# chongchen1999/llm-inference-engine

Measured on AMD Instinct MI355X. Metric: decode_tokens_per_s, higher is better.
Workload: dtype f16; 1 GPU; Llama-2-7B 32-layer fp16 decode, batch 1, ctx 2048 (BASELINE configs[2]); random-init weights, synthetic ids, KV pre-filled; global_batch=1, seq_len=2048, parallelism=replicas x1 (no collective), graph=True, layers=32

## Files before the change

include/llmie.h:

```cpp
#ifndef LLMIE_H
#define LLMIE_H

#include <stddef.h>
#include <stdint.h>

#ifdef __cplusplus
extern "C" {
#endif

#define LLMIE_ABI_VERSION 3

typedef enum { LLMIE_F32 = 0, LLMIE_F16 = 1 } llmie_dtype;

typedef enum {
    LLMIE_OK = 0,
    LLMIE_ERR_INVALID_ARG = -1,
    LLMIE_ERR_UNSUPPORTED = -2,
    LLMIE_ERR_LAUNCH = -3,
    LLMIE_ERR_WORKSPACE = -4
} llmie_status;

typedef void *llmie_stream;

typedef enum {
// ... 60 lines not shown
                      int step, const int32_t *step_dev, int rotary_dim, float rotary_base,
                      llmie_dtype dtype, llmie_stream stream);

size_t llmie_decoder_mha_workspace_bytes(int batch, int head_num, int head_size, int max_seq_len);
int llmie_decoder_mha(const void *qkv, const void *qkv_bias, void *k_cache, void *v_cache,
                      void *out, int layer, int batch, int head_num, int kv_head_num,
                      int head_size, int max_seq_len, int step, const int32_t *step_dev,
                      void *workspace, size_t workspace_bytes,
                      llmie_dtype dtype, llmie_stream stream);

int llmie_decoder_mha_rope(const void *qkv, const void *qkv_bias, void *k_cache, void *v_cache,
                           void *out, int layer, int batch, int head_num, int kv_head_num,
                           int head_size, int max_seq_len, int step, const int32_t *step_dev,
                           void *workspace, size_t workspace_bytes, const void *rope_table,
                           int rotary_dim, int32_t *tickets, llmie_dtype dtype, llmie_stream stream);

int llmie_decoder_mha_ragged(const void *qkv, const void *qkv_bias, void *k_cache, void *v_cache, void *out, int layer,
                             int batch, int head_num, int kv_head_num, int head_size, int max_seq_len,
                             const int32_t *ctx_len_dev, void *workspace, size_t workspace_bytes, const void *rope_table,
                             int rotary_dim, const int32_t *block_table, int max_pages, int num_pages,
                             llmie_dtype dtype, llmie_stream stream);

int llmie_concat_kv(const void *src, void *cache, const int32_t *cur_len,
                    const int32_t *history_len, int layer, int batch, int kv_head_num,
                    int max_q_len, int max_seq_len, int head_size,
                    llmie_dtype dtype, llmie_stream stream);

int llmie_repeat_kv(const void *cache, void *dst, const int32_t *ctx_len, int layer, int batch,
                    int head_num, int kv_head_num, int max_k_len, int max_seq_len, int head_size,
                    llmie_dtype dtype, llmie_stream stream);

int llmie_scale_mask_softmax(const void *qk, const void *mask, void *out, float scale,
                             int batch, int head_num, int q_len, int k_len,
                             llmie_dtype dtype, llmie_stream stream);

int llmie_transpose_remove_padding(const void *src, void *dst, const int32_t *padding_offset,
                                   int num_tokens, int batch, int seq_len, int head_num,
                                   int head_size, llmie_dtype dtype, llmie_stream stream);

int llmie_silu_and_mul(const void *in, void *out, int num_tokens, int inter,
                       llmie_dtype dtype, llmie_stream stream);

int llmie_topk(const void *probs, int32_t *tmp_ids, void *tmp_vals, int32_t *ids, void *vals,
               int rows, int vocab, int K, int blocks_per_row,
               llmie_dtype dtype, llmie_stream stream);

int llmie_sampling(const int32_t *topk_id, const void *topk_val, int32_t *seq_len,
                   uint8_t *finished, int32_t *out_id, int batch, int K, int step,
                   const int32_t *step_dev, int end_id, int vocab,
                   llmie_dtype dtype, llmie_stream stream);

typedef struct {
    float temperature;
    int top_k;
    float top_p;
    float min_p;
    float repetition_penalty;
    float presence_penalty;
    float frequency_penalty;
    uint32_t seed;
} llmie_sampling_params;
#define LLMIE_SAMPLE_MAX_HISTORY 8192
size_t llmie_sample_logits_workspace_bytes(int batch, int vocab);
int llmie_sample_logits(const void *logits, int batch, int vocab, const llmie_sampling_params *params_dev, int32_t *history,
                        int history_stride, int32_t *history_len, int history_append, int32_t *seq_len, uint8_t *finished,
                        int32_t *out_id, float *out_logprob, int step, const int32_t *step_dev, int end_id, void *workspace,
                        size_t workspace_bytes, llmie_dtype dtype, llmie_stream stream);

size_t llmie_score_tokens_workspace_bytes(int rows, int hidden_size, int vocab);
int llmie_score_tokens(const void *hidden, const void *norm_gamma, float rms_eps, const void *lm_head, const void *lm_bias,
                       const int32_t *targets, float *out_logprob, float *out_lse, int32_t *out_argmax,
                       float *out_argmax_logprob, int rows, int hidden_size, int vocab, void *workspace,
                       size_t workspace_bytes, llmie_dtype dtype, llmie_stream stream);


int llmie_linear_w8a16(const void *x, const int8_t *wq, const void *scale, void *y,
                       int M, int K, int N, const void *bias, const void *residual,
                       void *workspace, size_t workspace_bytes, llmie_stream stream);
int llmie_linear_w4a16(const void *x, const uint8_t *wq, const void *scale, void *y,
                       int M, int K, int N, int group, const void *bias, const void *residual,
                       void *workspace, size_t workspace_bytes, llmie_stream stream);
int llmie_linear_fp8(const void *x, const uint8_t *w_fp8, const float *w_scale, void *y,
                     int M, int K, int N, const void *bias, const void *residual,
                     void *workspace, size_t workspace_bytes, llmie_stream stream);
size_t llmie_linear_fp8_workspace_bytes(int M, int K, int N);
int llmie_linear_fp8_swiglu(const void *x, const uint8_t *w_fp8, const float *w_scale, void *y, int M, int K,
                            int two_inter, void *workspace, size_t workspace_bytes, llmie_stream stream);
int llmie_quantize_w8(const void *w, int8_t *wq, void *scale, int N, int K, llmie_stream stream);
int llmie_quantize_w4(const void *w, uint8_t *wq, void *scale, int N, int K, int group,
                      llmie_stream stream);
int llmie_quantize_fp8(const void *w, uint8_t *wq, float *scale, int N, int K, llmie_stream stream);

size_t llmie_packed_weight_bytes(llmie_weight_format fmt, int N, int K, int swiglu_pairs);
size_t llmie_packed_scale_bytes(llmie_weight_format fmt, int N, int K, int swiglu_pairs);
int llmie_pack_weight(llmie_weight_format fmt, const void *w, const void *scale, void *packed, void *packed_scale,
                      int N, int K, int swiglu_pairs, llmie_stream stream);
size_t llmie_linear_packed_workspace_bytes(llmie_weight_format fmt, int M, int K, int N);
enum { LLMIE_X32_X = 1, LLMIE_X32_Y = 2, LLMIE_X32_RES = 4 };
size_t llmie_x32_bytes(int C);
int llmie_x32_convert(const void *src, void *dst, int M, int C, int to_x32, llmie_stream stream);
int llmie_linear_packed(llmie_weight_format fmt, const void *x, const void *packed, const void *scale, void *y,
                        int M, int K, int N, int swiglu, int x32_flags, const void *residual, const void *gamma,
                        const void *pre_bias, float eps, void *workspace, size_t workspace_bytes,
                        llmie_stream stream);


typedef enum { LLMIE_KV_NATIVE = 0, LLMIE_KV_FP8 = 1 } llmie_kv_format;

typedef struct {
    const void *data;
    const void *scale;
    const void *bias;
} llmie_matrix;

typedef struct {
    const void *attn_norm_gamma;
    llmie_matrix qkv;
    llmie_matrix o;
    const void *ffn_norm_gamma;
    llmie_matrix gate_up;
    llmie_matrix down;
} llmie_layer_weights;

typedef struct {
    int head_num, kv_head_num, head_size, inter_size, num_layers, vocab_size;
    int max_seq_len, max_batch;
    int rotary_dim;
    float rotary_base, rms_eps;
    llmie_dtype dtype;
    llmie_weight_format wfmt;
    int int4_group;
    llmie_kv_format kv_fmt;
    float k_scale, v_scale;
    int flags;
} llmie_decoder_config;

#define LLMIE_DEC_NO_PACKED_COPY 1
#define LLMIE_DEC_PACKED_ONLY 2
size_t llmie_decoder_resident_weight_bytes(const llmie_decoder_config *cfg);

#define LLMIE_PLAN_PAGED 1u
#define LLMIE_PLAN_RAGGED 2u
#define LLMIE_PLAN_HIDDEN_MISALIGNED 4u
#define LLMIE_PLAN_WEIGHTS_MISALIGNED 8u
#define LLMIE_PLAN_GAMMAS_MISALIGNED 16u
#define LLMIE_PLAN_O_BIAS 32u
#define LLMIE_PLAN_SCALES_MISALIGNED 64u
#define LLMIE_SW_NO_FUSED_DECODE 1u
#define LLMIE_SW_NO_FUSED_BATCH 2u
#define LLMIE_SW_NO_PACKED_BATCH 4u
#define LLMIE_SW_CHAIN 8u
#define LLMIE_SW_NO_FUSED_SHORT_PREFILL 16u
#define LLMIE_SW_NO_QKV_ROPE_FUSION 32u
const char *llmie_decoder_plan_name(const llmie_decoder_config *cfg, int prefill, int rows, unsigned call_flags, unsigned switch_mask);

typedef struct llmie_decoder llmie_decoder;

size_t llmie_decoder_workspace_bytes(const llmie_decoder_config *cfg);
llmie_decoder *llmie_decoder_create(const llmie_decoder_config *cfg,
                                    const llmie_layer_weights *layers,
                                    void *workspace, size_t workspace_bytes);
void llmie_decoder_destroy(llmie_decoder *dec);
int llmie_decoder_repack(llmie_decoder *dec, const llmie_layer_weights *layers, llmie_stream stream);

int llmie_decoder_forward(llmie_decoder *dec, const void *hidden_in, void *hidden_out,
                          void *k_cache, void *v_cache, int batch, int step,
                          const int32_t *step_dev, llmie_stream stream);

#define LLMIE_KV_PAGE_TOKENS 128
int llmie_decoder_forward_paged(llmie_decoder *dec, const void *hidden_in, void *hidden_out, void *k_pool, void *v_pool,
                                const int32_t *block_table, int max_pages, int num_pages, int batch, int step,
                                const int32_t *step_dev, llmie_stream stream);
int llmie_decoder_forward_ragged(llmie_decoder *dec, const void *hidden_in, void *hidden_out, void *k_cache, void *v_cache,
                                 int batch, const int32_t *ctx_len_dev, llmie_stream stream);
int llmie_decoder_forward_paged_ragged(llmie_decoder *dec, const void *hidden_in, void *hidden_out, void *k_pool, void *v_pool,
                                       const int32_t *block_table, int max_pages, int num_pages, int batch,
                                       const int32_t *ctx_len_dev, llmie_stream stream);
int llmie_decoder_prefill_paged(llmie_decoder *dec, const void *hidden_in, void *hidden_out, void *k_pool, void *v_pool,
                                const int32_t *block_table, int max_pages, int num_pages, const int32_t *input_lengths,
                                const int32_t *history_lengths, int batch, int num_tokens, int max_q_len, void *workspace,
                                size_t workspace_bytes, llmie_stream stream);
int llmie_kv_pages_copy(void *dense, void *pool, const int32_t *block_table, const int32_t *ctx_len, int to_pages,
                        int layers, int batch, int kv_head_num, int max_seq_len, int head_size, int max_pages,
                        int num_pages, int elem_bytes, llmie_stream stream);

size_t llmie_decoder_prefill_workspace_bytes(const llmie_decoder_config *cfg, int max_tokens, int max_batch);
int llmie_decoder_prefill(llmie_decoder *dec, const void *hidden_in, void *hidden_out, void *k_cache, void *v_cache,
                          const int32_t *input_lengths, const int32_t *history_lengths, int batch, int num_tokens,
                          int max_q_len, void *workspace, size_t workspace_bytes, llmie_stream stream);

int llmie_lm_head_sample(llmie_decoder *dec, void *hidden ,
                         const void *final_norm_gamma, const llmie_matrix *lm_head,
                         llmie_weight_format lm_fmt, void *logits,
                         int32_t *tmp_ids, void *tmp_vals, int32_t *topk_ids, void *topk_vals,
                         int K, int blocks_per_row, int32_t *seq_len, uint8_t *finished,
                         int32_t *out_ids, int batch, int step, const int32_t *step_dev,
                         int end_id, llmie_stream stream);

int llmie_lm_head_sample_next(llmie_decoder *dec, void *hidden, const void *final_norm_gamma, const llmie_matrix *lm_head,
                              llmie_weight_format lm_fmt, void *logits, int32_t *tmp_ids, void *tmp_vals, int32_t *topk_ids,
                              void *topk_vals, int K, int blocks_per_row, int32_t *seq_len, uint8_t *finished, int32_t *out_ids,
                              int batch, int step, int32_t *step_dev, int end_id, const void *embed_table, void *next_hidden,
                              int advance_step, llmie_stream stream);

int llmie_lm_head_sample_params(llmie_decoder *dec, void *hidden, const void *final_norm_gamma, const llmie_matrix *lm_head,
                                llmie_weight_format lm_fmt, void *logits, const llmie_sampling_params *params_dev, int32_t *history,
                                int history_stride, int32_t *history_len, int history_append, int32_t *seq_len, uint8_t *finished,
                                int32_t *out_ids, float *out_logprob, int batch, int step, int32_t *step_dev, int end_id,
                                const void *embed_table, void *next_hidden, int advance_step, void *workspace, size_t workspace_bytes,
                                llmie_stream stream);

enum {
    LLMIE_OP_ATTN_NORM = 0, LLMIE_OP_QKV_GEMM, LLMIE_OP_ROPE, LLMIE_OP_MHA, LLMIE_OP_O_GEMM,
    LLMIE_OP_FFN_NORM, LLMIE_OP_GATE_UP_SWIGLU, LLMIE_OP_DOWN_GEMM, LLMIE_OP_FINAL_NORM,
    LLMIE_OP_LM_HEAD, LLMIE_OP_TOPK, LLMIE_OP_SAMPLING,
    LLMIE_OP_CHAIN,
    LLMIE_OP_COUNT
};
int llmie_decoder_profile_begin(llmie_decoder *dec, int max_events);
int llmie_decoder_profile_end(llmie_decoder *dec, llmie_stream stream, double *ms_by_op ,
                              int *launches_by_op );

int llmie_decoder_status(llmie_decoder *dec, llmie_stream stream);
int llmie_decoder_debug_stamps(llmie_decoder *dec, void *stamps_dev);

int llmie_advance_step(int32_t *step_dev, llmie_stream stream);

#ifdef __cplusplus
}
#endif
#endif
```

llm-inference-engine_amd/csrc/attention_decode.hip:

```cpp
#include "llmie_internal.h"

#include <cstdlib>
#include <type_traits>

namespace llmie {

struct fp8kv_t {
    uint8_t b;
};
template <typename KT> struct CacheVec {
    using type = typename Vec16<KT>::type;
    static constexpr int n = Vec16<KT>::n;
};
template <> struct CacheVec<fp8kv_t> {
    using type = uint4_t;
    static constexpr int n = 16;
};
template <typename KT, int N> __device__ __forceinline__ void kv_to_f32(const typename CacheVec<KT>::type &v, float (&o)[N]) {
    if constexpr (std::is_same<KT, fp8kv_t>::value) {
#pragma unroll
        for (int w = 0; w < 4; ++w) {
            const auto lo = __builtin_amdgcn_cvt_pk_f32_fp8(static_cast<int>(v[w]), false);
            const auto hi = __builtin_amdgcn_cvt_pk_f32_fp8(static_cast<int>(v[w]), true);
            o[4 * w] = lo[0];
            o[4 * w + 1] = lo[1];
            o[4 * w + 2] = hi[0];
            o[4 * w + 3] = hi[1];
        }
    } else {
#pragma unroll
        for (int e = 0; e < N; ++e) o[e] = to_f32(v[e]);
    }
}
template <typename KT, typename T, int N> __device__ __forceinline__ typename CacheVec<KT>::type kv_pack(const T (&x)[N], float inv_scale) {
    typename CacheVec<KT>::type v;
    if constexpr (std::is_same<KT, fp8kv_t>::value) {
#pragma unroll
        for (int w = 0; w < 4; ++w)
            v[w] = pack4_e4m3(to_f32(x[4 * w]) * inv_scale, to_f32(x[4 * w + 1]) * inv_scale, to_f32(x[4 * w + 2]) * inv_scale,
                              to_f32(x[4 * w + 3]) * inv_scale);
    } else {
#pragma unroll
        for (int e = 0; e < N; ++e) v[e] = x[e];
    }
    return v;
}
template <typename T, int N> __device__ __forceinline__ void load_elems(const T *p, T (&dst)[N]) {
    constexpr int PER = Vec16<T>::n;
    static_assert(N % PER == 0, "whole 16-byte loads");
#pragma unroll
    for (int c = 0; c < N / PER; ++c) {
        const typename Vec16<T>::type v = reinterpret_cast<const typename Vec16<T>::type *>(p)[c];
#pragma unroll
        for (int e = 0; e < PER; ++e) dst[c * PER + e] = v[e];
    }
}

template <typename KT, int HS, int NWV = 4, int GL = 8> struct AttnGeom {
    static constexpr int N = CacheVec<KT>::n;
    static constexpr int LPT = HS / N;
    static constexpr int TPW = 64 / LPT;
    static constexpr int CHUNK = NWV * GL * TPW;
};

__host__ __device__ inline int attn_min_chunk() { return 32; }

struct QkvSlabs {
    const float *slab;
    int KS;
    size_t stride;
    SlabScale sc;
};

constexpr int KV_PAGE = 128;
struct PagedKv {
    const int32_t *table;
    int max_pages;
    int step_stride;
    int out_x32;
};
__device__ __forceinline__ int seq_step(const int32_t *step_dev, int step_arg, int stride, int b, int max_seq_len) {
    const int s = step_dev ? step_dev[static_cast<size_t>(b) * stride] : step_arg;
    return (s >= 1 && s <= max_seq_len) ? s : 0;
}
__device__ __forceinline__ size_t attn_out_index(int x32, int b, int k, int width) {
    if (!x32) return static_cast<size_t>(b) * width + k;
    return (static_cast<size_t>(k >> 5) * 2 + (b >> 4)) * 512 + ((k & 31) >> 3) * 128 + (b & 15) * 8 + (k & 7);
}

__device__ __forceinline__ void merge_round(const float (&ms)[16], const float (&ls)[16], const float (&os)[16], int s0, int nsplits,
                                            float &M, float &L, float &o) {
    float Mc = M;
#pragma unroll
    for (int i = 0; i < 16; ++i)
        if (s0 + i < nsplits) Mc = fmaxf(Mc, ms[i]);
    const float rescale = (M == -INFINITY) ? 0.f : __expf(M - Mc);
    L *= rescale;
    o *= rescale;
#pragma unroll
    for (int i = 0; i < 16; ++i)
        if (s0 + i < nsplits) {
            const float f = __expf(ms[i] - Mc);
            L = fmaf(f, ls[i], L);
            o = fmaf(f, os[i], o);
        }
    M = Mc;
}
__device__ __forceinline__ void merge_load(const float *__restrict__ p, int s0, int last, size_t stride, int d, float (&ms)[16],
                                           float (&ls)[16], float (&os)[16]) {
#pragma unroll
    for (int i = 0; i < 16; ++i) {
        const int s = min(s0 + i, last);
        ms[i] = p[s * stride];
        ls[i] = p[s * stride + 1];
        os[i] = p[s * stride + 2 + d];
    }
}
__device__ __forceinline__ float merge_splits(const float *__restrict__ p, int nsplits, size_t stride, int d) {
    float M = -INFINITY, L = 0.f, o = 0.f;
    for (int s0 = 0; s0 < nsplits; s0 += 16) {
        float ms[16], ls[16], os[16];
        merge_load(p, s0, nsplits - 1, stride, d, ms, ls, os);
        merge_round(ms, ls, os, s0, nsplits, M, L, o);
    }
    return o / (L + 1e-6f);
}

template <typename T, int HS, int REP, int kAttnWaves = 4, int kAttnG = 8, typename KT = T>
__global__ __launch_bounds__(kAttnWaves * 64) void decode_attn_split_kernel(
    const T *__restrict__ qkv, const T *__restrict__ qkv_bias, KT *k_cache, KT *v_cache,
    float *__restrict__ part, T *__restrict__ out, int head_num, int kv_head_num, int max_seq_len,
    int step_arg, const int32_t *__restrict__ step_dev, int max_splits,
    const float2 *__restrict__ rope , int rotary_dim,
    int32_t *tickets ,
    const QkvSlabs qs ,
    const float k_scale, const float v_scale ,
    const PagedKv pg ,
    const int cpw ) {
    using G = AttnGeom<KT, HS, kAttnWaves, kAttnG>;
    using V = typename CacheVec<KT>::type;
    constexpr int N = G::N, LPT = G::LPT, TPW = G::TPW, CHUNK = G::CHUNK;
    constexpr int NT = kAttnWaves * 64;
    constexpr bool FP8KV = std::is_same<KT, fp8kv_t>::value;
    static_assert(HS % N == 0 && LPT >= 1 && LPT <= 64 && (LPT & (LPT - 1)) == 0, "head size");

    const int split = blockIdx.x, g = blockIdx.y, b = blockIdx.z;
    const int step = seq_step(step_dev, step_arg, pg.step_stride, b, max_seq_len);
    const int span = cpw * CHUNK;
    const int t0 = split * span;
    if (t0 >= step) return;
    int tc0 = t0;
    int t_end = min(step, tc0 + CHUNK);
    const int nsplits = (step + span - 1) / span;
    const int batch = gridDim.z;

    const int lane = threadIdx.x & 63, wave = threadIdx.x >> 6;
    const int sub = lane / LPT, dl = lane % LPT;
    const int qkv_heads = head_num + 2 * kv_head_num;
    const float scale = rsqrtf(static_cast<float>(HS));

    const T *row = qkv + static_cast<size_t>(b) * qkv_heads * HS;
    constexpr int NPG = CHUNK > KV_PAGE ? CHUNK / KV_PAGE : 1;
    static_assert(CHUNK % KV_PAGE == 0 || KV_PAGE % CHUNK == 0, "chunk vs page size");
    int pg0 = 0;
    KT *kbase[NPG], *vbase[NPG];
    auto set_pages = [&]() {
        pg0 = tc0 / KV_PAGE;
#pragma unroll
        for (int j = 0; j < NPG; ++j) {
            size_t off;
            if (pg.table) {
                const int page = pg.table[static_cast<size_t>(b) * pg.max_pages + min(pg0 + j, pg.max_pages - 1)];
                off = (static_cast<size_t>(page) * kv_head_num + g) * KV_PAGE * HS;
            } else {
                off = (static_cast<size_t>(b) * kv_head_num + g) * max_seq_len * HS + static_cast<size_t>(pg0 + j) * KV_PAGE * HS;
            }
            kbase[j] = k_cache + off;
            vbase[j] = v_cache + off;
        }
    };
    set_pages();
    auto krow = [&](int t) { return kbase[NPG == 1 ? 0 : (t / KV_PAGE - pg0)] + static_cast<size_t>(t % KV_PAGE) * HS; };
    auto vrow = [&](int t) { return vbase[NPG == 1 ? 0 : (t / KV_PAGE - pg0)] + static_cast<size_t>(t % KV_PAGE) * HS; };
    KT *kc = kbase[0];
    const int t_new = step - 1;
    T qraw[REP][N];
    constexpr int ITEMS_PER_HEAD = HS / 4;
    constexpr int LROUNDS = ((REP + 2) * ITEMS_PER_HEAD + NT - 1) / NT;
    __shared__ __attribute__((aligned(16))) T qkvlds[(REP + 2) * HS];
    const bool wg_has_new = t_new >= t0 && t_new < t0 + span;
    floatx4 spart[LROUNDS][4];
    half4_t sscale[LROUNDS];
    floatx4 sscalef[LROUNDS];
    const float xs_b = (qs.slab && qs.sc.wf) ? qs.sc.xs[b] : 1.f;
    size_t scol[LROUNDS];
    bool sact[LROUNDS];
    if (qs.slab) {
#pragma unroll
        for (int lr = 0; lr < LROUNDS; ++lr) {
            const int item = lr * NT + threadIdx.x;
            const int hsel = item / ITEMS_PER_HEAD, d4 = item - hsel * ITEMS_PER_HEAD;
            sact[lr] = hsel < REP || (wg_has_new && hsel < REP + 2);
            const int hh = hsel < REP ? g * REP + hsel : (hsel == REP ? head_num + g : head_num + kv_head_num + g);
            scol[lr] = static_cast<size_t>(hh) * HS + d4 * 4;
            if (sact[lr]) {
                const float *p = qs.slab + static_cast<size_t>(b) * qkv_heads * HS + scol[lr];
#pragma unroll
                for (int kk = 0; kk < 4; ++kk)
                    spart[lr][kk] = *reinterpret_cast<const floatx4 *>(p + static_cast<size_t>(min(kk, qs.KS - 1)) * qs.stride);
                if (qs.sc.wh) sscale[lr] = *reinterpret_cast<const half4_t *>(qs.sc.wh + scol[lr]);
                if (qs.sc.wf) sscalef[lr] = *reinterpret_cast<const floatx4 *>(qs.sc.wf + scol[lr]);
            }
        }
    } else {
#pragma unroll
        for (int r = 0; r < REP; ++r) load_elems<T, N>(row + static_cast<size_t>(g * REP + r) * HS + dl * N, qraw[r]);
    }
    const int hk = head_num + g, hv = head_num + kv_head_num + g;
    const T *dummy = reinterpret_cast<const T *>(kc);
    T knraw[N], vnraw[N], qbias[REP][N], kbias[N], vbias[N];
    load_elems<T, N>(qs.slab ? dummy : row + static_cast<size_t>(hk) * HS + dl * N, knraw);
    load_elems<T, N>(qs.slab ? dummy : row + static_cast<size_t>(hv) * HS + dl * N, vnraw);
#pragma unroll
    for (int r = 0; r < REP; ++r)
        load_elems<T, N>(qkv_bias ? qkv_bias + static_cast<size_t>(g * REP + r) * HS + dl * N : dummy, qbias[r]);
    load_elems<T, N>(qkv_bias ? qkv_bias + static_cast<size_t>(hk) * HS + dl * N : dummy, kbias);
    load_elems<T, N>(qkv_bias ? qkv_bias + static_cast<size_t>(hv) * HS + dl * N : dummy, vbias);
    float2 csraw[N];
    if (rope) {
        const float2 *cs = rope + static_cast<size_t>(t_new) * (HS / 2) + (dl % (LPT / 2)) * N;
#pragma unroll
        for (int e = 0; e < N; ++e) csraw[e] = cs[e];
    }
    V kv[kAttnG], vv[kAttnG];
    int tok[kAttnG];
    auto issue_loads = [&]() {
#pragma unroll
        for (int i = 0; i < kAttnG; ++i) {
            const int t = tc0 + (wave * kAttnG + i) * TPW + sub;
            tok[i] = t;
            kv[i] = load_nt(reinterpret_cast<const V *>(krow(min(t, t_end - 1))) + dl);
        }
#pragma unroll
        for (int i = 0; i < kAttnG; ++i)
            vv[i] = load_nt(reinterpret_cast<const V *>(vrow(min(tok[i], t_end - 1))) + dl);
    };
    issue_loads();
    if (qs.slab) {
#pragma unroll
        for (int lr = 0; lr < LROUNDS; ++lr) {
            if (sact[lr]) {
                const float *p = qs.slab + static_cast<size_t>(b) * qkv_heads * HS + scol[lr];
                floatx4 f = spart[lr][0];
#pragma unroll
                for (int kk = 1; kk < 4; ++kk)
                    if (kk < qs.KS) f += spart[lr][kk];
                for (int k = 4; k < qs.KS; ++k) f += *reinterpret_cast<const floatx4 *>(p + static_cast<size_t>(k) * qs.stride);
                const int item = lr * NT + threadIdx.x;
#pragma unroll
                for (int e = 0; e < 4; ++e) {
                    float v = f[e];
                    if (qs.sc.wh) v *= to_f32(sscale[lr][e]);
                    if (qs.sc.wf) v *= sscalef[lr][e] * xs_b;
                    qkvlds[item * 4 + e] = from_f32<T>(v);
                }
            }
        }
        __syncthreads();
#pragma unroll
        for (int r = 0; r < REP; ++r) load_elems<T, N>(&qkvlds[r * HS + dl * N], qraw[r]);
    }
    const bool rope_first = dl < LPT / 2;
    float rc[N], rs[N];
    if (rope) {
#pragma unroll
        for (int e = 0; e < N; ++e) {
            const bool rot = ((dl % (LPT / 2)) * N + e) < (rotary_dim >> 1);
            const float2 v = rot ? csraw[e] : float2{1.f, 0.f};
            rc[e] = v.x;
            rs[e] = rope_first ? -v.y : v.y;
        }
    }
    auto rotate = [&](float (&x)[N]) {
#pragma unroll
        for (int e = 0; e < N; ++e) {
            const float partner = (LPT / 2 < 16) ? lane_xor_lt16<(LPT / 2 < 16 ? LPT / 2 : 8)>(x[e]) : __shfl_xor(x[e], LPT / 2, 64);
            x[e] = x[e] * rc[e] + partner * rs[e];
        }
    };
    const float k_p2 = __builtin_bit_cast(float, __builtin_bit_cast(uint32_t, k_scale) & 0x7f800000u);
    const float k_q = FP8KV ? k_scale / k_p2 : k_scale;
    (void)k_p2;
    float qf[REP][N];
#pragma unroll
    for (int r = 0; r < REP; ++r) {
        float f[N];
#pragma unroll
        for (int e = 0; e < N; ++e) f[e] = to_f32(qraw[r][e]);
        if (rope) {
            rotate(f);
#pragma unroll
            for (int e = 0; e < N; ++e) f[e] = to_f32(from_f32<T>(f[e]));
        }
#pragma unroll
        for (int e = 0; e < N; ++e) {
            f[e] += qkv_bias ? to_f32(qbias[r][e]) : 0.f;
            qf[r][e] = f[e] * (scale * k_q);
        }
    }
    half2_t qh[FP8KV ? REP : 1][FP8KV ? N / 2 : 1];
    if constexpr (FP8KV) {
#pragma unroll
        for (int r = 0; r < REP; ++r)
#pragma unroll
            for (int j = 0; j < N / 2; ++j) qh[r][j] = half2_t{from_f32<half_t>(qf[r][2 * j]), from_f32<half_t>(qf[r][2 * j + 1])};
    }

    V knv, vnv;
    {
        T kn[N], vn[N];
#pragma unroll
        for (int e = 0; e < N; ++e) {
            kn[e] = knraw[e];
            vn[e] = vnraw[e];
        }
        if (qs.slab) {
            load_elems<T, N>(&qkvlds[REP * HS + dl * N], kn);
            load_elems<T, N>(&qkvlds[(REP + 1) * HS + dl * N], vn);
        }
        if (rope) {
            float f[N];
#pragma unroll
            for (int e = 0; e < N; ++e) f[e] = to_f32(kn[e]);
            rotate(f);
#pragma unroll
            for (int e = 0; e < N; ++e) kn[e] = from_f32<T>(f[e]);
        }
#pragma unroll
        for (int e = 0; e < N; ++e) {
            kn[e] = qkv_bias ? from_f32<T>(to_f32(kn[e]) + to_f32(kbias[e])) : kn[e];
            vn[e] = qkv_bias ? from_f32<T>(to_f32(vn[e]) + to_f32(vbias[e])) : vn[e];
        }
        knv = kv_pack<KT, T, N>(kn, 1.0f / k_scale);
        vnv = kv_pack<KT, T, N>(vn, 1.0f / v_scale);
    }
    auto inject = [&]() {
        bool mine = false;
        if (t_new >= tc0 && t_new < tc0 + CHUNK) {
#pragma unroll
        for (int i = 0; i < kAttnG; ++i) {
            const bool is_new = tok[i] == t_new;
            mine |= is_new;
            uint4_t kw = __builtin_bit_cast(uint4_t, kv[i]), vw = __builtin_bit_cast(uint4_t, vv[i]);
            const uint4_t knw = __builtin_bit_cast(uint4_t, knv), vnw = __builtin_bit_cast(uint4_t, vnv);
#pragma unroll
            for (int w = 0; w < 4; ++w) {
                kw[w] = is_new ? knw[w] : kw[w];
                vw[w] = is_new ? vnw[w] : vw[w];
            }
            kv[i] = __builtin_bit_cast(V, kw);
            vv[i] = __builtin_bit_cast(V, vw);
        }
        }
        if (mine) {
            reinterpret_cast<V *>(krow(t_new))[dl] = knv;
            reinterpret_cast<V *>(vrow(t_new))[dl] = vnv;
        }
    };
    inject();

    float mx[REP], acc[REP][N], ls[REP];
#pragma unroll
    for (int r = 0; r < REP; ++r) {
        mx[r] = -INFINITY;
        ls[r] = 0.f;
#pragma unroll
        for (int e = 0; e < N; ++e) acc[r][e] = 0.f;
    }
    auto accumulate = [&](const bool first) {
    float lg[REP][kAttnG];
    float cm[REP];
#pragma unroll
    for (int r = 0; r < REP; ++r) cm[r] = -INFINITY;
#pragma unroll
    for (int i = 0; i < kAttnG; ++i) {
        const bool valid = tok[i] < t_end;
        float kf[FP8KV ? 1 : N];
        half2_t kh[FP8KV ? N / 2 : 1];
        if constexpr (FP8KV) {
            const uint4_t kw = __builtin_bit_cast(uint4_t, kv[i]);
#pragma unroll
            for (int w = 0; w < 4; ++w) {
                kh[2 * w] = __builtin_amdgcn_cvt_scalef32_pk_f16_fp8(static_cast<int>(kw[w]), k_p2, false);
                kh[2 * w + 1] = __builtin_amdgcn_cvt_scalef32_pk_f16_fp8(static_cast<int>(kw[w]), k_p2, true);
            }
        } else {
            kv_to_f32<KT, N>(kv[i], kf);
        }
#pragma unroll
        for (int r = 0; r < REP; ++r) {
            float d = 0.f;
            if (valid) {
                if constexpr (FP8KV) {
#pragma unroll
                    for (int j = 0; j < N / 2; ++j) d = __builtin_amdgcn_fdot2(kh[j], qh[r][j], d, false);
                } else {
#pragma unroll
                    for (int e = 0; e < N; ++e) d = fmaf(qf[r][e], kf[e], d);
                }
            }
            d = group_sum<LPT>(d);
            lg[r][i] = valid ? d : -INFINITY;
            cm[r] = fmaxf(cm[r], lg[r][i]);
        }
    }
#pragma unroll
    for (int r = 0; r < REP; ++r) {
#pragma unroll
        for (int o = LPT; o < 64; o <<= 1) cm[r] = lane_xor_max_o(cm[r], o);
        const float mnew = fmaxf(mx[r], cm[r]);
        if (!first) {
            const float f = (mx[r] == -INFINITY) ? 0.f : __expf(mx[r] - mnew);
            ls[r] *= f;
#pragma unroll
            for (int e = 0; e < N; ++e) acc[r][e] *= f;
        }
        mx[r] = mnew;
    }
#pragma unroll
    for (int i = 0; i < kAttnG; ++i) {
        const bool valid = tok[i] < t_end;
        if (valid) {
            float vf[N];
            kv_to_f32<KT, N>(vv[i], vf);
#pragma unroll
            for (int r = 0; r < REP; ++r) {
                const float p = __expf(lg[r][i] - mx[r]);
                ls[r] += p;
#pragma unroll
                for (int e = 0; e < N; ++e) acc[r][e] = fmaf(p, vf[e], acc[r][e]);
            }
        }
    }
    };
    accumulate(true);
    if constexpr (FP8KV) {
        for (int c = 1; c < cpw; ++c) {
            tc0 += CHUNK;
            if (tc0 >= step) break;
            t_end = min(step, tc0 + CHUNK);
            set_pages();
            issue_loads();
            inject();
            accumulate(false);
        }
    }
#pragma unroll
    for (int r = 0; r < REP; ++r) {
#pragma unroll
        for (int o = LPT; o < 64; o <<= 1) {
            ls[r] = lane_xor_sum_o(ls[r], o);
#pragma unroll
            for (int e = 0; e < N; ++e) acc[r][e] = lane_xor_sum_o(acc[r][e], o);
        }
    }
    __shared__ float s_m[REP][kAttnWaves], s_l[REP][kAttnWaves];
    __shared__ float s_o[REP][kAttnWaves][HS];
    if (sub == 0) {
#pragma unroll
        for (int r = 0; r < REP; ++r) {
#pragma unroll
            for (int e = 0; e < N; ++e) s_o[r][wave][dl * N + e] = acc[r][e] * v_scale;
            if (dl == 0) {
                s_m[r][wave] = mx[r];
                s_l[r][wave] = ls[r];
            }
        }
    }
    __syncthreads();
    for (int i = threadIdx.x; i < REP * HS; i += NT) {
        const int r = i / HS, d = i - r * HS;
        float M = s_m[r][0];
#pragma unroll
        for (int w = 1; w < kAttnWaves; ++w) M = fmaxf(M, s_m[r][w]);
        float L = 0.f, o = 0.f;
#pragma unroll
        for (int w = 0; w < kAttnWaves; ++w) {
            const float f = (s_m[r][w] == -INFINITY) ? 0.f : __expf(s_m[r][w] - M);
            L += f * s_l[r][w];
            o += f * s_o[r][w][d];
        }
        const int h = g * REP + r;
        if (nsplits == 1) {
            out[attn_out_index(pg.out_x32, b, h * HS + d, head_num * HS)] = from_f32<T>(o / (L + 1e-6f));
        } else {
            float *p = part + ((static_cast<size_t>(b) * head_num + h) * max_splits + split) * (HS + 2);
            p[2 + d] = o;
            if (d == 0) {
                p[0] = M;
                p[1] = L;
            }
        }
    }
    (void)batch;
    if (tickets && nsplits > 1) {
        __shared__ int s_ticket;
        asm volatile("s_waitcnt vmcnt(0)" ::: "memory");
        __syncthreads();
        int32_t *cnt = tickets + static_cast<size_t>(b) * kv_head_num + g;
        if (threadIdx.x == 0) {
            __builtin_amdgcn_fence(__ATOMIC_RELEASE, "agent");
            asm volatile("s_waitcnt vmcnt(0)" ::: "memory");
            s_ticket = __hip_atomic_fetch_add(cnt, 1, __ATOMIC_RELAXED, __HIP_MEMORY_SCOPE_AGENT);
        }
        __syncthreads();
        if (s_ticket == nsplits - 1) {
            if (threadIdx.x == 0) {
                __builtin_amdgcn_fence(__ATOMIC_ACQUIRE, "agent");
                asm volatile("s_waitcnt vmcnt(0)" ::: "memory");
                __hip_atomic_store(cnt, 0, __ATOMIC_RELAXED, __HIP_MEMORY_SCOPE_AGENT);
            }
            __syncthreads();
            const size_t stride = static_cast<size_t>(HS) + 2;
            for (int i = threadIdx.x; i < REP * HS; i += NT) {
                const int r = i / HS, d = i - r * HS;
                const int h = g * REP + r;
                const float *p = part + (static_cast<size_t>(b) * head_num + h) * max_splits * stride;
                const float v = merge_splits(p, nsplits, stride, d);
                out[attn_out_index(pg.out_x32, b, h * HS + d, head_num * HS)] = from_f32<T>(v);
            }
        }
    }
}

template <typename T>
__global__ __launch_bounds__(256) void decode_attn_combine_kernel(const float *__restrict__ part,
                                                                  T *__restrict__ out, int head_num,
                                                                  int head_size, int chunk, int step_arg,
                                                                  const int32_t *__restrict__ step_dev,
                                                                  int max_splits, int step_stride, int max_seq_len, int out_x32) {
    const int h = blockIdx.x, b = blockIdx.y;
    const size_t stride = static_cast<size_t>(head_size) + 2;
    const float *p = part + (static_cast<size_t>(b) * head_num + h) * max_splits * stride;
    int d = threadIdx.x;
    float ms[16], ls[16], os[16];
    merge_load(p, 0, max_splits - 1, stride, min(d, head_size - 1), ms, ls, os);
    const int step = seq_step(step_dev, step_arg, step_stride, b, max_seq_len);
    const int nsplits = (step + chunk - 1) / chunk;
    if (nsplits <= 1) return;
    if (d < head_size) {
        float M = -INFINITY, L = 0.f, o = 0.f;
        merge_round(ms, ls, os, 0, nsplits, M, L, o);
        for (int s0 = 16; s0 < nsplits; s0 += 16) {
            merge_load(p, s0, nsplits - 1, stride, d, ms, ls, os);
            merge_round(ms, ls, os, s0, nsplits, M, L, o);
        }
        out[attn_out_index(out_x32, b, h * head_size + d, head_num * head_size)] = from_f32<T>(o / (L + 1e-6f));
    }
    for (d += blockDim.x; d < head_size; d += blockDim.x)
        out[attn_out_index(out_x32, b, h * head_size + d, head_num * head_size)] = from_f32<T>(merge_splits(p, nsplits, stride, d));
}

template <typename T>
__global__ __launch_bounds__(256) void decode_attn_generic_kernel(
    const T *__restrict__ qkv, const T *__restrict__ qkv_bias, T *k_cache, T *v_cache, T *__restrict__ out,
    int head_num, int kv_head_num, int head_size, int max_seq_len, int step_arg,
    const int32_t *__restrict__ step_dev) {
    extern __shared__ float logits[];
    __shared__ float red[4];
    const int h = blockIdx.x, b = blockIdx.y;
    const int step = seq_step(step_dev, step_arg, 0, b, max_seq_len);
    if (step == 0) return;
    const int rep = head_num / kv_head_num, g = h / rep;
    const int qkv_heads = head_num + 2 * kv_head_num;
    const T *row = qkv + static_cast<size_t>(b) * qkv_heads * head_size;
    const int hk = head_num + g, hv = head_num + kv_head_num + g;
    const size_t head_off = (static_cast<size_t>(b) * kv_head_num + g) * max_seq_len * head_size;
    T *kc = k_cache + head_off, *vc = v_cache + head_off;
    const int t_new = step - 1;
    const float scale = rsqrtf(static_cast<float>(head_size));
    auto qv = [&](int d) { return to_f32(row[static_cast<size_t>(h) * head_size + d]) + (qkv_bias ? to_f32(qkv_bias[static_cast<size_t>(h) * head_size + d]) : 0.f); };
    auto knew = [&](int d) { return from_f32<T>(to_f32(row[static_cast<size_t>(hk) * head_size + d]) + (qkv_bias ? to_f32(qkv_bias[static_cast<size_t>(hk) * head_size + d]) : 0.f)); };
    auto vnew = [&](int d) { return from_f32<T>(to_f32(row[static_cast<size_t>(hv) * head_size + d]) + (qkv_bias ? to_f32(qkv_bias[static_cast<size_t>(hv) * head_size + d]) : 0.f)); };
    if (h % rep == 0) {
        for (int d = threadIdx.x; d < head_size; d += 256) {
            kc[static_cast<size_t>(t_new) * head_size + d] = knew(d);
            vc[static_cast<size_t>(t_new) * head_size + d] = vnew(d);
        }
    }
    float mx = -INFINITY;
    for (int t = threadIdx.x; t < step; t += 256) {
        float acc = 0.f;
        for (int d = 0; d < head_size; ++d) {
            const float kvl = (t == t_new) ? to_f32(knew(d)) : to_f32(kc[static_cast<size_t>(t) * head_size + d]);
            acc = fmaf(qv(d), kvl, acc);
        }
        acc *= scale;
        logits[t] = acc;
        mx = fmaxf(mx, acc);
    }
    mx = block_max<4>(mx, red);
    float sum = 0.f;
    for (int t = threadIdx.x; t < step; t += 256) {
        const float p = expf(logits[t] - mx);
        logits[t] = p;
        sum += p;
    }
    sum = block_sum<4>(sum, red) + 1e-6f;
    __syncthreads();
    for (int d = threadIdx.x; d < head_size; d += 256) {
        float o = 0.f;
        for (int t = 0; t < step; ++t) {
            const float vvl = (t == t_new) ? to_f32(vnew(d)) : to_f32(vc[static_cast<size_t>(t) * head_size + d]);
            o = fmaf(logits[t], vvl, o);
        }
        out[(static_cast<size_t>(b) * head_num + h) * head_size + d] = from_f32<T>(o / sum);
    }
}

struct KvScale {
    float k, v;
};

template <typename T, int HS, int REP, typename KT = T>
static void launch_split(const T *qkv, const T *bias, KT *kc, KT *vc, float *part, T *out, int batch,
                         int head_num, int kv_head_num, int max_seq_len, int step, const int32_t *step_dev,
                         int max_splits_ws, const float2 *rope, int rot_dim, int32_t *tickets, const QkvSlabs &qs,
                         KvScale ks, PagedKv pg, hipStream_t st) {
    const int bound = step_dev ? max_seq_len : step;
    int cpw = 1;
    if constexpr (!std::is_same<KT, T>::value) {
        while (cpw < 8 && batch * kv_head_num >= 128 * cpw) cpw *= 2;
    }
    int CHUNK, splits;
#define LLMIE_ATTN_LAUNCH(NWV_, GL_)                                                                                   \
    do {                                                                                                                \
        CHUNK = cpw * AttnGeom<KT, HS, NWV_, GL_>::CHUNK;                                                               \
        splits = (bound + CHUNK - 1) / CHUNK;                                                                           \
        dim3 grid(splits, kv_head_num, batch);                                                                          \
        decode_attn_split_kernel<T, HS, REP, NWV_, GL_, KT><<<grid, NWV_ * 64, 0, st>>>(                                \
            qkv, bias, kc, vc, part, out, head_num, kv_head_num, max_seq_len, step, step_dev, max_splits_ws, rope, rot_dim, \
            tickets, qs, ks.k, ks.v, pg, cpw);                                                                          \
    } while (0)
    LLMIE_ATTN_LAUNCH(4, 8);
#undef LLMIE_ATTN_LAUNCH
    if (splits > 1 && !tickets) {
        dim3 cgrid(head_num, batch);
        decode_attn_combine_kernel<T><<<cgrid, HS < 64 ? 64 : (HS > 256 ? 256 : HS), 0, st>>>(part, out, head_num, HS, CHUNK,
                                                                                              step, step_dev, max_splits_ws, pg.step_stride,
                                                                                              max_seq_len, pg.out_x32);
    }
}

template <typename T, int HS, typename KT = T>
static bool dispatch_rep(int rep, const T *qkv, const T *bias, KT *kc, KT *vc, float *part, T *out, int batch,
                         int head_num, int kv_head_num, int max_seq_len, int step, const int32_t *step_dev,
                         int max_splits_ws, const float2 *rope, int rot_dim, int32_t *tickets, const QkvSlabs &qs,
                         KvScale ks, PagedKv pg, hipStream_t st) {
    switch (rep) {
        case 1: launch_split<T, HS, 1, KT>(qkv, bias, kc, vc, part, out, batch, head_num, kv_head_num, max_seq_len, step, step_dev, max_splits_ws, rope, rot_dim, tickets, qs, ks, pg, st); return true;
        case 2: launch_split<T, HS, 2, KT>(qkv, bias, kc, vc, part, out, batch, head_num, kv_head_num, max_seq_len, step, step_dev, max_splits_ws, rope, rot_dim, tickets, qs, ks, pg, st); return true;
        case 4: launch_split<T, HS, 4, KT>(qkv, bias, kc, vc, part, out, batch, head_num, kv_head_num, max_seq_len, step, step_dev, max_splits_ws, rope, rot_dim, tickets, qs, ks, pg, st); return true;
        case 8:
            if constexpr (!std::is_same<KT, T>::value) return false;
            else launch_split<T, HS, 8, KT>(qkv, bias, kc, vc, part, out, batch, head_num, kv_head_num, max_seq_len, step, step_dev, max_splits_ws, rope, rot_dim, tickets, qs, ks, pg, st); return true;
        default: return false;
    }
}

template <typename T>
static int decoder_mha_impl(const T *qkv, const T *bias, T *k_cache, T *v_cache, T *out, int layer, int batch,
                            int head_num, int kv_head_num, int head_size, int max_seq_len, int step,
                            const int32_t *step_dev, void *workspace, size_t workspace_bytes, const float2 *rope,
                            int rot_dim, int32_t *tickets, const QkvSlabs &qs, hipStream_t st, PagedKv pg = PagedKv{nullptr, 0, 0, 0},
                            int num_pages = 0) {
    const size_t layer_off = pg.table ? static_cast<size_t>(layer) * num_pages * kv_head_num * KV_PAGE * head_size
                                      : static_cast<size_t>(layer) * batch * kv_head_num * max_seq_len * head_size;
    T *kc = k_cache + layer_off, *vc = v_cache + layer_off;
    const int rep = head_num / kv_head_num;
    const int max_splits_ws = (max_seq_len + attn_min_chunk() - 1) / attn_min_chunk();
    const bool aligned = ((reinterpret_cast<uintptr_t>(qkv) | reinterpret_cast<uintptr_t>(kc) |
                           reinterpret_cast<uintptr_t>(vc)) % 16 == 0) && (!bias || reinterpret_cast<uintptr_t>(bias) % 16 == 0);
    bool done = false;
    if (aligned && batch <= 65535 && kv_head_num <= 65535) {
        const size_t need = llmie_decoder_mha_workspace_bytes(batch, head_num, head_size, max_seq_len);
        float *part = static_cast<float *>(workspace);
        auto ws_ok = [&]() { return workspace && workspace_bytes >= need; };
        if (head_size == 128 && ws_ok())
            done = dispatch_rep<T, 128>(rep, qkv, bias, kc, vc, part, out, batch, head_num, kv_head_num, max_seq_len, step, step_dev, max_splits_ws, rope, rot_dim, tickets, qs, KvScale{1.f, 1.f}, pg, st);
        else if (head_size == 64 && ws_ok())
            done = dispatch_rep<T, 64>(rep, qkv, bias, kc, vc, part, out, batch, head_num, kv_head_num, max_seq_len, step, step_dev, max_splits_ws, rope, rot_dim, tickets, qs, KvScale{1.f, 1.f}, pg, st);
        else if (head_size == 32 && ws_ok())
            done = dispatch_rep<T, 32>(rep, qkv, bias, kc, vc, part, out, batch, head_num, kv_head_num, max_seq_len, step, step_dev, max_splits_ws, rope, rot_dim, tickets, qs, KvScale{1.f, 1.f}, pg, st);
        else if (head_size == 256 && ws_ok())
            done = dispatch_rep<T, 256>(rep, qkv, bias, kc, vc, part, out, batch, head_num, kv_head_num, max_seq_len, step, step_dev, max_splits_ws, rope, rot_dim, tickets, qs, KvScale{1.f, 1.f}, pg, st);
        if (!done && (head_size == 128 || head_size == 64 || head_size == 32 || head_size == 256) && !ws_ok() &&
            (rep == 1 || rep == 2 || rep == 4 || rep == 8)) {
            set_error("decoder_mha: workspace too small (%zu < %zu bytes)", workspace_bytes, need);
            return LLMIE_ERR_WORKSPACE;
        }
    }
    if (!done && pg.table) {
        set_error("decoder_mha: the paged KV cache needs head_size in {32,64,128,256} and head_num/kv_head_num in {1,2,4,8}");
        return LLMIE_ERR_UNSUPPORTED;
    }
    if (!done && qs.slab) {
        set_error("decoder_mha: q/k/v from split-K slabs needs head_size in {32,64,128,256} and head_num/kv_head_num in {1,2,4,8}");
        return LLMIE_ERR_UNSUPPORTED;
    }
    if (!done && rope) {
        set_error("decoder_mha: fused RoPE needs head_size in {32,64,128,256} and head_num/kv_head_num in {1,2,4,8}");
        return LLMIE_ERR_UNSUPPORTED;
    }
    if (!done && (pg.step_stride || pg.out_x32)) {
        set_error("decoder_mha: ragged batches / x32 output need head_size in {32,64,128,256} and head_num/kv_head_num in {1,2,4,8}");
        return LLMIE_ERR_UNSUPPORTED;
    }
    if (!done) {
        const int bound = step_dev ? max_seq_len : step;
        const size_t lds = sizeof(float) * static_cast<size_t>(bound);
        if (lds > 60 * 1024) {
            set_error("decoder_mha: generic path supports at most 15360 tokens (head_size=%d, rep=%d)", head_size, rep);
            return LLMIE_ERR_UNSUPPORTED;
        }
        dim3 grid(head_num, batch);
        decode_attn_generic_kernel<T><<<grid, 256, lds, st>>>(qkv, bias, kc, vc, out, head_num, kv_head_num,
                                                             head_size, max_seq_len, step, step_dev);
    }
    return launch_status("decoder_mha");
}

static int decoder_mha_fp8kv(const half_t *qkv, const half_t *bias, uint8_t *k_cache, uint8_t *v_cache, half_t *out, int layer, int batch,
                             int head_num, int kv_head_num, int head_size, int max_seq_len, int step, const int32_t *step_dev,
                             void *workspace, size_t workspace_bytes, const float2 *rope, int rot_dim, const QkvSlabs &qs,
                             KvScale ks, hipStream_t st, PagedKv pg, int num_pages) {
    const size_t layer_off = pg.table ? static_cast<size_t>(layer) * num_pages * kv_head_num * KV_PAGE * head_size
                                      : static_cast<size_t>(layer) * batch * kv_head_num * max_seq_len * head_size;
    fp8kv_t *kc = reinterpret_cast<fp8kv_t *>(k_cache) + layer_off, *vc = reinterpret_cast<fp8kv_t *>(v_cache) + layer_off;
    const int rep = head_num / kv_head_num;
    const int max_splits_ws = (max_seq_len + attn_min_chunk() - 1) / attn_min_chunk();
    const size_t need = llmie_decoder_mha_workspace_bytes(batch, head_num, head_size, max_seq_len);
    if ((reinterpret_cast<uintptr_t>(qkv) | reinterpret_cast<uintptr_t>(kc) | reinterpret_cast<uintptr_t>(vc) |
         reinterpret_cast<uintptr_t>(bias)) % 16 || !workspace || workspace_bytes < need || batch > 65535 || !(ks.k > 0.f) ||
        !(ks.v > 0.f) || (rep != 1 && rep != 2 && rep != 4) || (head_size != 128 && head_size != 64)) {
        set_error("decoder_mha(fp8 KV): needs head_size 64/128, head ratio 1/2/4, 16-byte aligned buffers, positive scales and "
                  "the llmie_decoder_mha workspace");
        return LLMIE_ERR_UNSUPPORTED;
    }
    float *part = static_cast<float *>(workspace);
    bool done;
    if (head_size == 128)
        done = dispatch_rep<half_t, 128, fp8kv_t>(rep, qkv, bias, kc, vc, part, out, batch, head_num, kv_head_num, max_seq_len, step,
                                                  step_dev, max_splits_ws, rope, rot_dim, nullptr, qs, ks, pg, st);
    else
        done = dispatch_rep<half_t, 64, fp8kv_t>(rep, qkv, bias, kc, vc, part, out, batch, head_num, kv_head_num, max_seq_len, step,
                                                 step_dev, max_splits_ws, rope, rot_dim, nullptr, qs, ks, pg, st);
    (void)done;
    return launch_status("decoder_mha(fp8 KV)");
}

int decoder_mha_rope(const void *qkv, const void *qkv_bias, const KvView &kv, void *out, int layer, int batch,
                     int head_num, int kv_head_num, int head_size, int max_seq_len, const DecodePos &pos,
                     void *workspace, size_t workspace_bytes, const float2 *rope, int rot_dim, int32_t *tickets,
                     llmie_dtype dtype, hipStream_t st, const SplitKSlabs *qkv_slabs, const SlabScale *qkv_scale, int out_x32) {
    void *k_cache = kv.k, *v_cache = kv.v;
    const int32_t *block_table = kv.block_table, *step_dev = pos.step_dev;
    const int max_pages = kv.max_pages, num_pages = kv.num_pages, kv_fp8 = kv.fp8, step = pos.step, ragged = pos.ragged;
    const float k_scale = kv.k_scale, v_scale = kv.v_scale;
    const PagedKv pg{block_table, max_pages, ragged ? 1 : 0, out_x32 ? 1 : 0};
    if (ragged && !step_dev) {
        set_error("decoder_mha: a ragged batch needs the device array of context lengths");
        return LLMIE_ERR_INVALID_ARG;
    }
    if (out_x32 && (batch > 32 || dtype != LLMIE_F16)) {
        set_error("decoder_mha: the x32 output image holds at most 32 fp16 rows");
        return LLMIE_ERR_UNSUPPORTED;
    }
    if (block_table && (max_pages <= 0 || num_pages <= 0 || static_cast<long long>(max_pages) * KV_PAGE < max_seq_len)) {
        set_error("decoder_mha: paged KV cache needs max_pages * %d >= max_seq_len and num_pages > 0", KV_PAGE);
        return LLMIE_ERR_UNSUPPORTED;
    }
    QkvSlabs qs{nullptr, 0, 0, SlabScale{nullptr, nullptr, nullptr}};
    const SlabScale no_scale{nullptr, nullptr, nullptr};
    const SlabScale &qsc = qkv_scale ? *qkv_scale : no_scale;
    if (qkv_slabs && (reinterpret_cast<uintptr_t>(qsc.wh) % 8 || reinterpret_cast<uintptr_t>(qsc.wf) % 16 ||
                      reinterpret_cast<uintptr_t>(qkv_slabs->slab) % 16 ||
                      (static_cast<size_t>(qkv_slabs->M) * qkv_slabs->N) % 4)) {
        set_error("decoder_mha: q/k/v from split-K slabs needs 16-byte aligned slabs and aligned scale vectors");
        return LLMIE_ERR_UNSUPPORTED;
    }
    if (qkv_slabs) qs = QkvSlabs{qkv_slabs->slab, qkv_slabs->KS, static_cast<size_t>(qkv_slabs->M) * qkv_slabs->N, qsc};
    if (kv_fp8) {
        if (dtype != LLMIE_F16 || tickets) {
            set_error("decoder_mha(fp8 KV): fp16 activations, separate merge kernel only");
            return LLMIE_ERR_UNSUPPORTED;
        }
        return decoder_mha_fp8kv((const half_t *)qkv, (const half_t *)qkv_bias, (uint8_t *)k_cache, (uint8_t *)v_cache, (half_t *)out,
                                 layer, batch, head_num, kv_head_num, head_size, max_seq_len, step, step_dev, workspace,
                                 workspace_bytes, rope, rot_dim, qs, KvScale{k_scale, v_scale}, st, pg, num_pages);
    }
    if (dtype == LLMIE_F32)
        return decoder_mha_impl<float>((const float *)qkv, (const float *)qkv_bias, (float *)k_cache, (float *)v_cache,
                                       (float *)out, layer, batch, head_num, kv_head_num, head_size, max_seq_len, step,
                                       step_dev, workspace, workspace_bytes, rope, rot_dim, tickets, qs, st, pg, num_pages);
    return decoder_mha_impl<half_t>((const half_t *)qkv, (const half_t *)qkv_bias, (half_t *)k_cache, (half_t *)v_cache,
                                    (half_t *)out, layer, batch, head_num, kv_head_num, head_size, max_seq_len, step,
                                    step_dev, workspace, workspace_bytes, rope, rot_dim, tickets, qs, st, pg, num_pages);
}

}

using namespace llmie;

extern "C" size_t llmie_decoder_mha_workspace_bytes(int batch, int head_num, int head_size, int max_seq_len) {
    if (batch <= 0 || head_num <= 0 || head_size <= 0 || max_seq_len <= 0) return 0;
    const size_t splits = (static_cast<size_t>(max_seq_len) + attn_min_chunk() - 1) / attn_min_chunk();
    return static_cast<size_t>(batch) * head_num * splits * (head_size + 2) * sizeof(float);
}

extern "C" int llmie_decoder_mha(const void *qkv, const void *qkv_bias, void *k_cache, void *v_cache, void *out,
                                 int layer, int batch, int head_num, int kv_head_num, int head_size,
                                 int max_seq_len, int step, const int32_t *step_dev, void *workspace,
                                 size_t workspace_bytes, llmie_dtype dtype, llmie_stream stream) {
    LLMIE_REQUIRE(qkv && k_cache && v_cache && out, "decoder_mha: NULL pointer");
    LLMIE_REQUIRE(layer >= 0 && batch > 0 && head_num > 0 && kv_head_num > 0 && head_size > 0 && max_seq_len > 0,
                  "decoder_mha: bad shape");
    LLMIE_REQUIRE(head_num % kv_head_num == 0, "decoder_mha: kv_head_num must divide head_num");
    LLMIE_REQUIRE(step_dev || (step >= 1 && step <= max_seq_len), "decoder_mha: step %d outside [1, max_seq_len=%d]",
                  step, max_seq_len);
    if (dtype == LLMIE_F32)
        return decoder_mha_impl<float>((const float *)qkv, (const float *)qkv_bias, (float *)k_cache, (float *)v_cache,
                                       (float *)out, layer, batch, head_num, kv_head_num, head_size, max_seq_len, step,
                                       step_dev, workspace, workspace_bytes, nullptr, 0, nullptr, QkvSlabs{nullptr, 0, 0, SlabScale{nullptr, nullptr, nullptr}}, as_stream(stream));
    if (dtype == LLMIE_F16)
        return decoder_mha_impl<half_t>((const half_t *)qkv, (const half_t *)qkv_bias, (half_t *)k_cache,
                                        (half_t *)v_cache, (half_t *)out, layer, batch, head_num, kv_head_num, head_size,
                                        max_seq_len, step, step_dev, workspace, workspace_bytes, nullptr, 0, nullptr, QkvSlabs{nullptr, 0, 0, SlabScale{nullptr, nullptr, nullptr}}, as_stream(stream));
    LLMIE_UNSUPPORTED("decoder_mha: dtype %d", (int)dtype);
}

extern "C" int llmie_decoder_mha_rope(const void *qkv, const void *qkv_bias, void *k_cache, void *v_cache, void *out,
                                      int layer, int batch, int head_num, int kv_head_num, int head_size,
                                      int max_seq_len, int step, const int32_t *step_dev, void *workspace,
                                      size_t workspace_bytes, const void *rope_table, int rotary_dim, int32_t *tickets,
                                      llmie_dtype dtype, llmie_stream stream) {
    LLMIE_REQUIRE(qkv && k_cache && v_cache && out, "decoder_mha_rope: NULL pointer");
    LLMIE_REQUIRE(layer >= 0 && batch > 0 && head_num > 0 && kv_head_num > 0 && head_size > 0 && max_seq_len > 0,
                  "decoder_mha_rope: bad shape");
    LLMIE_REQUIRE(head_num % kv_head_num == 0, "decoder_mha_rope: kv_head_num must divide head_num");
    LLMIE_REQUIRE(step_dev || (step >= 1 && step <= max_seq_len), "decoder_mha_rope: step %d outside [1, max_seq_len=%d]",
                  step, max_seq_len);
    LLMIE_REQUIRE(!rope_table || (rotary_dim > 0 && rotary_dim % 2 == 0), "decoder_mha_rope: bad rotary_dim");
    if (dtype != LLMIE_F32 && dtype != LLMIE_F16) LLMIE_UNSUPPORTED("decoder_mha_rope: dtype %d", (int)dtype);
    const int rep = head_num / kv_head_num;
    const bool hs_ok = head_size == 32 || head_size == 64 || head_size == 128 || head_size == 256;
    const bool rep_ok = rep == 1 || rep == 2 || rep == 4 || rep == 8;
    if ((rope_table || tickets) && !(hs_ok && rep_ok))
        LLMIE_UNSUPPORTED("decoder_mha_rope: fused RoPE / in-launch merge need head_size in {32,64,128,256} and "
                          "head_num/kv_head_num in {1,2,4,8}");
    return decoder_mha_rope(qkv, qkv_bias, kv_dense(k_cache, v_cache), out, layer, batch, head_num, kv_head_num, head_size,
                            max_seq_len, DecodePos{step, step_dev, 0}, workspace, workspace_bytes,
                            static_cast<const float2 *>(rope_table), rotary_dim, tickets, dtype, as_stream(stream));
}

extern "C" int llmie_decoder_mha_ragged(const void *qkv, const void *qkv_bias, void *k_cache, void *v_cache, void *out, int layer,
                                        int batch, int head_num, int kv_head_num, int head_size, int max_seq_len,
                                        const int32_t *ctx_len_dev, void *workspace, size_t workspace_bytes, const void *rope_table,
                                        int rotary_dim, const int32_t *block_table, int max_pages, int num_pages,
                                        llmie_dtype dtype, llmie_stream stream) {
    LLMIE_REQUIRE(qkv && k_cache && v_cache && out && ctx_len_dev, "decoder_mha_ragged: NULL pointer");
    LLMIE_REQUIRE(layer >= 0 && batch > 0 && head_num > 0 && kv_head_num > 0 && head_size > 0 && max_seq_len > 0,
                  "decoder_mha_ragged: bad shape");
    LLMIE_REQUIRE(head_num % kv_head_num == 0, "decoder_mha_ragged: kv_head_num must divide head_num");
    LLMIE_REQUIRE(!rope_table || (rotary_dim > 0 && rotary_dim % 2 == 0), "decoder_mha_ragged: bad rotary_dim");
    if (dtype != LLMIE_F32 && dtype != LLMIE_F16) LLMIE_UNSUPPORTED("decoder_mha_ragged: dtype %d", (int)dtype);
    return decoder_mha_rope(qkv, qkv_bias, KvView{k_cache, v_cache, block_table, max_pages, num_pages, 0, 1.f, 1.f}, out, layer, batch,
                            head_num, kv_head_num, head_size, max_seq_len, DecodePos{-1, ctx_len_dev, 1}, workspace, workspace_bytes,
                            static_cast<const float2 *>(rope_table), rotary_dim, nullptr, dtype, as_stream(stream));
}
```

llm-inference-engine_amd/csrc/engine.hip:

```cpp
#include "llmie_internal.h"

#include <cmath>
#include <cstdlib>
#include <new>
#include <vector>

using namespace llmie;

struct llmie_decoder {
    llmie_decoder_config cfg;
    std::vector<llmie_layer_weights> layers;
    int H, QKV, I;
    size_t esz;
    char *resid, *qkv, *mha, *act, *gu;
    void *attn_ws;
    size_t attn_ws_bytes;
    float2 *rope_table;
    void *fp8_ws;
    size_t fp8_ws_bytes;
    SlabWs slab_ws;
    unsigned *tail_ticket = nullptr;
    struct PackedLayer {
        const unsigned char *qkv, *o, *gate_up, *down;
        const void *sc[4];
    };
    std::vector<PackedLayer> packed;
    int pk_wf = 0;
    bool packed_only = false;
    half_t *hx = nullptr, *actx = nullptr;
    half_t *mhax = nullptr;
    float *pk_slab = nullptr;
    size_t pk_slab_floats = 0;
    unsigned char *pk_base = nullptr;
    unsigned *pk_sync = nullptr, *pk_err = nullptr;
    unsigned long long *pk_stamps = nullptr;
    bool profiling = false;
    std::vector<hipEvent_t> ev;
    std::vector<int> ev_op;
    size_t ev_used = 0;
};

struct OpTimer {
    llmie_decoder *d;
    hipStream_t st;
    bool on;
    size_t idx;
    OpTimer(llmie_decoder *dec, int op, llmie_stream s) : d(dec), st(as_stream(s)), on(false), idx(0) {
        if (d->profiling && d->ev_used + 1 <= d->ev_op.size()) {
            idx = d->ev_used++;
            d->ev_op[idx] = op;
            on = hipEventRecord(d->ev[2 * idx], st) == hipSuccess;
        }
    }
    ~OpTimer() {
        if (on) (void)hipEventRecord(d->ev[2 * idx + 1], st);
    }
};
#define TIMED(op, expr)                 \
    do {                                \
        OpTimer _t(dec, op, stream);    \
        rc = (expr);                    \
    } while (0);                        \
    if (rc) return rc

static size_t align_up(size_t v) { return (v + 255) & ~static_cast<size_t>(255); }

static bool config_ok(const llmie_decoder_config *c) {
    if (!c) return false;
    if (c->head_num <= 0 || c->kv_head_num <= 0 || c->head_size <= 0 || c->inter_size <= 0 ||
        c->num_layers <= 0 || c->max_seq_len <= 0 || c->max_batch <= 0)
        return false;
    if (c->head_num % c->kv_head_num) return false;
    if (c->rotary_dim <= 0 || c->rotary_dim % 2) return false;
    if (c->dtype != LLMIE_F32 && c->dtype != LLMIE_F16) return false;
    if (c->dtype == LLMIE_F32 && c->wfmt != LLMIE_W_F32) return false;
    if (c->dtype == LLMIE_F16 && c->wfmt == LLMIE_W_F32) return false;
    if (c->kv_fmt != LLMIE_KV_NATIVE && c->kv_fmt != LLMIE_KV_FP8) return false;
    if (c->flags & ~(LLMIE_DEC_NO_PACKED_COPY | LLMIE_DEC_PACKED_ONLY)) return false;
    if ((c->flags & LLMIE_DEC_NO_PACKED_COPY) && (c->flags & LLMIE_DEC_PACKED_ONLY)) return false;
    if (c->kv_fmt == LLMIE_KV_FP8) {
        const int rep = c->head_num / c->kv_head_num;
        if (c->dtype != LLMIE_F16 || (c->head_size != 128 && c->head_size != 64) || (rep != 1 && rep != 2 && rep != 4)) return false;
    }
    return true;
}

struct Carve {
    size_t off = 0;
    size_t take(size_t bytes) {
        const size_t o = off;
        off += align_up(bytes);
        return o;
    }
};

static int gemv_max_batch(llmie_weight_format wfmt) {
    switch (wfmt) {
        case LLMIE_W_F16: return 5;
        case LLMIE_W_INT8: return 2;
        case LLMIE_W_FP8: return 2;
        case LLMIE_W_INT4: return 2;
        default: return 4;
    }
}

static int packed_rows_max(const llmie_decoder_config &c) { return c.wfmt == LLMIE_W_FP8 ? 16 : 32; }
static bool packed_batch(const llmie_decoder_config &c, int batch) {
    return (batch > gemv_max_batch(c.wfmt) || (c.flags & LLMIE_DEC_PACKED_ONLY)) && batch <= packed_rows_max(c);
}

static int packed_wf(const llmie_decoder_config *c) {
    if (c->dtype != LLMIE_F16) return 0;
    const int wf = c->wfmt == LLMIE_W_F16 ? PKF_F16
                   : (c->wfmt == LLMIE_W_INT8 ? PKF_I8 : (c->wfmt == LLMIE_W_FP8 ? PKF_FP8 : (c->wfmt == LLMIE_W_INT4 && c->int4_group == 128 ? PKF_I4 : 0)));
    const bool only = (c->flags & LLMIE_DEC_PACKED_ONLY) != 0;
    if (!wf || (c->flags & LLMIE_DEC_NO_PACKED_COPY)) return 0;
    const int rows_max = packed_rows_max(*c);
    if (!packed_batch(*c, only || c->max_batch < rows_max ? c->max_batch : rows_max)) return 0;
    const int H = c->head_num * c->head_size, QKV = (c->head_num + 2 * c->kv_head_num) * c->head_size, I = c->inter_size;
    const int m = c->max_batch < 32 ? c->max_batch : 32;
    if (H % 32 || I % 32) return 0;
    if (!pk_eligible(wf, m, H, QKV, PKE_PLAIN) || !pk_eligible(wf, m, H, H, PKE_PLAIN) || !pk_eligible(wf, m, H, 2 * I, PKE_SWIGLU) ||
        !pk_eligible(wf, m, I, H, PKE_PLAIN))
        return 0;
    return wf;
}
struct PackedCarve {
    size_t per_layer[4], layer_bytes, hx, actx, mhax, slab, sync, total;
};
static PackedCarve packed_carve(const llmie_decoder_config *c, int wf) {
    PackedCarve p{};
    if (!wf) return p;
    const int H = c->head_num * c->head_size, QKV = (c->head_num + 2 * c->kv_head_num) * c->head_size, I = c->inter_size;
    p.per_layer[0] = align_up(pk_packed_bytes(wf, QKV, H, 0)) + align_up(pk_packed_scale_bytes(wf, QKV, H, 0));
    p.per_layer[1] = align_up(pk_packed_bytes(wf, H, H, 0)) + align_up(pk_packed_scale_bytes(wf, H, H, 0));
    p.per_layer[2] = align_up(pk_packed_bytes(wf, 2 * I, H, 1)) + align_up(pk_packed_scale_bytes(wf, 2 * I, H, 1));
    p.per_layer[3] = align_up(pk_packed_bytes(wf, H, I, 0)) + align_up(pk_packed_scale_bytes(wf, H, I, 0));
    p.layer_bytes = p.per_layer[0] + p.per_layer[1] + p.per_layer[2] + p.per_layer[3];
    p.hx = align_up(static_cast<size_t>(H) * 64);
    p.actx = align_up(static_cast<size_t>(I) * 64);
    p.mhax = p.hx;
    const int m = c->max_batch < 32 ? c->max_batch : 32;
    size_t sl = 0;
    for (int mm = 1; mm <= m; ++mm) {
        const size_t f = pk_slab_floats(wf, mm, I, H);
        sl = f > sl ? f : sl;
    }
    p.slab = align_up(sl * sizeof(float) + 16);
    p.sync = align_up(static_cast<size_t>(c->num_layers) * pk_chain_sync_bytes()) + 256;
    p.total = p.layer_bytes * c->num_layers + p.hx + p.actx + p.mhax + p.slab + p.sync;
    return p;
}
static size_t engine_slab_floats(const llmie_decoder_config *c, int rows) {
    int wbits;
    switch (c->wfmt) {
        case LLMIE_W_F16: wbits = 16; break;
// ... 191 lines not shown
        unsigned char *tail = pb + pc.layer_bytes * cfg->num_layers;
        d->hx = reinterpret_cast<half_t *>(tail);
        d->actx = reinterpret_cast<half_t *>(tail + pc.hx);
        d->mhax = reinterpret_cast<half_t *>(tail + pc.hx + pc.actx);
        d->pk_slab = reinterpret_cast<float *>(tail + pc.hx + pc.actx + pc.mhax);
        d->pk_slab_floats = (pc.slab - 16) / sizeof(float);
        d->pk_sync = reinterpret_cast<unsigned *>(tail + pc.hx + pc.actx + pc.mhax + pc.slab);
        d->pk_err = reinterpret_cast<unsigned *>(tail + pc.hx + pc.actx + pc.mhax + pc.slab + pc.sync - 256);
        if (prc != LLMIE_OK || hipMemset(tail, 0, pc.hx + pc.actx + pc.mhax) != hipSuccess || hipMemset(d->pk_sync, 0, pc.sync) != hipSuccess ||
            hipDeviceSynchronize() != hipSuccess) {
            set_error("decoder_create: packing the weights for the batch path failed");
            delete d;
            return nullptr;
        }
        if (cfg->flags & LLMIE_DEC_PACKED_ONLY) {
            d->packed_only = true;
            for (llmie_layer_weights &w : d->layers) w.qkv.data = w.o.data = w.gate_up.data = w.down.data = nullptr;
        }
    }
    {
        const int half = cfg->head_size / 2;
        std::vector<float2> tab(static_cast<size_t>(cfg->max_seq_len) * half);
        for (int pos = 0; pos < cfg->max_seq_len; ++pos)
            for (int j = 0; j < half; ++j) {
                float2 v{1.f, 0.f};
                if (j < cfg->rotary_dim / 2) {
                    const float ang = static_cast<float>(pos) / powf(cfg->rotary_base, static_cast<float>(2 * j) / static_cast<float>(cfg->rotary_dim));
                    v = float2{cosf(ang), sinf(ang)};
                }
                tab[static_cast<size_t>(pos) * half + j] = v;
            }
        if (hipMemcpy(d->rope_table, tab.data(), tab.size() * sizeof(float2), hipMemcpyHostToDevice) != hipSuccess) {
            set_error("decoder_create: RoPE table upload failed");
            delete d;
            return nullptr;
        }
    }
    return d;
}

extern "C" void llmie_decoder_destroy(llmie_decoder *dec) {
    if (!dec) return;
    for (hipEvent_t e : dec->ev) (void)hipEventDestroy(e);
    delete dec;
}

extern "C" int llmie_decoder_profile_begin(llmie_decoder *dec, int max_events) {
    LLMIE_REQUIRE(dec && max_events > 0, "decoder_profile_begin: bad arguments");
    while (dec->ev.size() < 2 * static_cast<size_t>(max_events)) {
        hipEvent_t e;
        if (hipEventCreate(&e) != hipSuccess) {
            set_error("decoder_profile_begin: hipEventCreate failed");
            return LLMIE_ERR_LAUNCH;
        }
        dec->ev.push_back(e);
    }
    dec->ev_op.assign(max_events, 0);
    dec->ev_used = 0;
    dec->profiling = true;
    return LLMIE_OK;
}

extern "C" int llmie_decoder_profile_end(llmie_decoder *dec, llmie_stream stream, double *ms_by_op, int *launches_by_op) {
    LLMIE_REQUIRE(dec && ms_by_op && launches_by_op, "decoder_profile_end: NULL pointer");
    dec->profiling = false;
    if (hipStreamSynchronize(as_stream(stream)) != hipSuccess) {
        set_error("decoder_profile_end: stream synchronise failed");
        return LLMIE_ERR_LAUNCH;
    }
    for (int i = 0; i < LLMIE_OP_COUNT; ++i) {
        ms_by_op[i] = 0.0;
        launches_by_op[i] = 0;
    }
    for (size_t i = 0; i < dec->ev_used; ++i) {
        float ms = 0.f;
        if (hipEventElapsedTime(&ms, dec->ev[2 * i], dec->ev[2 * i + 1]) == hipSuccess) {
            ms_by_op[dec->ev_op[i]] += ms;
            launches_by_op[dec->ev_op[i]] += 1;
        }
    }
    dec->ev_used = 0;
    return LLMIE_OK;
}

extern "C" int llmie_decoder_status(llmie_decoder *dec, llmie_stream stream) {
    LLMIE_REQUIRE(dec, "decoder_status: NULL decoder");
    if (hipStreamSynchronize(as_stream(stream)) != hipSuccess) {
        set_error("decoder_status: stream synchronise failed: %s", hipGetErrorString(hipGetLastError()));
        return LLMIE_ERR_LAUNCH;
    }
    if (!dec->pk_err) return LLMIE_OK;
    unsigned word = 0;
    if (hipMemcpy(&word, dec->pk_err, sizeof(word), hipMemcpyDeviceToHost) != hipSuccess) {
        set_error("decoder_status: reading the device error word failed");
        return LLMIE_ERR_LAUNCH;
    }
    if (word) {
        (void)hipMemset(dec->pk_err, 0, sizeof(word));
        (void)hipMemset(dec->pk_sync, 0, static_cast<size_t>(dec->cfg.num_layers) * pk_chain_sync_bytes());
        set_error("decoder: a grid barrier of the persistent chain launch timed out (code 0x%08x, phase %u): not every workgroup was "
                  "resident; set LLMIE_NO_CHAIN=1 to use the launch sequence", word, word & 0xfu);
        return LLMIE_ERR_LAUNCH;
    }
    return LLMIE_OK;
}

extern "C" int llmie_decoder_debug_stamps(llmie_decoder *dec, void *stamps_dev) {
    LLMIE_REQUIRE(dec, "decoder_debug_stamps: NULL decoder");
    dec->pk_stamps = static_cast<unsigned long long *>(stamps_dev);
    return LLMIE_OK;
}

static int engine_linear(const llmie_decoder *d, llmie_weight_format fmt, const void *x, const llmie_matrix &w,
                         void *y, int M, int K, int N, bool swiglu, const void *residual, bool use_bias,
                         llmie_stream stream) {
    const void *bias = use_bias ? w.bias : nullptr;
    switch (fmt) {
        case LLMIE_W_F16:
            return linear_f16_nk((const half_t *)x, (const half_t *)w.data, (half_t *)y, M, K, N,
                                 swiglu ? EPI_SWIGLU_ : EPI_NONE_, (const half_t *)bias, (const half_t *)residual, d->slab_ws,
                                 as_stream(stream));
        case LLMIE_W_F32:
            if (swiglu) {
                int rc = llmie_linear(x, w.data, d->gu, M, K, N, 1, bias, nullptr, LLMIE_F32, nullptr, 0, stream);
                if (rc) return rc;
                return llmie_silu_and_mul(d->gu, y, M, N / 2, LLMIE_F32, stream);
            }
            return llmie_linear(x, w.data, y, M, K, N, 1, bias, residual, LLMIE_F32, nullptr, 0, stream);
        case LLMIE_W_INT8:
        case LLMIE_W_INT4: {
            const int bits = fmt == LLMIE_W_INT8 ? 8 : 4;
            int rc = linear_wq(bits, (const half_t *)x, w.data, (const half_t *)w.scale, (half_t *)y, M, K, N, d->cfg.int4_group,
                               swiglu ? EPI_SWIGLU_ : EPI_NONE_, (const half_t *)bias, (const half_t *)residual, nullptr, nullptr,
                               0.f, d->slab_ws, as_stream(stream));
            return rc;
        }
        case LLMIE_W_FP8: {
            if (swiglu) {
                int rc = linear_fp8((const half_t *)x, (const uint8_t *)w.data, (const float *)w.scale, (half_t *)d->gu, M, K, N,
                                    (const half_t *)bias, nullptr, d->fp8_ws, d->fp8_ws_bytes, d->slab_ws, as_stream(stream));
                if (rc) return rc;
                return llmie_silu_and_mul(d->gu, y, M, N / 2, LLMIE_F16, stream);
            }
            return linear_fp8((const half_t *)x, (const uint8_t *)w.data, (const float *)w.scale, (half_t *)y, M, K, N,
                              (const half_t *)bias, (const half_t *)residual, d->fp8_ws, d->fp8_ws_bytes, d->slab_ws, as_stream(stream));
        }
        default:
            set_error("engine: weight format %d not supported by this build", (int)fmt);
            return LLMIE_ERR_UNSUPPORTED;
    }
}

struct EngineSwitches {
    bool no_fused_decode, no_fused_batch, no_packed_batch, chain, no_fused_short_prefill, no_qkv_rope_fusion;
};
static const EngineSwitches &engine_switches() {
    static const EngineSwitches s{getenv("LLMIE_NO_FUSED_DECODE") != nullptr,        getenv("LLMIE_NO_FUSED_BATCH") != nullptr,
                                  getenv("LLMIE_NO_PACKED_BATCH") != nullptr,        getenv("LLMIE_CHAIN") != nullptr,
                                  getenv("LLMIE_NO_FUSED_SHORT_PREFILL") != nullptr, getenv("LLMIE_NO_QKV_ROPE_FUSION") != nullptr};
    return s;
}
static EngineSwitches switches_of_mask(unsigned m) {
    return EngineSwitches{(m & LLMIE_SW_NO_FUSED_DECODE) != 0,        (m & LLMIE_SW_NO_FUSED_BATCH) != 0, (m & LLMIE_SW_NO_PACKED_BATCH) != 0,
                          (m & LLMIE_SW_CHAIN) != 0,                  (m & LLMIE_SW_NO_FUSED_SHORT_PREFILL) != 0,
                          (m & LLMIE_SW_NO_QKV_ROPE_FUSION) != 0};
}
static bool fused_attention_geometry(const llmie_decoder_config &c) {
    const int rep = c.head_num / c.kv_head_num;
    return (c.head_size == 32 || c.head_size == 64 || c.head_size == 128 || c.head_size == 256) && (rep == 1 || rep == 2 || rep == 4 || rep == 8);
}

enum DecodePath : int { DP_REFUSED = 0, DP_GEMV, DP_PACKED, DP_PACKED_CHAIN, DP_SPLITK, DP_UNFUSED };
enum DecodeRefusal : int { DREF_NONE = 0, DREF_PACKED_ONLY, DREF_PAGED, DREF_KV_FP8, DREF_RAGGED };
struct DecodeCall {
    llmie_decoder_config cfg;
    int batch;
    bool paged, ragged;
    unsigned mis_hidden, mis_wqkv0;
    EngineSwitches sw;
};
struct DecodePlan {
    int path, refusal;
    bool chain_wanted;
};
static DecodePlan plan_decode(const DecodeCall &d) {
    const llmie_decoder_config &c = d.cfg;
    const int batch = d.batch, H = c.head_num * c.head_size, I = c.inter_size;
    const bool attn_ok = fused_attention_geometry(c);
    const int wbits = c.wfmt == LLMIE_W_F16 ? 16 : (c.wfmt == LLMIE_W_INT8 ? 8 : (c.wfmt == LLMIE_W_INT4 ? 4 : 0));
    const bool fp8 = c.wfmt == LLMIE_W_FP8, packed_only = (c.flags & LLMIE_DEC_PACKED_ONLY) != 0;
    const int gemv_max = gemv_max_batch(c.wfmt);
    const bool int4_ok = wbits == 4 && c.int4_group == 128 && batch <= 64;
    const bool batch_path_ok = !d.sw.no_fused_batch && c.dtype == LLMIE_F16 && (wbits == 16 || wbits == 8 || int4_ok || fp8) && attn_ok &&
                               batch <= 128 && H % 256 == 0 && I % 256 == 0 && H >= 512 && I >= 512 && splitk_rownorm_eligible(H);
    const bool gemv_ok = !packed_only && (batch <= gemv_max || !batch_path_ok) &&
                         (wbits == 16 ? gemv_f16_eligible(batch, H, reinterpret_cast<const void *>(static_cast<uintptr_t>(d.mis_hidden)),
                                                          reinterpret_cast<const void *>(static_cast<uintptr_t>(d.mis_wqkv0)))
                                      : ((wbits != 0 || fp8) && ksplit_eligible(batch, H, fp8 ? 8 : wbits)));
    if (!d.sw.no_fused_decode && c.dtype == LLMIE_F16 && (wbits != 0 || fp8) && attn_ok && H % 8 == 0 && gemv_ok) return {DP_GEMV, DREF_NONE, false};
    const bool packed_on = !d.sw.no_packed_batch && !d.sw.no_fused_decode && attn_ok;
    if (packed_only && !(packed_on && packed_batch(c, batch))) return {DP_REFUSED, DREF_PACKED_ONLY, false};
    if (packed_on && packed_wf(&c) && packed_batch(c, batch)) return {DP_PACKED, DREF_NONE, d.sw.chain};
    if (batch_path_ok) return {DP_SPLITK, DREF_NONE, false};
    if (d.paged) return {DP_REFUSED, DREF_PAGED, false};
    if (c.kv_fmt == LLMIE_KV_FP8) return {DP_REFUSED, DREF_KV_FP8, false};
    if (d.ragged && !attn_ok) return {DP_REFUSED, DREF_RAGGED, false};
    return {DP_UNFUSED, DREF_NONE, false};
}
static int decode_refuse(const DecodeCall &d, const DecodePlan &p) {
    switch (p.refusal) {
        case DREF_PACKED_ONLY:
            set_error("decoder_forward: a LLMIE_DEC_PACKED_ONLY engine decodes on the packed kernels only (batch <= %d, no path switch)",
                      packed_rows_max(d.cfg));
            break;
        case DREF_PAGED: set_error("decoder_forward_paged: the paged KV cache needs the fused decode paths (fp16 engines, batch <= 128)"); break;
        case DREF_KV_FP8:
            set_error("decoder_forward: the fp8 KV cache needs the fused decode paths (batch <= 128, fp16/int8/int4/fp8 weights with "
                      "H and I multiples of 256 at batch > 8)");
            break;
        default: set_error("decoder_forward_ragged: needs head_size in {32,64,128,256} and head_num/kv_head_num in {1,2,4,8}"); break;
    }
    return LLMIE_ERR_UNSUPPORTED;
}
static const char *decode_path_name(int path) {
    static const char *const names[] = {"refused", "gemv", "packed", "packed_chain", "splitk", "unfused"};
    return names[path];
}

enum PrefillPath : int { PP_REFUSED = 0, PP_PACKED_ONLY, PP_SHORT_SPLITK, PP_LEAN, PP_GENERAL };
enum PrefillRefusal : int { PREF_NONE = 0, PREF_FORMAT, PREF_PACKED_ONLY_FP8 };
struct PrefillCall {
    llmie_decoder_config cfg;
    int T;
    bool weights_a16;
    bool int4_scales_a4;
    bool hidden_gammas_a16;
    bool o_bias;
    EngineSwitches sw;
};
struct PrefillPlan {
    int path, refusal;
};
static PrefillPlan plan_prefill(const PrefillCall &p) {
    const llmie_decoder_config &c = p.cfg;
    const int T = p.T, H = c.head_num * c.head_size, I = c.inter_size;
    const bool fp8 = c.wfmt == LLMIE_W_FP8;
    const int wqbits = c.wfmt == LLMIE_W_INT8 ? 8 : (c.wfmt == LLMIE_W_INT4 ? 4 : 0);
    if (c.dtype != LLMIE_F16 || (c.wfmt != LLMIE_W_F16 && !fp8 && !wqbits) || c.head_size != 128) return {PP_REFUSED, PREF_FORMAT};
    if (c.flags & LLMIE_DEC_PACKED_ONLY) return fp8 ? PrefillPlan{PP_REFUSED, PREF_PACKED_ONLY_FP8} : PrefillPlan{PP_PACKED_ONLY, PREF_NONE};
    const bool short_fmt_ok = !fp8 && (wqbits != 4 || (c.int4_group == 128 && T <= 64));
    if (!p.sw.no_fused_short_prefill && short_fmt_ok && p.weights_a16 && (wqbits != 4 || p.int4_scales_a4) && T <= 128 && H % 256 == 0 &&
        I % 256 == 0 && H >= 512 && I >= 512 && splitk_rownorm_eligible(H))
        return {PP_SHORT_SPLITK, PREF_NONE};
    if (!fp8 && p.hidden_gammas_a16 && rmsnorm_oop_eligible(H) && !p.o_bias) return {PP_LEAN, PREF_NONE};
    return {PP_GENERAL, PREF_NONE};
}
static int prefill_refuse(const PrefillPlan &p) {
    if (p.refusal == PREF_FORMAT)
        LLMIE_UNSUPPORTED("decoder_prefill: fp16 activations + fp16 / int8 / int4 / fp8 weights + head_size 128 only (use the per-kernel path)");
    LLMIE_UNSUPPORTED("decoder_prefill: LLMIE_DEC_PACKED_ONLY engines prefill fp16 / int8 / int4 weights only");
}
static const char *prefill_path_name(int path) {
    static const char *const names[] = {"refused", "packed_only", "short_splitk", "lean", "general"};
    return names[path];
}

extern "C" const char *llmie_decoder_plan_name(const llmie_decoder_config *cfg, int prefill, int rows, unsigned call_flags,
                                               unsigned switch_mask) {
    if (!config_ok(cfg)) {
        set_error("decoder_plan_name: invalid config");
        return nullptr;
    }
    if ((cfg->flags & LLMIE_DEC_PACKED_ONLY) && !packed_wf(cfg)) {
        set_error("decoder_create: LLMIE_DEC_PACKED_ONLY needs max_batch <= 32 (fp8: 16) and shapes / a format the packed kernels take");
        return nullptr;
    }
    const EngineSwitches sw = switches_of_mask(switch_mask);
    if (prefill) {
        if (rows < 1) {
            set_error("decoder_plan_name: %d tokens", rows);
            return nullptr;
        }
        const PrefillCall pc{*cfg, rows, !(call_flags & LLMIE_PLAN_WEIGHTS_MISALIGNED), !(call_flags & LLMIE_PLAN_SCALES_MISALIGNED),
                             !(call_flags & (LLMIE_PLAN_HIDDEN_MISALIGNED | LLMIE_PLAN_GAMMAS_MISALIGNED)), (call_flags & LLMIE_PLAN_O_BIAS) != 0, sw};
        const PrefillPlan p = plan_prefill(pc);
        if (p.path == PP_REFUSED) return (void)prefill_refuse(p), nullptr;
        return prefill_path_name(p.path);
    }
    if (rows < 1 || rows > cfg->max_batch) {
        set_error("decoder_forward: batch %d outside [1,%d]", rows, cfg->max_batch);
        return nullptr;
    }
    const DecodeCall dc{*cfg, rows, (call_flags & LLMIE_PLAN_PAGED) != 0, (call_flags & LLMIE_PLAN_RAGGED) != 0,
                        (call_flags & LLMIE_PLAN_HIDDEN_MISALIGNED) ? 8u : 0u, (call_flags & LLMIE_PLAN_WEIGHTS_MISALIGNED) ? 8u : 0u, sw};
    const DecodePlan p = plan_decode(dc);
    if (p.path == DP_REFUSED) return (void)decode_refuse(dc, p), nullptr;
    return decode_path_name(p.path);
}

static KvView kv_view(const llmie_decoder_config &c, void *k, void *v, const int32_t *block_table, int max_pages, int num_pages) {
    const bool fp8 = c.kv_fmt == LLMIE_KV_FP8;
    return KvView{k, v, block_table, max_pages, num_pages, fp8 ? 1 : 0, (fp8 && c.k_scale > 0.f) ? c.k_scale : 1.f,
                  (fp8 && c.v_scale > 0.f) ? c.v_scale : 1.f};
}

struct DecodeStep {
    llmie_decoder *dec;
    const llmie_decoder_config &c;
    void *h;
    int batch;
    KvView kv;
    DecodePos pos;
    llmie_stream stream;
    hipStream_t st;
    int H, QKV, I, wbits;
    bool fp8;
    llmie_dtype dt;

    int attention(const void *qkv, const void *qkv_bias, void *out, int layer, const SplitKSlabs *qkv_slabs = nullptr,
                  const SlabScale *qkv_scale = nullptr, int out_x32 = 0) const {
        return decoder_mha_rope(qkv, qkv_bias, kv, out, layer, batch, c.head_num, c.kv_head_num, c.head_size, c.max_seq_len, pos, dec->attn_ws,
                                dec->attn_ws_bytes, dec->rope_table, c.rotary_dim, nullptr, dt, st, qkv_slabs, qkv_scale, out_x32);
    }

    int gemv() const {
        int rc;
        auto lin = [&](const void *x, const llmie_matrix &w, void *y, int K, int N, int epi, const void *residual,
                       const void *gamma, const void *pre_bias) -> int {
            if (fp8) {
                if (ksplit_eligible(batch, K, 8))
                    return linear_fp8_gemv((const half_t *)x, (const uint8_t *)w.data, (const float *)w.scale, (half_t *)y, batch,
                                           K, N, epi, nullptr, (const half_t *)residual, (const half_t *)gamma,
                                           (const half_t *)pre_bias, c.rms_eps, st);
                return linear_fp8((const half_t *)x, (const uint8_t *)w.data, (const float *)w.scale, (half_t *)y, batch, K, N, nullptr,
                                  (const half_t *)residual, dec->fp8_ws, dec->fp8_ws_bytes, dec->slab_ws, st);
            }
            if (wbits == 16) {
                if (gamma)
                    return linear_f16_nk_norm((const half_t *)x, (const half_t *)w.data, (half_t *)y, batch, K, N, epi, nullptr,
                                              (const half_t *)residual, (const half_t *)gamma, (const half_t *)pre_bias,
                                              c.rms_eps, st);
                return linear_f16_nk((const half_t *)x, (const half_t *)w.data, (half_t *)y, batch, K, N, epi, nullptr,
                                     (const half_t *)residual, dec->slab_ws, st);
            }
            return linear_wq(wbits, (const half_t *)x, w.data, (const half_t *)w.scale, (half_t *)y, batch, K, N, c.int4_group,
                             epi, nullptr, (const half_t *)residual, (const half_t *)gamma, (const half_t *)pre_bias,
                             c.rms_eps, dec->slab_ws, st);
        };
        for (int l = 0; l < c.num_layers; ++l) {
            const llmie_layer_weights &w = dec->layers[l];
            TIMED(LLMIE_OP_QKV_GEMM, lin(h, w.qkv, dec->qkv, H, QKV, EPI_NONE_, nullptr, w.attn_norm_gamma, nullptr));
            TIMED(LLMIE_OP_MHA, attention(dec->qkv, w.qkv.bias, dec->mha, l));
            TIMED(LLMIE_OP_O_GEMM, lin(dec->mha, w.o, h, H, H, EPI_NONE_, h, nullptr, nullptr));
            TIMED(LLMIE_OP_GATE_UP_SWIGLU, lin(h, w.gate_up, dec->act, H, 2 * I, EPI_SWIGLU_, nullptr, w.ffn_norm_gamma, w.o.bias));
            TIMED(LLMIE_OP_DOWN_GEMM, lin(dec->act, w.down, h, I, H, EPI_NONE_, h, nullptr, nullptr));
        }
        return LLMIE_OK;
    }

    int packed() const {
        int rc;
        const int wf = dec->pk_wf;
        half_t *hh = static_cast<half_t *>(h);
        half_t *qkvb = reinterpret_cast<half_t *>(dec->qkv);
        for (int l = 0; l < c.num_layers; ++l) {
            const llmie_layer_weights &w = dec->layers[l];
            const llmie_decoder::PackedLayer &pw = dec->packed[l];
            const bool first = l == 0, last = l + 1 == c.num_layers;
            TIMED(LLMIE_OP_QKV_GEMM, pk_linear(wf, first ? hh : dec->hx, pw.qkv, pw.sc[0] ? pw.sc[0] : w.qkv.scale, qkvb, batch, H, QKV, PKE_PLAIN, first ? 0 : PKX_X,
                                               nullptr, static_cast<const half_t *>(w.attn_norm_gamma), nullptr, c.rms_eps, nullptr, 0, st));
            TIMED(LLMIE_OP_MHA, attention(dec->qkv, w.qkv.bias, dec->mhax, l, nullptr, nullptr, 1));
            TIMED(LLMIE_OP_O_GEMM, pk_linear(wf, dec->mhax, pw.o, pw.sc[1] ? pw.sc[1] : w.o.scale, dec->hx, batch, H, H, PKE_PLAIN, PKX_X | PKX_Y | (first ? 0 : PKX_RES),
                                             first ? hh : dec->hx, nullptr, nullptr, 0.f, nullptr, 0, st));
            TIMED(LLMIE_OP_GATE_UP_SWIGLU, pk_linear(wf, dec->hx, pw.gate_up, pw.sc[2] ? pw.sc[2] : w.gate_up.scale, dec->actx, batch, H, 2 * I, PKE_SWIGLU, PKX_X | PKX_Y,
                                                     nullptr, static_cast<const half_t *>(w.ffn_norm_gamma), static_cast<const half_t *>(w.o.bias),
                                                     c.rms_eps, nullptr, 0, st));
            TIMED(LLMIE_OP_DOWN_GEMM, pk_linear(wf, dec->actx, pw.down, pw.sc[3] ? pw.sc[3] : w.down.scale, last ? hh : dec->hx, batch, I, H, PKE_PLAIN,
                                                PKX_X | PKX_RES | (last ? 0 : PKX_Y), dec->hx, nullptr, nullptr, 0.f, dec->pk_slab,
                                                dec->pk_slab_floats, st));
        }
        return LLMIE_OK;
    }
    bool chain_joins() const {
        if (!dec->pk_sync) return false;
        const int wf = dec->pk_wf;
        half_t *qkvb = reinterpret_cast<half_t *>(dec->qkv);
        const llmie_layer_weights &w = dec->layers[0];
        const llmie_decoder::PackedLayer &pw = dec->packed[0];
        PkChain ch;
        pk_chain_begin(&ch, wf, batch);
        return ch.ok &&
                !pk_chain_add(&ch, 0, dec->mhax, pw.o, pw.sc[1] ? pw.sc[1] : w.o.scale, dec->hx, H, H, PKE_PLAIN, PKX_X | PKX_Y | PKX_RES, dec->hx, nullptr, nullptr, 0.f, nullptr, 0) &&
                !pk_chain_add(&ch, 1, dec->hx, pw.gate_up, pw.sc[2] ? pw.sc[2] : w.gate_up.scale, dec->actx, H, 2 * I, PKE_SWIGLU, PKX_X | PKX_Y, nullptr,
                              static_cast<const half_t *>(w.ffn_norm_gamma), static_cast<const half_t *>(w.o.bias), c.rms_eps, nullptr, 0) &&
                !pk_chain_add(&ch, 2, dec->actx, pw.down, pw.sc[3] ? pw.sc[3] : w.down.scale, dec->hx, I, H, PKE_PLAIN, PKX_X | PKX_RES | PKX_Y, dec->hx, nullptr, nullptr,
                              0.f, dec->pk_slab, dec->pk_slab_floats) &&
                (c.num_layers == 1 ||
                 !pk_chain_add(&ch, 4, dec->hx, pw.qkv, pw.sc[0] ? pw.sc[0] : w.qkv.scale, qkvb, H, QKV, PKE_PLAIN, PKX_X, nullptr,
                               static_cast<const half_t *>(w.attn_norm_gamma), nullptr, c.rms_eps, nullptr, 0));
    }
    int packed_chain() const {
        int rc;
        const int wf = dec->pk_wf;
        half_t *hh = static_cast<half_t *>(h);
        half_t *qkvb = reinterpret_cast<half_t *>(dec->qkv);
        for (int l = 0; l < c.num_layers; ++l) {
            const llmie_layer_weights &w = dec->layers[l];
            const llmie_decoder::PackedLayer &pw = dec->packed[l];
            const bool first = l == 0, last = l + 1 == c.num_layers;
            if (first)
                TIMED(LLMIE_OP_QKV_GEMM, pk_linear(wf, hh, pw.qkv, pw.sc[0] ? pw.sc[0] : w.qkv.scale, qkvb, batch, H, QKV, PKE_PLAIN, 0, nullptr,
                                                   static_cast<const half_t *>(w.attn_norm_gamma), nullptr, c.rms_eps, nullptr, 0, st));
            TIMED(LLMIE_OP_MHA, attention(dec->qkv, w.qkv.bias, dec->mhax, l, nullptr, nullptr, 1));
            PkChain ch;
            pk_chain_begin(&ch, wf, batch);
            rc = pk_chain_add(&ch, 0, dec->mhax, pw.o, pw.sc[1] ? pw.sc[1] : w.o.scale, dec->hx, H, H, PKE_PLAIN, PKX_X | PKX_Y | (first ? 0 : PKX_RES),
                              first ? hh : dec->hx, nullptr, nullptr, 0.f, nullptr, 0);
            if (!rc) rc = pk_chain_add(&ch, 1, dec->hx, pw.gate_up, pw.sc[2] ? pw.sc[2] : w.gate_up.scale, dec->actx, H, 2 * I, PKE_SWIGLU, PKX_X | PKX_Y, nullptr,
                                       static_cast<const half_t *>(w.ffn_norm_gamma), static_cast<const half_t *>(w.o.bias), c.rms_eps, nullptr, 0);
            if (!rc) rc = pk_chain_add(&ch, 2, dec->actx, pw.down, pw.sc[3] ? pw.sc[3] : w.down.scale, last ? hh : dec->hx, I, H, PKE_PLAIN,
                                       PKX_X | PKX_RES | (last ? 0 : PKX_Y), dec->hx, nullptr, nullptr, 0.f, dec->pk_slab, dec->pk_slab_floats);
            if (!rc && !last) {
                const llmie_layer_weights &wn = dec->layers[l + 1];
                const llmie_decoder::PackedLayer &pn = dec->packed[l + 1];
                rc = pk_chain_add(&ch, 4, dec->hx, pn.qkv, pn.sc[0] ? pn.sc[0] : wn.qkv.scale, qkvb, H, QKV, PKE_PLAIN, PKX_X, nullptr,
                                  static_cast<const half_t *>(wn.attn_norm_gamma), nullptr, c.rms_eps, nullptr, 0);
            }
            if (rc) return rc;
            ch.stamps = dec->pk_stamps;
            TIMED(LLMIE_OP_CHAIN, pk_chain_launch(&ch, dec->pk_sync + static_cast<size_t>(l) * (pk_chain_sync_bytes() / sizeof(unsigned)), dec->pk_err, st));
        }
        return LLMIE_OK;
    }

    int splitk() const {
        int rc;
        half_t *hh = static_cast<half_t *>(h), *resid = reinterpret_cast<half_t *>(dec->resid);
        half_t *mha = reinterpret_cast<half_t *>(dec->mha), *act = reinterpret_cast<half_t *>(dec->act);
        const int fmt = fp8 ? WF_FP8 : wbits;
        const size_t unit = dec->fp8_ws_bytes, kmax = static_cast<size_t>(I > H ? I : H);
        auto xq_of = [&](int u) { return fp8 ? reinterpret_cast<uint8_t *>(dec->fp8_ws) + u * unit : nullptr; };
        auto xs_of = [&](int u) {
            return fp8 ? reinterpret_cast<float *>(xq_of(u) + ((static_cast<size_t>(c.max_batch) * kmax + 255) & ~size_t(255))) : nullptr;
        };
        uint8_t *xqA = xq_of(0), *xqB = xq_of(1), *xqC = xq_of(2);
        float *xsA = xs_of(0), *xsB = xs_of(1), *xsC = xs_of(2);
        auto scale_of = [&](const llmie_matrix &m, const float *xs) {
            if (fp8) return SlabScale{nullptr, static_cast<const float *>(m.scale), xs};
            return SlabScale{wbits == 8 ? static_cast<const half_t *>(m.scale) : nullptr, nullptr, nullptr};
        };
        auto gs_of = [&](const llmie_matrix &m) { return wbits == 4 ? static_cast<const half_t *>(m.scale) : nullptr; };
        TIMED(LLMIE_OP_ATTN_NORM, llmie_rmsnorm(h, dec->resid, dec->layers[0].attn_norm_gamma, c.rms_eps, batch, H, dt, stream));
        if (fp8) TIMED(LLMIE_OP_ATTN_NORM, quantize_rows_fp8(hh, xqA, xsA, batch, H, st));
        for (int l = 0; l < c.num_layers; ++l) {
            const llmie_layer_weights &w = dec->layers[l];
            const bool last = l + 1 == c.num_layers;
            const void *xin = fp8 ? static_cast<const void *>(xqA) : hh;
            SplitKSlabs sk;
            TIMED(LLMIE_OP_QKV_GEMM, linear_splitk_partial(fmt, xin, w.qkv.data, batch, H, QKV, st, &sk, dec->slab_ws, gs_of(w.qkv)));
            const SlabScale qsc = scale_of(w.qkv, xsA);
            TIMED(LLMIE_OP_MHA, attention(nullptr, w.qkv.bias, dec->mha, l, &sk, &qsc));
            if (fp8) TIMED(LLMIE_OP_O_GEMM, quantize_rows_fp8(mha, xqB, xsB, batch, H, st));
            TIMED(LLMIE_OP_O_GEMM, linear_splitk_partial(fmt, fp8 ? static_cast<const void *>(xqB) : mha, w.o.data, batch, H, H, st, &sk, dec->slab_ws, gs_of(w.o)));
            TIMED(LLMIE_OP_FFN_NORM, splitk_rownorm(sk, scale_of(w.o, xsB), static_cast<const half_t *>(w.o.bias), resid,
                                                    static_cast<const half_t *>(w.ffn_norm_gamma), c.rms_eps,
                                                    fp8 ? nullptr : hh, xqA, xsA, st));
            TIMED(LLMIE_OP_GATE_UP_SWIGLU, linear_splitk_partial(fmt, xin, w.gate_up.data, batch, H, 2 * I, st, &sk, dec->slab_ws, gs_of(w.gate_up)));
            TIMED(LLMIE_OP_GATE_UP_SWIGLU, splitk_finalize(sk, scale_of(w.gate_up, xsA), act, EPI_SWIGLU_, nullptr, nullptr, st));
            if (fp8) TIMED(LLMIE_OP_DOWN_GEMM, quantize_rows_fp8(act, xqC, xsC, batch, I, st));
            TIMED(LLMIE_OP_DOWN_GEMM, linear_splitk_partial(fmt, fp8 ? static_cast<const void *>(xqC) : act, w.down.data, batch, I, H, st, &sk, dec->slab_ws, gs_of(w.down)));
            const void *next_gamma = last ? nullptr : dec->layers[l + 1].attn_norm_gamma;
            TIMED(LLMIE_OP_ATTN_NORM, splitk_rownorm(sk, scale_of(w.down, xsC), nullptr, resid, static_cast<const half_t *>(next_gamma),
                                                     c.rms_eps, (fp8 && !last) ? nullptr : hh, last ? nullptr : xqA, xsA, st));
        }
        return LLMIE_OK;
    }
    int unfused() const;
};

int DecodeStep::unfused() const {
    int rc;
    const bool fused_rope = fused_attention_geometry(c);
    for (int l = 0; l < c.num_layers; ++l) {
        const llmie_layer_weights &w = dec->layers[l];
        TIMED(LLMIE_OP_ATTN_NORM, llmie_rmsnorm(h, dec->resid, w.attn_norm_gamma, c.rms_eps, batch, H, dt, stream));
        TIMED(LLMIE_OP_QKV_GEMM, engine_linear(dec, c.wfmt, h, w.qkv, dec->qkv, batch, H, QKV, false, nullptr, false, stream));
        if (fused_rope) {
            TIMED(LLMIE_OP_MHA, attention(dec->qkv, w.qkv.bias, dec->mha, l));
        } else {
            TIMED(LLMIE_OP_ROPE, llmie_rope_decode(dec->qkv, batch, c.head_num, c.kv_head_num, c.head_size, pos.step, pos.step_dev,
                                                   c.rotary_dim, c.rotary_base, dt, stream));
            TIMED(LLMIE_OP_MHA, llmie_decoder_mha(dec->qkv, w.qkv.bias, kv.k, kv.v, dec->mha, l, batch, c.head_num,
                                                  c.kv_head_num, c.head_size, c.max_seq_len, pos.step, pos.step_dev, dec->attn_ws,
                                                  dec->attn_ws_bytes, dt, stream));
        }
        TIMED(LLMIE_OP_O_GEMM, engine_linear(dec, c.wfmt, dec->mha, w.o, h, batch, H, H, false, nullptr, false, stream));
        TIMED(LLMIE_OP_FFN_NORM, llmie_fused_add_bias_residual_rmsnorm(dec->resid, h, w.o.bias, w.ffn_norm_gamma,
                                                                       c.rms_eps, batch, H, dt, stream));
        TIMED(LLMIE_OP_GATE_UP_SWIGLU, engine_linear(dec, c.wfmt, h, w.gate_up, dec->act, batch, H, 2 * I, true, nullptr, false, stream));
        TIMED(LLMIE_OP_DOWN_GEMM, engine_linear(dec, c.wfmt, dec->act, w.down, h, batch, I, H, false, dec->resid, false, stream));
    }
    return LLMIE_OK;
}

static int decoder_forward(llmie_decoder *dec, const void *hidden_in, void *hidden_out, void *k_cache, void *v_cache,
                           const int32_t *block_table, int max_pages, int num_pages, int batch, const DecodePos &pos, llmie_stream stream) {
    LLMIE_REQUIRE(dec && hidden_in && hidden_out && k_cache && v_cache, "decoder_forward: NULL pointer");
    const llmie_decoder_config &c = dec->cfg;
    LLMIE_REQUIRE(batch >= 1 && batch <= c.max_batch, "decoder_forward: batch %d outside [1,%d]", batch, c.max_batch);
    LLMIE_REQUIRE(pos.step_dev || (pos.step >= 1 && pos.step <= c.max_seq_len), "decoder_forward: step %d outside [1,%d]", pos.step,
                  c.max_seq_len);
    if (hidden_out != hidden_in) {
        hipError_t e = hipMemcpyAsync(hidden_out, hidden_in, static_cast<size_t>(batch) * dec->H * dec->esz,
                                      hipMemcpyDeviceToDevice, as_stream(stream));
        if (e != hipSuccess) {
            set_error("decoder_forward: copy failed: %s", hipGetErrorString(e));
            return LLMIE_ERR_LAUNCH;
        }
    }
    const DecodeCall call{c, batch, block_table != nullptr, pos.ragged != 0, mis16(hidden_out), mis16(dec->layers[0].qkv.data), engine_switches()};
    const DecodePlan plan = plan_decode(call);
    const DecodeStep s{dec, c, hidden_out, batch, kv_view(c, k_cache, v_cache, block_table, max_pages, num_pages), pos, stream, as_stream(stream),
                       dec->H, dec->QKV, dec->I, c.wfmt == LLMIE_W_F16 ? 16 : (c.wfmt == LLMIE_W_INT8 ? 8 : (c.wfmt == LLMIE_W_INT4 ? 4 : 0)),
                       c.wfmt == LLMIE_W_FP8, c.dtype};
    switch (plan.path) {
        case DP_GEMV: return s.gemv();
        case DP_PACKED: return plan.chain_wanted && s.chain_joins() ? s.packed_chain() : s.packed();
        case DP_SPLITK: return s.splitk();
        case DP_UNFUSED: return s.unfused();
        default: return decode_refuse(call, plan);
    }
}

extern "C" int llmie_decoder_forward(llmie_decoder *dec, const void *hidden_in, void *hidden_out, void *k_cache,
                                     void *v_cache, int batch, int step, const int32_t *step_dev,
                                     llmie_stream stream) {
    return decoder_forward(dec, hidden_in, hidden_out, k_cache, v_cache, nullptr, 0, 0, batch, DecodePos{step, step_dev, 0}, stream);
}

extern "C" int llmie_decoder_forward_ragged(llmie_decoder *dec, const void *hidden_in, void *hidden_out, void *k_cache,
                                            void *v_cache, int batch, const int32_t *ctx_len_dev, llmie_stream stream) {
    LLMIE_REQUIRE(dec && ctx_len_dev, "decoder_forward_ragged: NULL pointer");
    return decoder_forward(dec, hidden_in, hidden_out, k_cache, v_cache, nullptr, 0, 0, batch, DecodePos{-1, ctx_len_dev, 1}, stream);
}

static int paged_args_ok(const llmie_decoder *dec, const int32_t *block_table, int max_pages, int num_pages, const char *who) {
    LLMIE_REQUIRE(dec && block_table, "%s: NULL pointer", who);
    LLMIE_REQUIRE(max_pages > 0 && num_pages > 0 &&
                      static_cast<long long>(max_pages) * LLMIE_KV_PAGE_TOKENS >= dec->cfg.max_seq_len,
                  "%s: max_pages * %d must cover max_seq_len %d", who, LLMIE_KV_PAGE_TOKENS, dec->cfg.max_seq_len);
    return LLMIE_OK;
}

extern "C" int llmie_decoder_forward_paged_ragged(llmie_decoder *dec, const void *hidden_in, void *hidden_out, void *k_pool,
                                                  void *v_pool, const int32_t *block_table, int max_pages, int num_pages, int batch,
                                                  const int32_t *ctx_len_dev, llmie_stream stream) {
    LLMIE_REQUIRE(dec && ctx_len_dev, "decoder_forward_paged_ragged: NULL pointer");
    if (int rc = paged_args_ok(dec, block_table, max_pages, num_pages, "decoder_forward_paged")) return rc;
    return decoder_forward(dec, hidden_in, hidden_out, k_pool, v_pool, block_table, max_pages, num_pages, batch, DecodePos{-1, ctx_len_dev, 1},
                           stream);
}

extern "C" int llmie_decoder_forward_paged(llmie_decoder *dec, const void *hidden_in, void *hidden_out, void *k_pool, void *v_pool,
                                           const int32_t *block_table, int max_pages, int num_pages, int batch, int step,
                                           const int32_t *step_dev, llmie_stream stream) {
    if (int rc = paged_args_ok(dec, block_table, max_pages, num_pages, "decoder_forward_paged")) return rc;
    return decoder_forward(dec, hidden_in, hidden_out, k_pool, v_pool, block_table, max_pages, num_pages, batch, DecodePos{step, step_dev, 0},
                           stream);
}

static size_t prefill_slab_floats(const llmie_decoder_config *c, int T) {
    size_t m = engine_slab_floats(c, T < 192 ? T : 192);
    if (T > 192 && c->wfmt != LLMIE_W_FP8) {
        const int H = c->head_num * c->head_size, QKV = (c->head_num + 2 * c->kv_head_num) * c->head_size, I = c->inter_size;
        const int shapes[4][2] = {{H, QKV}, {H, H}, {H, 2 * I}, {I, H}};
        for (const auto &sh : shapes) {
            const size_t f = linear_f16_reserve_slab_floats(T, sh[0], sh[1]);
            m = f > m ? f : m;
        }
    }
    return m;
}
struct PrefillCarve {
    size_t resid, qkv, attn, gu, act, pad, cum, fp8_ws, slabs, deq, tokens, total;
};
static PrefillCarve prefill_carve(const llmie_decoder_config *c, int T, int B) {
    const size_t e = 2, H = static_cast<size_t>(c->head_num) * c->head_size;
    const size_t QKV = static_cast<size_t>(c->head_num + 2 * c->kv_head_num) * c->head_size, I = c->inter_size;
    Carve k;
    PrefillCarve o;
    o.resid = k.take(static_cast<size_t>(T) * H * e);
    o.qkv = k.take(static_cast<size_t>(T) * QKV * e);
    o.attn = k.take(static_cast<size_t>(T) * H * e);
    o.gu = k.take(static_cast<size_t>(T) * 2 * I * e);
    o.act = k.take(static_cast<size_t>(T) * I * e);
    o.pad = k.take(static_cast<size_t>(T) * sizeof(int32_t));
    o.cum = k.take(static_cast<size_t>(B + 1) * sizeof(int32_t));
    o.fp8_ws = k.take(c->wfmt == LLMIE_W_FP8 ? llmie_linear_fp8_workspace_bytes(T, static_cast<int>(I > H ? I : H), 0) : 256);
    o.slabs = k.take(prefill_slab_floats(c, T) * sizeof(float) + 256);
    size_t dq = 0;
    if (c->wfmt == LLMIE_W_INT8 || c->wfmt == LLMIE_W_INT4 || (c->flags & LLMIE_DEC_PACKED_ONLY)) {
        const size_t shapes[4][2] = {{H, QKV}, {H, H}, {H, 2 * I}, {I, H}};
        for (const auto &sh : shapes) {
            const size_t b = sh[0] * sh[1] * sizeof(half_t);
            dq = b > dq ? b : dq;
        }
    }
    o.deq = k.take(dq + 256);
    o.tokens = k.take(static_cast<size_t>(T) * 2 * sizeof(int32_t) + 256);
    o.total = k.off;
    return o;
}

extern "C" size_t llmie_decoder_prefill_workspace_bytes(const llmie_decoder_config *cfg, int max_tokens, int max_batch) {
    if (!config_ok(cfg) || max_tokens <= 0 || max_batch <= 0) return 0;
    return prefill_carve(cfg, max_tokens, max_batch).total;
}

struct PrefillPass {
    llmie_decoder *dec;
    const llmie_decoder_config &c;
    llmie_stream stream;
    hipStream_t st;
    KvView kv;
    const int32_t *cum, *history_lengths;
    int batch, T, max_q_len, H, QKV, I;
    bool fp8;
    int wqbits;
    half_t *h, *resid, *qkv, *attn, *gu, *act;
    void *f8ws;
    size_t f8ws_bytes;
    SlabWs slabs;
    void *deq;
    size_t deq_bytes;
    QkvRopeArgs *rope_args;
    bool rope_fuse_off, rope_fusable;

    int proj(const half_t *x, const llmie_matrix &w, half_t *y, int K, int N, const half_t *residual) const {
        if (wqbits)
            return linear_wq(wqbits, x, w.data, (const half_t *)w.scale, y, T, K, N, c.int4_group, EPI_NONE_, nullptr, residual, nullptr,
                             nullptr, 0.f, slabs, st, deq, deq_bytes);
        if (fp8)
            return linear_fp8(x, (const uint8_t *)w.data, (const float *)w.scale, y, T, K, N, nullptr, residual, f8ws, f8ws_bytes,
                              slabs, st);
        return linear_f16_nk(x, (const half_t *)w.data, y, T, K, N, EPI_NONE_, nullptr, residual, slabs, st);
    }
    int gate_up(const half_t *x, const llmie_matrix &w) const {
        int rc;
        const LinearCall gc = linear_call(wqbits ? wqbits : 16, T, H, 2 * I, EPI_SWIGLU_, c.int4_group, x, w.data, w.scale, act, nullptr, nullptr,
                                          nullptr, nullptr, slabs, wqbits ? deq : nullptr, deq_bytes);
        if (wqbits && (T < kWqPrefillRows || gemm256_swiglu_fills(T, 2 * I)) && plan_linear_wq(gc).route != LR_REFUSED) {
            TIMED(LLMIE_OP_GATE_UP_SWIGLU, linear_wq(wqbits, x, w.data, (const half_t *)w.scale, act, T, H, 2 * I, c.int4_group, EPI_SWIGLU_,
                                                     nullptr, nullptr, nullptr, nullptr, 0.f, slabs, st, deq, deq_bytes));
        } else if (!wqbits && plan_linear_f16(gc).route != LR_REFUSED) {
            TIMED(LLMIE_OP_GATE_UP_SWIGLU, linear_f16_nk(x, (const half_t *)w.data, act, T, H, 2 * I, EPI_SWIGLU_, nullptr, nullptr, slabs, st));
        } else {
            TIMED(LLMIE_OP_GATE_UP_SWIGLU, proj(x, w, gu, H, 2 * I, nullptr));
            TIMED(LLMIE_OP_GATE_UP_SWIGLU, llmie_silu_and_mul(gu, act, T, I, LLMIE_F16, stream));
        }
        return LLMIE_OK;
    }
    int qkv_rope(int l, const llmie_matrix &w, G256Operands ops, const void *x, const float *xs, const void *Wd, const void *wsc) const {
        gemm256_qkv_rope_launch(ops, x, Wd, qkv, T, QKV, H, xs, static_cast<const float *>(wsc), static_cast<const half_t *>(w.bias), rope_args, l, st);
        return launch_status("decoder_prefill(qkv + rope + append)");
    }
    int qkv_proj(int l, const llmie_matrix &w, const half_t *x, int *fused) const {
        *fused = 0;
        if (rope_fusable && !fp8 && reinterpret_cast<uintptr_t>(w.bias) % 8 == 0) {
            if (!wqbits && gemm256_qkv_rope_eligible(G256_F16, T, QKV, H, x, w.data, nullptr, qkv)) {
                *fused = 1;
                return qkv_rope(l, w, G256_F16, x, nullptr, w.data, nullptr);
            }
            const int route = !wqbits ? LR_REFUSED
                                      : plan_linear_wq(linear_call(wqbits, T, H, QKV, EPI_NONE_, c.int4_group, x, w.data, w.scale, qkv, nullptr, nullptr,
                                                                   nullptr, nullptr, slabs, deq, deq_bytes)).route;
            if (route == LR_W8_G8P && gemm256_qkv_rope_eligible(G256_W8, T, QKV, H, x, w.data, w.scale, qkv)) {
                *fused = 1;
// ... 340 lines not shown
```

llm-inference-engine_amd/csrc/gemm_kernels.cuh:

```cuda
#pragma once
#include "device_utils.cuh"

namespace llmie {

enum : int { EPI_NONE = 0, EPI_SWIGLU = 1 };


struct GemvArgs {
    const half_t *x;
    const void *W;
    half_t *y;
    int K, N;
    const half_t *bias;
    const half_t *residual;
    const half_t *gamma;
    const half_t *pre_bias;
    float eps;
    int epi, norm;
    const void *scale;
    int group;
};


template <int WBITS> struct WFmt;
template <> struct WFmt<16> { static constexpr int XE = 1; };
template <> struct WFmt<8> { static constexpr int XE = 2; };
template <> struct WFmt<4> { static constexpr int XE = 4; };

__device__ __forceinline__ half2_t as_half2(unsigned int u) { return __builtin_bit_cast(half2_t, u); }

template <int WBITS, bool FP8 = false>
__device__ __forceinline__ float chunk_dot(const uint4_t w, const half8_t (&x)[WFmt<WBITS>::XE], float acc) {
    if constexpr (WBITS == 16) {
        return dot8(__builtin_bit_cast(half8_t, w), x[0], acc);
    } else if constexpr (WBITS == 8 && FP8) {
#pragma unroll
        for (int i = 0; i < 4; ++i) {
            const half2_t wlo = __builtin_amdgcn_cvt_scalef32_pk_f16_fp8(static_cast<int>(w[i]), 1.0f, false);
            const half2_t whi = __builtin_amdgcn_cvt_scalef32_pk_f16_fp8(static_cast<int>(w[i]), 1.0f, true);
            const half8_t xv = x[i >> 1];
            const int b = (i & 1) * 4;
            acc = __builtin_amdgcn_fdot2(wlo, half2_t{xv[b], xv[b + 1]}, acc, false);
            acc = __builtin_amdgcn_fdot2(whi, half2_t{xv[b + 2], xv[b + 3]}, acc, false);
        }
        return acc;
    } else if constexpr (WBITS == 8) {
#pragma unroll
        for (int i = 0; i < 4; ++i) {
            const unsigned int v = w[i] ^ 0x80808080u;
            const unsigned int lo = __builtin_amdgcn_perm(0x64646464u, v, 0x04010400u);
            const unsigned int hi = __builtin_amdgcn_perm(0x64646464u, v, 0x04030402u);
            const half2_t wlo = as_half2(lo), whi = as_half2(hi);
            const half8_t xv = x[i >> 1];
            const int b = (i & 1) * 4;
            acc = __builtin_amdgcn_fdot2(wlo, half2_t{xv[b], xv[b + 1]}, acc, false);
            acc = __builtin_amdgcn_fdot2(whi, half2_t{xv[b + 2], xv[b + 3]}, acc, false);
        }
        return acc;
    } else {
#pragma unroll
        for (int i = 0; i < 4; ++i) {
            const half8_t xv = x[i];
            const unsigned int w0 = w[i], w8 = w[i] >> 8;
            const half2_t h0 = as_half2((w0 & 0x000F000Fu) | 0x64006400u);
            const half2_t h1 = as_half2((w0 & 0x00F000F0u) | 0x64006400u);
            const half2_t h2 = as_half2((w8 & 0x000F000Fu) | 0x64006400u);
            const half2_t h3 = as_half2((w8 & 0x00F000F0u) | 0x64006400u);
            acc = __builtin_amdgcn_fdot2(h0, half2_t{xv[0], xv[1]}, acc, false);
            acc = __builtin_amdgcn_fdot2(h1, half2_t{xv[2], xv[3]}, acc, false);
            acc = __builtin_amdgcn_fdot2(h2, half2_t{xv[4], xv[5]}, acc, false);
            acc = __builtin_amdgcn_fdot2(h3, half2_t{xv[6], xv[7]}, acc, false);
        }
        return acc;
    }
}
__device__ __forceinline__ half8_t prescale_x_int4(const half8_t v) {
    const float s = 0.0625f;
    return half8_t{v[0], v[1], from_f32<half_t>(to_f32(v[2]) * s), from_f32<half_t>(to_f32(v[3]) * s),
                   v[4], v[5], from_f32<half_t>(to_f32(v[6]) * s), from_f32<half_t>(to_f32(v[7]) * s)};
}
__device__ __forceinline__ float int4_offset_term(const half8_t v) {
    return 1032.0f * (to_f32(v[0]) + to_f32(v[1]) + to_f32(v[4]) + to_f32(v[5])) +
           1152.0f * (to_f32(v[2]) + to_f32(v[3]) + to_f32(v[6]) + to_f32(v[7]));
}
__device__ __forceinline__ half8_t permute_x_int4(const half8_t v) {
    return half8_t{v[0], v[4], v[1], v[5], v[2], v[6], v[3], v[7]};
}

template <int M, int RPW, int XC, int WBITS, bool DB = false, bool FP8 = false, int RI = 1>
__global__ __launch_bounds__(256) void gemv_ksplit_kernel(const GemvArgs a) {
    static_assert(RPW % 2 == 0, "rows come in pairs");
    constexpr int XE = WFmt<WBITS>::XE;
    constexpr int EPC = 8 * XE;
    __shared__ float red[2][4][M * RPW];
    __shared__ float ssq[4][M];
    const int K = a.K, N = a.N;
    const int nch = K / EPC;
    const int nx8 = K >> 3;
    const size_t row_bytes = static_cast<size_t>(K) * WBITS / 8;
    static_assert(RI == 1 || RI == 2, "one or two rows per workgroup instruction");
    const int tid = threadIdx.x, lane = tid & 63, wave = tid >> 6;
    constexpr int TPR = 256 / RI, WPR = 4 / RI;
    const int sub = tid / TPR, ct = tid % TPR;
    const bool swiglu = a.epi == EPI_SWIGLU;
    const int half_n = N >> 1;
    const int out_n = swiglu ? half_n : N;
    const int ngroups = swiglu ? (half_n + (RPW / 2) * RI - 1) / ((RPW / 2) * RI) : (N + RPW * RI - 1) / (RPW * RI);
    auto row_of = [&](int grp, int r) {
        int row = swiglu ? (grp * (RPW / 2) + (r >> 1)) * RI + sub + (r & 1) * half_n : (grp * RPW + r) * RI + sub;
        const int lim = swiglu ? ((r & 1) ? N : half_n) : N;
        return row < lim ? row : lim - 1;
    };

    half8_t xr[M][XC][XE];
    const half8_t *xg = reinterpret_cast<const half8_t *>(a.x);
#pragma unroll
    for (int m = 0; m < M; ++m)
#pragma unroll
        for (int j = 0; j < XC; ++j) {
            const int cc = j * TPR + ct;
#pragma unroll
            for (int e = 0; e < XE; ++e)
                xr[m][j][e] = cc < nch ? xg[m * nx8 + cc * XE + e] : half8_t{0, 0, 0, 0, 0, 0, 0, 0};
        }
    half8_t g[XC][XE];
    if (a.norm) {
        const half8_t *gm = reinterpret_cast<const half8_t *>(a.gamma);
#pragma unroll
        for (int j = 0; j < XC; ++j) {
            const int cc = j * TPR + ct;
#pragma unroll
            for (int e = 0; e < XE; ++e) g[j][e] = cc < nch ? gm[cc * XE + e] : half8_t{0, 0, 0, 0, 0, 0, 0, 0};
        }
    }
    constexpr int SR = WBITS == 4 ? RPW : 1, SX = WBITS == 4 ? XC : 1;
    uint4_t wbA[RPW][XC], wbB[DB ? RPW : 1][DB ? XC : 1];
    half_t wscA[SR][SX], wscB[DB ? SR : 1][DB ? SX : 1];
    const unsigned char *Wb = reinterpret_cast<const unsigned char *>(a.W);
    const half_t *scale = reinterpret_cast<const half_t *>(a.scale);
    const int sgroups = (WBITS == 4) ? K / a.group : 1;
    auto load_group = [&](int grp, auto &wb, auto &wsc) {
#pragma unroll
        for (int r = 0; r < RPW; ++r) {
            const uint4_t *w = reinterpret_cast<const uint4_t *>(Wb + static_cast<size_t>(row_of(grp, r)) * row_bytes);
            if constexpr (WBITS == 4) {
                const half_t *srow = scale + static_cast<size_t>(row_of(grp, r)) * sgroups;
#pragma unroll
                for (int j = 0; j < XC; ++j) wsc[r][j] = srow[(min(j * TPR + ct, nch - 1) * EPC) / a.group];
            }
#pragma unroll
            for (int j = 0; j < XC; ++j) {
                const int cc = min(j * TPR + ct, nch - 1);
                wb[r][j] = load_nt(w + cc);
            }
        }
    };
    int grp = blockIdx.x;
    if (grp < ngroups) load_group(grp, wbA, wscA);

    if (a.norm) {
        const half8_t *pb = reinterpret_cast<const half8_t *>(a.pre_bias);
        if (pb) {
#pragma unroll
            for (int j = 0; j < XC; ++j) {
                const int cc = j * TPR + ct;
                if (cc < nch) {
#pragma unroll
                    for (int e = 0; e < XE; ++e) {
                        const half8_t b = pb[cc * XE + e];
#pragma unroll
                        for (int m = 0; m < M; ++m)
#pragma unroll
                            for (int i = 0; i < 8; ++i) xr[m][j][e][i] = from_f32<half_t>(to_f32(xr[m][j][e][i]) + to_f32(b[i]));
                    }
                }
            }
        }
#pragma unroll
        for (int m = 0; m < M; ++m) {
            float ss = 0.f;
#pragma unroll
            for (int j = 0; j < XC; ++j)
#pragma unroll
                for (int e = 0; e < XE; ++e) ss = dot8(xr[m][j][e], xr[m][j][e], ss);
            ss = wave_sum(ss);
            if (lane == 0) ssq[wave][m] = ss;
        }
        __syncthreads();
#pragma unroll
        for (int m = 0; m < M; ++m) {
            const float inv = rsqrtf((RI == 1 ? ssq[0][m] + ssq[1][m] + ssq[2][m] + ssq[3][m] : ssq[0][m] + ssq[1][m]) / static_cast<float>(K) + a.eps);
#pragma unroll
            for (int j = 0; j < XC; ++j)
#pragma unroll
                for (int e = 0; e < XE; ++e)
#pragma unroll
                    for (int i = 0; i < 8; ++i)
                        xr[m][j][e][i] = from_f32<half_t>(to_f32(xr[m][j][e][i]) * to_f32(g[j][e][i]) * inv);
        }
    }
    if constexpr (WBITS == 4) {
#pragma unroll
        for (int m = 0; m < M; ++m)
#pragma unroll
            for (int j = 0; j < XC; ++j)
#pragma unroll
                for (int e = 0; e < XE; ++e) xr[m][j][e] = prescale_x_int4(permute_x_int4(xr[m][j][e]));
    }
    float xcorr4[WBITS == 4 ? M : 1][WBITS == 4 ? XC : 1];
    if constexpr (WBITS == 4) {
#pragma unroll
        for (int m = 0; m < M; ++m)
#pragma unroll
            for (int j = 0; j < XC; ++j) {
                float t = 0.f;
#pragma unroll
                for (int e = 0; e < XE; ++e) t += int4_offset_term(xr[m][j][e]);
                xcorr4[m][j] = -t;
            }
    }
    __shared__ float amx[FP8 ? 4 : 1][M], xscale_sh[M];
    if constexpr (FP8) {
#pragma unroll
        for (int m = 0; m < M; ++m) {
            float amax = 0.f;
#pragma unroll
            for (int j = 0; j < XC; ++j)
#pragma unroll
                for (int e = 0; e < XE; ++e)
#pragma unroll
                    for (int i = 0; i < 8; ++i) amax = fmaxf(amax, fabsf(to_f32(xr[m][j][e][i])));
            amax = wave_max(amax);
            if (lane == 0) amx[wave][m] = amax;
        }
        __syncthreads();
#pragma unroll
        for (int m = 0; m < M; ++m) {
            const float amax = fmaxf(fmaxf(amx[0][m], amx[1][m]), fmaxf(amx[2][m], amx[3][m]));
            const float sc = amax > 0.f ? amax / 448.0f : 1.0f;
            if (tid == 0) xscale_sh[m] = sc;
#pragma unroll
            for (int j = 0; j < XC; ++j)
#pragma unroll
                for (int e = 0; e < XE; ++e)
#pragma unroll
                    for (int i = 0; i < 8; i += 2) {
                        const float f0 = fminf(fmaxf(to_f32(xr[m][j][e][i]) / sc, -448.f), 448.f);
                        const float f1 = fminf(fmaxf(to_f32(xr[m][j][e][i + 1]) / sc, -448.f), 448.f);
                        const int pk = __builtin_amdgcn_cvt_pk_fp8_f32(f0, f1, 0, false);
                        const half2_t h = __builtin_amdgcn_cvt_scalef32_pk_f16_fp8(pk, 1.0f, false);
                        xr[m][j][e][i] = h[0];
                        xr[m][j][e][i + 1] = h[1];
                    }
        }
    }

    float xcorr[M];
#pragma unroll
    for (int m = 0; m < M; ++m) {
        xcorr[m] = 0.f;
        if constexpr (WBITS == 8 && !FP8) {
            float sx = 0.f;
#pragma unroll
            for (int j = 0; j < XC; ++j)
#pragma unroll
                for (int e = 0; e < XE; ++e)
#pragma unroll
                    for (int i = 0; i < 8; ++i) sx += to_f32(xr[m][j][e][i]);
            xcorr[m] = -1152.0f * sx;
        }
    }
    auto step = [&](auto &wb, auto &wsc, auto &wbn, auto &wscn, const int cur, const int it) {
        const int nxt = cur + gridDim.x;
        if constexpr (DB) {
            if (nxt < ngroups) load_group(nxt, wbn, wscn);
        }
        float acc[M][RPW];
#pragma unroll
        for (int r = 0; r < RPW; ++r) {
            float sc[XC];
            if constexpr (WBITS == 4) {
#pragma unroll
                for (int j = 0; j < XC; ++j) sc[j] = to_f32(wsc[r][j]);
            }
#pragma unroll
            for (int m = 0; m < M; ++m) {
                float sdot = xcorr[m];
#pragma unroll
                for (int j = 0; j < XC; ++j) {
                    if constexpr (WBITS == 4) sdot = fmaf(sc[j], chunk_dot<4>(wb[r][j], xr[m][j], xcorr4[m][j]), sdot);
                    else sdot = chunk_dot<WBITS, FP8>(wb[r][j], xr[m][j], sdot);
                }
                acc[m][r] = sdot;
            }
        }
        if constexpr (!DB) {
            if (nxt < ngroups) load_group(nxt, wb, wsc);
        }
#pragma unroll
        for (int r = 0; r < RPW; ++r)
#pragma unroll
            for (int m = 0; m < M; ++m) acc[m][r] = wave_sum(acc[m][r]);
        float *slot = &red[it & 1][0][0];
        if (lane == 0) {
#pragma unroll
            for (int m = 0; m < M; ++m)
#pragma unroll
                for (int r = 0; r < RPW; ++r) slot[wave * (M * RPW) + m * RPW + r] = acc[m][r];
        }
        __syncthreads();
        auto row_scale = [&](int row) {
            if constexpr (FP8) return reinterpret_cast<const float *>(a.scale)[row];
            else return (WBITS == 8) ? to_f32(scale[row]) : 1.0f;
        };
        if (swiglu) {
            if (tid < M * (RPW / 2) * RI) {
                const int m = tid / ((RPW / 2) * RI), qh = tid % ((RPW / 2) * RI), q = qh / RI, h = qh % RI;
                const int col = (cur * (RPW / 2) + q) * RI + h;
                if (col < half_n) {
                    float gt = 0.f, up = 0.f;
#pragma unroll
                    for (int w = 0; w < WPR; ++w) {
                        gt += slot[(h * WPR + w) * (M * RPW) + m * RPW + 2 * q];
                        up += slot[(h * WPR + w) * (M * RPW) + m * RPW + 2 * q + 1];
                    }
                    gt *= row_scale(col) * (FP8 ? xscale_sh[m] : 1.0f);
                    up *= row_scale(col + half_n) * (FP8 ? xscale_sh[m] : 1.0f);
                    a.y[static_cast<size_t>(m) * out_n + col] = from_f32<half_t>((gt / (1.0f + expf(-gt))) * up);
                }
            }
        } else {
            if (tid < M * RPW * RI) {
                const int m = tid / (RPW * RI), rh = tid % (RPW * RI), r = rh / RI, h = rh % RI;
                const int col = (cur * RPW + r) * RI + h;
                if (col < N) {
                    float v = 0.f;
#pragma unroll
                    for (int w = 0; w < WPR; ++w) v += slot[(h * WPR + w) * (M * RPW) + m * RPW + r];
                    v *= row_scale(col) * (FP8 ? xscale_sh[m] : 1.0f);
                    if (a.bias) v += to_f32(a.bias[col]);
                    if (a.residual) v += to_f32(a.residual[static_cast<size_t>(m) * N + col]);
                    a.y[static_cast<size_t>(m) * N + col] = from_f32<half_t>(v);
                }
            }
        }
    };
    for (int it = 0; grp < ngroups;) {
        step(wbA, wscA, wbB, wscB, grp, it);
        grp += gridDim.x;
        ++it;
        if constexpr (DB) {
            if (grp < ngroups) {
                step(wbB, wscB, wbA, wscA, grp, it);
                grp += gridDim.x;
                ++it;
            }
        }
    }
}

template <int M>
__global__ __launch_bounds__(256) void gemv_lds_kernel(const GemvArgs a) {
    constexpr int U = 8;
    extern __shared__ __attribute__((aligned(16))) unsigned char smem_raw[];
    half8_t *xs = reinterpret_cast<half8_t *>(smem_raw);
    __shared__ float inv_rms[M];
    const int K = a.K, N = a.N;
    const int nch = K >> 3, total = M * nch;
    const int tid = threadIdx.x, lane = tid & 63, wave = tid >> 6;
    const bool swiglu = a.epi == EPI_SWIGLU;
    {
        const half8_t *xg = reinterpret_cast<const half8_t *>(a.x);
        const half8_t *pb = reinterpret_cast<const half8_t *>(a.pre_bias);
        for (int i = tid; i < total; i += 256) {
            half8_t v = xg[i];
            if (a.norm && pb) {
                const half8_t b = pb[i % nch];
#pragma unroll
                for (int e = 0; e < 8; ++e) v[e] = from_f32<half_t>(to_f32(v[e]) + to_f32(b[e]));
            }
            xs[i] = v;
        }
    }
    __syncthreads();
    if (a.norm) {
        for (int m = wave; m < M; m += 4) {
            float ss = 0.f;
            for (int c = lane; c < nch; c += 64) {
                const half8_t v = xs[m * nch + c];
                ss = dot8(v, v, ss);
            }
            ss = wave_sum(ss);
            if (lane == 0) inv_rms[m] = rsqrtf(ss / static_cast<float>(K) + a.eps);
        }
        __syncthreads();
        const half8_t *gm = reinterpret_cast<const half8_t *>(a.gamma);
        for (int i = tid; i < total; i += 256) {
            const int m = i / nch, c = i - m * nch;
            half8_t v = xs[i];
            const half8_t g = gm[c];
            const float sc = inv_rms[m];
#pragma unroll
            for (int e = 0; e < 8; ++e) v[e] = from_f32<half_t>(to_f32(v[e]) * to_f32(g[e]) * sc);
            xs[i] = v;
        }
        __syncthreads();
    }
    const int half_n = N >> 1;
    const int npairs = swiglu ? half_n : ((N + 1) >> 1);
    for (int pair = blockIdx.x * 4 + wave; pair < npairs; pair += gridDim.x * 4) {
        const int r0 = swiglu ? pair : 2 * pair;
        const int r1 = swiglu ? pair + half_n : min(2 * pair + 1, N - 1);
        const half8_t *w0 = reinterpret_cast<const half8_t *>(static_cast<const half_t *>(a.W) + static_cast<size_t>(r0) * K);
        const half8_t *w1 = reinterpret_cast<const half8_t *>(static_cast<const half_t *>(a.W) + static_cast<size_t>(r1) * K);
        float acc0[M], acc1[M];
#pragma unroll
        for (int m = 0; m < M; ++m) acc0[m] = acc1[m] = 0.f;
        for (int c = lane; c < nch; c += 64 * U) {
            half8_t a0[U], a1[U];
#pragma unroll
            for (int u = 0; u < U; ++u) {
                const int cc = c + 64 * u;
                if (cc < nch) {
                    a0[u] = load_nt(w0 + cc);
                    a1[u] = load_nt(w1 + cc);
                }
            }
#pragma unroll
            for (int u = 0; u < U; ++u) {
                const int cc = c + 64 * u;
                if (cc < nch) {
#pragma unroll
                    for (int m = 0; m < M; ++m) {
                        const half8_t xv = xs[m * nch + cc];
                        acc0[m] = dot8(a0[u], xv, acc0[m]);
                        acc1[m] = dot8(a1[u], xv, acc1[m]);
                    }
                }
            }
        }
#pragma unroll
        for (int m = 0; m < M; ++m) {
            acc0[m] = wave_sum(acc0[m]);
            acc1[m] = wave_sum(acc1[m]);
        }
        if (lane == 0) {
#pragma unroll
            for (int m = 0; m < M; ++m) {
                if (swiglu) {
                    const float gt = acc0[m], up = acc1[m];
                    a.y[static_cast<size_t>(m) * half_n + pair] = from_f32<half_t>((gt / (1.0f + expf(-gt))) * up);
                } else {
                    float v0 = acc0[m], v1 = acc1[m];
                    const bool has1 = 2 * pair + 1 < N;
                    if (a.bias) {
                        v0 += to_f32(a.bias[r0]);
                        v1 += to_f32(a.bias[r1]);
                    }
                    if (a.residual) {
                        v0 += to_f32(a.residual[static_cast<size_t>(m) * N + r0]);
                        if (has1) v1 += to_f32(a.residual[static_cast<size_t>(m) * N + r1]);
                    }
                    a.y[static_cast<size_t>(m) * N + r0] = from_f32<half_t>(v0);
                    if (has1) a.y[static_cast<size_t>(m) * N + r1] = from_f32<half_t>(v1);
                }
            }
        }
    }
}

template <int MT, int NT, int NW, int EPI>
__global__ __launch_bounds__(NW * 64) void skinny_mfma_f16_kernel(const half_t *__restrict__ x,
                                                                  const half_t *__restrict__ W,
                                                                  half_t *__restrict__ y, int M, int K,
                                                                  int N, const half_t *__restrict__ bias,
                                                                  const half_t *residual) {
    __shared__ floatx4 red[NW][NT * MT][64];
    const int lane = threadIdx.x & 63, wave = threadIdx.x >> 6;
    const int r = lane & 15, q = lane >> 4;
    const int half_n = N >> 1;
    int nrow[NT];
    if constexpr (EPI == EPI_SWIGLU) {
        static_assert(NT == 2, "swiglu epilogue pairs a gate tile with its up tile");
        nrow[0] = blockIdx.x * 16 + r;
        nrow[1] = nrow[0] + half_n;
    } else {
#pragma unroll
        for (int t = 0; t < NT; ++t) nrow[t] = (blockIdx.x * NT + t) * 16 + r;
    }
    const int nlimit = (EPI == EPI_SWIGLU) ? half_n : N;
    const half_t *wp[NT];
#pragma unroll
    for (int t = 0; t < NT; ++t) {
        const int rr = (EPI == EPI_SWIGLU) ? min(nrow[0], half_n - 1) + t * half_n : min(nrow[t], N - 1);
        wp[t] = W + static_cast<size_t>(rr) * K + 8 * q;
    }
    const half_t *xp[MT];
    bool xok[MT];
#pragma unroll
    for (int j = 0; j < MT; ++j) {
        xok[j] = (16 * j + r) < M;
        xp[j] = x + static_cast<size_t>(xok[j] ? 16 * j + r : 0) * K + 8 * q;
    }
    floatx4 acc[NT][MT];
#pragma unroll
    for (int t = 0; t < NT; ++t)
#pragma unroll
        for (int j = 0; j < MT; ++j) acc[t][j] = floatx4{0.f, 0.f, 0.f, 0.f};

    constexpr int U = 4;
    const int ksteps = K >> 5;
// ... 453 lines not shown
```

llm-inference-engine_amd/csrc/linear.hip:

```cpp
#include "gemm_kernels.cuh"
#include "gemm256.cuh"
#include "gemm8p.cuh"
#include "gemm_mid.cuh"
#include "llmie_internal.h"

#include <algorithm>
#include <cstdlib>

namespace llmie {

template <int M, int RPW, int XC, int WBITS, bool DB = false, bool FP8 = false, int RI = 1> static void launch_ksplit(const GemvArgs &a, hipStream_t st) {
    const bool swiglu = a.epi == EPI_SWIGLU;
    const int groups = swiglu ? (a.N / 2 + (RPW / 2) * RI - 1) / ((RPW / 2) * RI) : (a.N + RPW * RI - 1) / (RPW * RI);
    constexpr int target = (WBITS == 16 || WBITS == 4) ? 512 : 768;
    const int iters = (groups + target - 1) / target;
    const int grid = (groups + iters - 1) / iters;
    gemv_ksplit_kernel<M, RPW, XC, WBITS, DB, FP8, RI><<<grid, 256, 0, st>>>(a);
}

static int ksplit_xc(int K, int wbits) { return (K * wbits / 128 + 255) / 256; }

struct KsplitForm {
    int xc, rpw;
};
constexpr int kKsplitForms = 5;
constexpr KsplitForm ksplit_form_at(int wbits, bool fp8, int i) {
    constexpr KsplitForm f16[kKsplitForms] = {{1, 8}, {2, 4}, {4, 4}, {6, 4}, {8, 2}};
    constexpr KsplitForm q[kKsplitForms] = {{1, 8}, {2, 4}, {3, 2}, {0, 0}, {0, 0}};
    if (wbits == 16) return f16[i];
    if (i == 0 && wbits == 8 && !fp8) return KsplitForm{1, 4};
    return q[i];
}
static int ksplit_form(int M, int K, int wbits) {
    if (M < 1 || M > 8 || K % (128 / wbits) != 0) return -1;
    const int xe = wbits == 16 ? 1 : (wbits == 8 ? 2 : 4);
    const int xc = ksplit_xc(K, wbits);
    for (int i = 0; i < kKsplitForms; ++i) {
        const KsplitForm f = ksplit_form_at(wbits, false, i);
        if (f.xc && xc <= f.xc) return M * f.xc * xe <= 16 ? i : -1;
    }
    return -1;
}
bool ksplit_eligible(int M, int K, int wbits) { return ksplit_form(M, K, wbits) >= 0; }

template <int M, int WBITS, bool FP8, int I> static void launch_ksplit_form(const GemvArgs &a, hipStream_t st) {
    constexpr KsplitForm f = ksplit_form_at(WBITS, FP8, I);
    if constexpr (f.xc != 0 && M * f.xc * WFmt<WBITS>::XE <= 16) {
        if constexpr (WBITS == 4 && I == 0) {
            if (a.K * WBITS / 128 <= 128 && (a.epi != EPI_SWIGLU || (a.N / 2) % 2 == 0)) {
                launch_ksplit<M, 8, 1, WBITS, true, FP8, 2>(a, st);
                return;
            }
        }
        launch_ksplit<M, f.rpw, f.xc, WBITS, WBITS != 16, FP8>(a, st);
    }
}
template <int M, int WBITS, bool FP8 = false> static void dispatch_ksplit(int form, const GemvArgs &a, hipStream_t st) {
    switch (form) {
        case 0: launch_ksplit_form<M, WBITS, FP8, 0>(a, st); break;
        case 1: launch_ksplit_form<M, WBITS, FP8, 1>(a, st); break;
        case 2: launch_ksplit_form<M, WBITS, FP8, 2>(a, st); break;
        case 3: launch_ksplit_form<M, WBITS, FP8, 3>(a, st); break;
        case 4: launch_ksplit_form<M, WBITS, FP8, 4>(a, st); break;
        default: break;
    }
}

static int gemv_f16_route(int M, int K) {
    if (K % 8 || M < 1 || M > 8) return LR_REFUSED;
    if (ksplit_form(M, K, 16) >= 0) return LR_GEMV_KSPLIT;
    return static_cast<size_t>(M) * K * 2 <= 64 * 1024 ? LR_GEMV_LDS : LR_REFUSED;
}

template <int M> static void dispatch_gemv_m(const GemvArgs &a, hipStream_t st) {
    const int form = ksplit_form(M, a.K, 16);
    if (form >= 0) return dispatch_ksplit<M, 16>(form, a, st);
    const bool swiglu = a.epi == EPI_SWIGLU;
    const int npairs = swiglu ? a.N / 2 : (a.N + 1) / 2;
    int wgs = (npairs + 3) / 4;
    if (wgs > 2048) wgs = 2048;
    gemv_lds_kernel<M><<<wgs, 256, static_cast<size_t>(M) * a.K * sizeof(half_t), st>>>(a);
}

static void dispatch_gemv(int M, const GemvArgs &a, hipStream_t st) {
    switch (M) {
        case 1: return dispatch_gemv_m<1>(a, st);
        case 2: return dispatch_gemv_m<2>(a, st);
        case 3: return dispatch_gemv_m<3>(a, st);
        case 4: return dispatch_gemv_m<4>(a, st);
        case 5: return dispatch_gemv_m<5>(a, st);
        case 6: return dispatch_gemv_m<6>(a, st);
        case 7: return dispatch_gemv_m<7>(a, st);
        case 8: return dispatch_gemv_m<8>(a, st);
        default: return;
    }
}

template <int WBITS, bool FP8 = false> static bool dispatch_gemv_q(int M, const GemvArgs &a, hipStream_t st) {
    const int form = ksplit_form(M, a.K, WBITS);
    if (form < 0) return false;
    switch (M) {
        case 1: dispatch_ksplit<1, WBITS, FP8>(form, a, st); break;
        case 2: dispatch_ksplit<2, WBITS, FP8>(form, a, st); break;
        case 3: dispatch_ksplit<3, WBITS, FP8>(form, a, st); break;
        case 4: dispatch_ksplit<4, WBITS, FP8>(form, a, st); break;
        case 5: dispatch_ksplit<5, WBITS, FP8>(form, a, st); break;
        case 6: dispatch_ksplit<6, WBITS, FP8>(form, a, st); break;
        case 7: dispatch_ksplit<7, WBITS, FP8>(form, a, st); break;
        default: dispatch_ksplit<8, WBITS, FP8>(form, a, st); break;
    }
    return true;
}
void gemv_q_launch(int wbits, int M, const GemvArgs &a, hipStream_t st) {
    if (wbits == 8) dispatch_gemv_q<8>(M, a, st);
    else dispatch_gemv_q<4>(M, a, st);
}
bool gemv_fp8_launch(int M, const GemvArgs &a, hipStream_t st) { return dispatch_gemv_q<8, true>(M, a, st); }

template <int EPI>
static void dispatch_skinny(int M, const half_t *x, const half_t *W, half_t *y, int K, int N,
                            const half_t *bias, const half_t *residual, hipStream_t st) {
    constexpr int NW = 8;
    const int mt = (M + 15) / 16;
    if constexpr (EPI == EPI_SWIGLU) {
        const int wgs = (N / 2 + 15) / 16;
        switch (mt) {
            case 1: skinny_mfma_f16_kernel<1, 2, NW, EPI><<<wgs, NW * 64, 0, st>>>(x, W, y, M, K, N, bias, residual); break;
            case 2: skinny_mfma_f16_kernel<2, 2, NW, EPI><<<wgs, NW * 64, 0, st>>>(x, W, y, M, K, N, bias, residual); break;
            case 3: skinny_mfma_f16_kernel<3, 2, NW, EPI><<<wgs, NW * 64, 0, st>>>(x, W, y, M, K, N, bias, residual); break;
            case 4: skinny_mfma_f16_kernel<4, 2, NW, EPI><<<wgs, NW * 64, 0, st>>>(x, W, y, M, K, N, bias, residual); break;
            default: break;
        }
    } else {
        const int tiles = (N + 15) / 16;
        switch (mt) {
            case 1: skinny_mfma_f16_kernel<1, 1, NW, EPI><<<tiles, NW * 64, 0, st>>>(x, W, y, M, K, N, bias, residual); break;
            case 2: skinny_mfma_f16_kernel<2, 2, NW, EPI><<<(tiles + 1) / 2, NW * 64, 0, st>>>(x, W, y, M, K, N, bias, residual); break;
            case 3: skinny_mfma_f16_kernel<3, 2, NW, EPI><<<(tiles + 1) / 2, NW * 64, 0, st>>>(x, W, y, M, K, N, bias, residual); break;
            case 4: skinny_mfma_f16_kernel<4, 2, NW, EPI><<<(tiles + 1) / 2, NW * 64, 0, st>>>(x, W, y, M, K, N, bias, residual); break;
            default: break;
        }
    }
}

template <typename T>
static void launch_generic(const T *a, const T *b, T *c, int batch, int M, int N, int K, bool trans_b,
                           const T *bias, const T *residual, hipStream_t st) {
    dim3 grid((N + 63) / 64, (M + 63) / 64, batch);
    const size_t sa = static_cast<size_t>(M) * K, sb = static_cast<size_t>(N) * K, sc = static_cast<size_t>(M) * N;
    if (trans_b)
        generic_gemm_kernel<T, true><<<grid, 256, 0, st>>>(a, b, c, M, N, K, sa, sb, sc, bias, residual);
    else
        generic_gemm_kernel<T, false><<<grid, 256, 0, st>>>(a, b, c, M, N, K, sa, sb, sc, bias, residual);
}

static __global__ __launch_bounds__(256) void skinny_finalize_kernel(const float *__restrict__ slab, half_t *y, int M, int N, int KS,
                                                              const SlabScale scale, const half_t *__restrict__ bias,
                                                              const half_t *residual, int epi) {
    const int out_n = epi == EPI_SWIGLU ? N / 2 : N;
    const size_t total = static_cast<size_t>(M) * out_n;
    const size_t slab_sz = static_cast<size_t>(M) * N;
    for (size_t i = blockIdx.x * 256ull + threadIdx.x; i < total; i += static_cast<size_t>(gridDim.x) * 256) {
        const int m = static_cast<int>(i / out_n), n = static_cast<int>(i - static_cast<size_t>(m) * out_n);
        auto gather = [&](int col) {
            float v = 0.f;
            for (int k = 0; k < KS; ++k) v += slab[k * slab_sz + static_cast<size_t>(m) * N + col];
            return scale.apply(v, m, col);
        };
        float v;
        if (epi == EPI_SWIGLU) {
            const float gt = gather(n), up = gather(n + out_n);
            v = (gt / (1.0f + expf(-gt))) * up;
        } else {
            v = gather(n);
            if (bias) v += to_f32(bias[n]);
            if (residual) v += to_f32(residual[static_cast<size_t>(m) * N + n]);
        }
        y[static_cast<size_t>(m) * out_n + n] = from_f32<half_t>(v);
    }
}

template <bool SWIGLU>
static __global__ __launch_bounds__(256) void splitk_finalize4_kernel(const float *__restrict__ slab, half_t *y, int M, int N, int KS,
                                                                      const SlabScale scale, const half_t *__restrict__ bias,
                                                                      const half_t *residual) {
    const int out_n = SWIGLU ? N / 2 : N, n4 = out_n / 4;
    const size_t total = static_cast<size_t>(M) * n4, slab_sz = static_cast<size_t>(M) * N;
    constexpr int NV = SWIGLU ? 2 : 1;
    for (size_t i = blockIdx.x * 256ull + threadIdx.x; i < total; i += static_cast<size_t>(gridDim.x) * 256) {
        const int m = static_cast<int>(i / n4), n = static_cast<int>(i - static_cast<size_t>(m) * n4) * 4;
        floatx4 v[NV];
        for (int k0 = 0; k0 < KS; k0 += 8) {
            floatx4 t[8][NV];
#pragma unroll
            for (int kk = 0; kk < 8; ++kk)
#pragma unroll
// ... 866 lines not shown
```

llm-inference-engine_amd/csrc/llmie_internal.h:

```cpp
#pragma once
#include "device_utils.cuh"

namespace llmie {

enum : int { EPI_NONE_ = 0, EPI_SWIGLU_ = 1 };

struct SlabWs {
    float *p;
    size_t floats;
};
size_t linear_splitk_ws_floats(int wbits, int M, int K, int N);

enum LinearRoute : int {
    LR_REFUSED = 0,
    LR_GEMV_KSPLIT, LR_GEMV_LDS, LR_SPLITK, LR_SPLITK_PASSES, LR_SKINNY, LR_SWIGLU256, LR_TILES256, LR_TILES256_PART, LR_TILES128, LR_GENERIC,
    LR_W8_G8P, LR_W8_G8P_SWIGLU, LR_W8_SPLITK_PASSES, LR_WQ_IMAGE_PREFILL, LR_WQ_IMAGE_LAST, LR_WQ_GEMV, LR_W4_SPLITK, LR_W4_CHUNKS,
    LR_W8_SPLITK, LR_W8_SKINNY,
};
enum LinearRefusal : int { LREF_NONE = 0, LREF_F16_SWIGLU, LREF_SLABS, LREF_W4_SPLITK, LREF_WQ_NORM, LREF_WQ_SWIGLU, LREF_WQ_SHAPE };
struct LinearCall {
    int bits, M, K, N, epi, group;
    bool bias, residual, gamma, pre_bias;
    unsigned mis_x, mis_w, mis_y, mis_bias, mis_residual, mis_gamma, mis_pre_bias, mis_scale, mis_image;
    bool slabs;
    size_t slab_floats;
    bool image;
    size_t image_bytes;
};
struct LinearPlan {
    int route;
    int refusal;
    size_t slab_floats;
    size_t image_bytes;
    int pass_rows;
    int inner;
};
inline unsigned mis16(const void *p) { return static_cast<unsigned>(reinterpret_cast<uintptr_t>(p) % 16); }
LinearCall linear_call_sizing(int bits, int M, int K, int N, int epi, int group = 128);
LinearCall linear_call(int bits, int M, int K, int N, int epi, int group, const void *x, const void *w, const void *scale, const void *y,
                       const void *bias, const void *residual, const void *gamma, const void *pre_bias, SlabWs ws, const void *image,
                       size_t image_bytes);
LinearPlan plan_linear_f16(const LinearCall &c);
LinearPlan plan_linear_wq(const LinearCall &c);
const char *linear_route_name(int route);
int linear_refuse(const LinearCall &c, const LinearPlan &p);
size_t linear_f16_reserve_slab_floats(int M, int K, int N);
int linear_f16_nk(const half_t *x, const half_t *W, half_t *y, int M, int K, int N, int epi,
                  const half_t *bias, const half_t *residual, SlabWs ws, hipStream_t st);

bool gemv_f16_eligible(int M, int K, const void *x, const void *W);
int linear_f16_nk_norm(const half_t *x, const half_t *W, half_t *y, int M, int K, int N, int epi, const half_t *bias,
                       const half_t *residual, const half_t *gamma, const half_t *pre_bias, float eps, hipStream_t st);

struct SplitKSlabs {
    float *slab;
    int KS, M, N;
};
enum : int { WF_FP8 = 108 };
int linear_splitk_partial(int wbits, const void *x, const void *W, int M, int K, int N, hipStream_t st, SplitKSlabs *out,
                          SlabWs ws, const half_t *gscale = nullptr );
int splitk_finalize(const SplitKSlabs &sk, const SlabScale &sc, half_t *y, int epi, const half_t *bias, const half_t *residual,
                    hipStream_t st);
bool splitk_rownorm_eligible(int N);
int splitk_rownorm(const SplitKSlabs &sk, const SlabScale &wscale, const half_t *bias, half_t *resid, const half_t *gamma,
                   float eps, half_t *y, uint8_t *xq, float *xscale, hipStream_t st);
bool rmsnorm_quant_eligible(int hidden);
int rmsnorm_quant_f16(const half_t *x, half_t *resid, const half_t *bias, const half_t *gamma, float eps, int tokens, int hidden,
                      bool fused, uint8_t *xq, float *xscale, hipStream_t st);
bool rmsnorm_oop_eligible(int hidden);
int rmsnorm_oop_f16(const half_t *x, half_t *y, const half_t *gamma, float eps, int tokens, int hidden, hipStream_t st);
int quantize_rows_fp8(const half_t *x, uint8_t *xq, float *xscale, int M, int K, hipStream_t st);
int linear_splitk(int wbits, const half_t *x, const void *W, const half_t *scale, half_t *y, int M, int K, int N, int epi,
                  const half_t *bias, const half_t *residual, SlabWs ws, hipStream_t st);
enum G256Operands : int { G256_F16 = 0, G256_E4M3 = 1, G256_W8 = 2 };
enum G256Form : int { G256_PLAIN = 0, G256_SWIGLU = 1, G256_QKV_ROPE = 2 };
struct G256Range {
    bool eight_phase;
    int width, col0, tiles;
};
struct G256Plan {
    int ranges;
    G256Range range[2];
};
G256Plan plan_gemm256(G256Form form, G256Operands ops, int M, int N, int K);
bool gemm256_fills(int M, int N);
bool gemm256_swiglu_fills(int M, int two_inter);
int gemm256_narrow_rounds(int M, int N);
bool gemm8p_fits(int N, int K, int elem_bytes);
void gemm256_launch(G256Operands ops, const void *x, const void *W, half_t *y, int M, int N, int K, const half_t *bias,
                    const half_t *residual, const float *xscale, const float *wscale, hipStream_t st);
void gemm256_swiglu_launch(G256Operands ops, const void *x, const void *W, half_t *y, int M, int two_inter, int K, const float *xscale,
                           const float *wscale, hipStream_t st);
bool gemm256_qkv_rope_eligible(G256Operands ops, int M, int N, int K, const void *x, const void *W, const void *wscale, const void *qkv);
void gemm256_qkv_rope_launch(G256Operands ops, const void *x, const void *W, half_t *qkv, int M, int N, int K, const float *xscale,
                             const float *wscale, const half_t *bias, const QkvRopeArgs *rap, int layer, hipStream_t st);
int dequantize_weights_f16(int wbits, const void *wq, const half_t *scale, half_t *w16, int N, int K, int group, hipStream_t st);
constexpr int kWqPrefillRows = 192;
size_t linear_wq_dequant_bytes(int wbits, int M, int K, int N);
struct WqWorkspace {
    void *deq;
    size_t deq_bytes;
    SlabWs slabs;
};
WqWorkspace wq_workspace(int wbits, int M, int K, int N, void *workspace, size_t workspace_bytes);
struct GemvArgs;
bool ksplit_eligible(int M, int K, int wbits);
void gemv_q_launch(int wbits, int M, const GemvArgs &a, hipStream_t st);
bool gemv_fp8_launch(int M, const GemvArgs &a, hipStream_t st);
int linear_fp8_gemv(const half_t *x, const uint8_t *wq, const float *wscale, half_t *y, int M, int K, int N, int epi,
                    const half_t *bias, const half_t *residual, const half_t *gamma, const half_t *pre_bias, float eps,
                    hipStream_t st);
int linear_fp8(const half_t *x, const uint8_t *w_fp8, const float *w_scale, half_t *y, int M, int K, int N, const half_t *bias,
               const half_t *residual, void *act_ws, size_t act_ws_bytes, SlabWs slabs, hipStream_t st);
int linear_wq(int wbits, const half_t *x, const void *wq, const half_t *scale, half_t *y, int M, int K, int N, int group,
              int epi, const half_t *bias, const half_t *residual, const half_t *gamma, const half_t *pre_bias, float eps,
              SlabWs ws, hipStream_t st, void *deq = nullptr, size_t deq_bytes = 0);

enum : int { PKF_F16 = 16, PKF_I8 = 8, PKF_I4 = 4, PKF_FP8 = 108 };
enum : int { PKE_PLAIN = 0, PKE_SWIGLU = 1 };
enum : int { PKX_X = 1, PKX_Y = 2, PKX_RES = 4 };
size_t pk_packed_bytes(int wf, int N, int K, int swiglu);
size_t pk_packed_scale_bytes(int wf, int N, int K, int swiglu);
int pk_pack(int wf, const void *src, const void *src_scale, void *dst, void *dst_scale, int N, int K, int swiglu, hipStream_t st);
int pk_unpack_f16(int wf, const void *packed, const half_t *scale, half_t *w16, int N, int K, int swiglu, hipStream_t st);
bool pk_eligible(int wf, int M, int K, int N, int epi);
size_t pk_slab_floats(int wf, int M, int K, int N);
int pk_linear(int wf, const half_t *x, const void *Wp, const void *scale, half_t *y, int M, int K, int N, int epi, int x32_flags,
              const half_t *residual, const half_t *gamma, const half_t *pre_bias, float eps, float *slab_ws, size_t slab_ws_floats,
              hipStream_t st);
int x32_convert(const half_t *src, half_t *dst, int M, int K, int to_x32, hipStream_t st);
struct PkChain {
    int wf, M, nph, lds;
    bool ok;
    unsigned long long *stamps;
    alignas(16) unsigned char args[1024];
};
void pk_chain_begin(PkChain *ch, int wf, int M);
int pk_chain_add(PkChain *ch, int slot , const half_t *x, const void *Wp, const void *scale, half_t *y, int K, int N, int epi, int x32_flags,
                 const half_t *residual, const half_t *gamma, const half_t *pre_bias, float eps, float *slab_ws, size_t slab_ws_floats);
int pk_chain_launch(PkChain *ch, unsigned *sync, unsigned *err, hipStream_t st);
size_t pk_chain_sync_bytes();

struct KvView {
    void *k, *v;
    const int32_t *block_table;
    int max_pages, num_pages;
    int fp8;
    float k_scale, v_scale;
};
inline KvView kv_dense(void *k, void *v) { return KvView{k, v, nullptr, 0, 0, 0, 1.f, 1.f}; }
struct DecodePos {
    int step;
    const int32_t *step_dev;
    int ragged;
};
int decoder_mha_rope(const void *qkv, const void *qkv_bias, const KvView &kv, void *out, int layer, int batch,
                     int head_num, int kv_head_num, int head_size, int max_seq_len, const DecodePos &pos,
                     void *workspace, size_t workspace_bytes, const float2 *rope, int rot_dim,
                     int32_t *tickets ,
                     llmie_dtype dtype, hipStream_t st,
                     const SplitKSlabs *qkv_slabs = nullptr ,
                     const SlabScale *qkv_scale = nullptr,
                     int out_x32 = 0 );

int topk_round1_only(const void *probs, int32_t *tmp_ids, void *tmp_vals, int rows, int vocab, int K, int bpr, llmie_dtype dtype, hipStream_t st);
int decode_tail(const int32_t *tmp_ids, const void *tmp_vals, int32_t *ids, void *vals, int K, int bpr, int32_t *seq_len, uint8_t *finished,
                int32_t *out_id, int rows, int step, int32_t *step_dev, int end_id, int vocab, const void *embed, void *next_hidden, int hidden,
                int advance, unsigned *ticket, llmie_dtype dtype, hipStream_t st);

int prefill_attention_f16(half_t *qkv, const half_t *qkv_bias, const KvView &kv, half_t *out,
                          const int32_t *cum_seqlens, const int32_t *history_len, const float2 *rope, int layer, int batch,
                          int num_tokens, int max_q_len, int head_num, int kv_head_num, int head_size, int max_seq_len,
                          int rotary_dim, hipStream_t st,
                          int rope_done = 0 );
bool splitk_finalize_qkv_rope_eligible(const SplitKSlabs &sk, int head_size, const void *qkv, const void *bias);
int splitk_finalize_qkv_rope(const SplitKSlabs &sk, const SlabScale &sc, half_t *qkv, const half_t *qkv_bias, const KvView &kv,
                             const int32_t *cum_seqlens, const int32_t *history_len, const float2 *rope, int layer, int batch, int head_num,
                             int kv_head_num, int max_seq_len, int rotary_dim, hipStream_t st);
int prefill_token_table(const int32_t *cum_seqlens, const int32_t *history_len, int batch, int num_tokens, int32_t *tok_b, int32_t *tok_tpos,
                        QkvRopeArgs args, QkvRopeArgs *args_dev, hipStream_t st);

int sample_logits_check(const void *logits, int batch, int vocab, const llmie_sampling_params *params, const int32_t *history,
                        int history_stride, const int32_t *history_len, const int32_t *seq_len, const uint8_t *finished,
                        const int32_t *out_id, const void *workspace, size_t workspace_bytes, llmie_dtype dtype);
int sample_logits_launch(const void *logits, int batch, int vocab, const llmie_sampling_params *params, int32_t *history,
                         int history_stride, int32_t *history_len, int history_append, int32_t *seq_len, uint8_t *finished,
                         int32_t *out_id, float *out_logprob, int step, const int32_t *step_dev, int end_id, void *workspace,
                         llmie_dtype dtype, const void *embed, void *next_hidden, int hidden, int advance, unsigned *ticket,
                         hipStream_t st);

}
```

Baseline: 383.5 tokens/s.

## Overlap K/V projection GEMV with attention over cached tokens in one launch

The QKV GEMM is split so only the Q rows are computed first. A combined kernel then runs the K/V projection GEMV (with RoPE, bias and cache write) in some workgroups while other workgroups attend over the old KV cache, which excludes the new token. A small merge kernel folds in the new token's score and value when combining the split partials. The aim is to hide attention's KV-cache reads behind the K/V weight streaming and shorten the serial QKV→attention dependency. The cost is an extra kernel launch per layer, more partial-merge work, and shared workgroup resources between two different workloads.

```diff
diff --git a/include/llmie.h b/include/llmie.h
--- a/include/llmie.h
+++ b/include/llmie.h
@@ -236,6 +236,7 @@
 #define LLMIE_SW_CHAIN 8u
 #define LLMIE_SW_NO_FUSED_SHORT_PREFILL 16u
 #define LLMIE_SW_NO_QKV_ROPE_FUSION 32u
+#define LLMIE_SW_NO_KV_OVERLAP 64u
 const char *llmie_decoder_plan_name(const llmie_decoder_config *cfg, int prefill, int rows, unsigned call_flags, unsigned switch_mask);
 
 typedef struct llmie_decoder llmie_decoder;
diff --git a/llm-inference-engine_amd/csrc/attention_decode.hip b/llm-inference-engine_amd/csrc/attention_decode.hip
--- a/llm-inference-engine_amd/csrc/attention_decode.hip
+++ b/llm-inference-engine_amd/csrc/attention_decode.hip
@@ -1,3 +1,4 @@
+#include "gemm_kernels.cuh"
 #include "llmie_internal.h"
 
 #include <cstdlib>
@@ -126,8 +127,11 @@
     return o / (L + 1e-6f);
 }
 
-template <typename T, int HS, int REP, int kAttnWaves = 4, int kAttnG = 8, typename KT = T>
-__global__ __launch_bounds__(kAttnWaves * 64) void decode_attn_split_kernel(
+__device__ __forceinline__ float rope_rotate(float x, float partner, float rc, float rs) { return x * rc + partner * rs; }
+
+template <typename T, int HS, int REP, int kAttnWaves, int kAttnG, typename KT, bool OLD_ONLY>
+__device__ __forceinline__ void decode_attn_split_body(
+    const int split, const int g, const int b,
     const T *__restrict__ qkv, const T *__restrict__ qkv_bias, KT *k_cache, KT *v_cache,
     float *__restrict__ part, T *__restrict__ out, int head_num, int kv_head_num, int max_seq_len,
     int step_arg, const int32_t *__restrict__ step_dev, int max_splits,
@@ -144,22 +148,21 @@
     constexpr bool FP8KV = std::is_same<KT, fp8kv_t>::value;
     static_assert(HS % N == 0 && LPT >= 1 && LPT <= 64 && (LPT & (LPT - 1)) == 0, "head size");
 
-    const int split = blockIdx.x, g = blockIdx.y, b = blockIdx.z;
-    const int step = seq_step(step_dev, step_arg, pg.step_stride, b, max_seq_len);
+    const int step_all = seq_step(step_dev, step_arg, pg.step_stride, b, max_seq_len);
+    const int step = OLD_ONLY ? step_all - 1 : step_all;
     const int span = cpw * CHUNK;
     const int t0 = split * span;
     if (t0 >= step) return;
     int tc0 = t0;
     int t_end = min(step, tc0 + CHUNK);
     const int nsplits = (step + span - 1) / span;
-    const int batch = gridDim.z;
 
     const int lane = threadIdx.x & 63, wave = threadIdx.x >> 6;
     const int sub = lane / LPT, dl = lane % LPT;
     const int qkv_heads = head_num + 2 * kv_head_num;
     const float scale = rsqrtf(static_cast<float>(HS));
 
-    const T *row = qkv + static_cast<size_t>(b) * qkv_heads * HS;
+    const T *row = qkv + static_cast<size_t>(b) * (OLD_ONLY ? head_num : qkv_heads) * HS;
     constexpr int NPG = CHUNK > KV_PAGE ? CHUNK / KV_PAGE : 1;
     static_assert(CHUNK % KV_PAGE == 0 || KV_PAGE % CHUNK == 0, "chunk vs page size");
     int pg0 = 0;
@@ -183,12 +186,12 @@
     auto krow = [&](int t) { return kbase[NPG == 1 ? 0 : (t / KV_PAGE - pg0)] + static_cast<size_t>(t % KV_PAGE) * HS; };
     auto vrow = [&](int t) { return vbase[NPG == 1 ? 0 : (t / KV_PAGE - pg0)] + static_cast<size_t>(t % KV_PAGE) * HS; };
     KT *kc = kbase[0];
-    const int t_new = step - 1;
+    const int t_new = step_all - 1;
     T qraw[REP][N];
     constexpr int ITEMS_PER_HEAD = HS / 4;
     constexpr int LROUNDS = ((REP + 2) * ITEMS_PER_HEAD + NT - 1) / NT;
     __shared__ __attribute__((aligned(16))) T qkvlds[(REP + 2) * HS];
-    const bool wg_has_new = t_new >= t0 && t_new < t0 + span;
+    const bool wg_has_new = !OLD_ONLY && t_new >= t0 && t_new < t0 + span;
     floatx4 spart[LROUNDS][4];
     half4_t sscale[LROUNDS];
     floatx4 sscalef[LROUNDS];
@@ -219,13 +222,17 @@
     const int hk = head_num + g, hv = head_num + kv_head_num + g;
     const T *dummy = reinterpret_cast<const T *>(kc);
     T knraw[N], vnraw[N], qbias[REP][N], kbias[N], vbias[N];
-    load_elems<T, N>(qs.slab ? dummy : row + static_cast<size_t>(hk) * HS + dl * N, knraw);
-    load_elems<T, N>(qs.slab ? dummy : row + static_cast<size_t>(hv) * HS + dl * N, vnraw);
+    if constexpr (!OLD_ONLY) {
+        load_elems<T, N>(qs.slab ? dummy : row + static_cast<size_t>(hk) * HS + dl * N, knraw);
+        load_elems<T, N>(qs.slab ? dummy : row + static_cast<size_t>(hv) * HS + dl * N, vnraw);
+    }
 #pragma unroll
     for (int r = 0; r < REP; ++r)
         load_elems<T, N>(qkv_bias ? qkv_bias + static_cast<size_t>(g * REP + r) * HS + dl * N : dummy, qbias[r]);
-    load_elems<T, N>(qkv_bias ? qkv_bias + static_cast<size_t>(hk) * HS + dl * N : dummy, kbias);
-    load_elems<T, N>(qkv_bias ? qkv_bias + static_cast<size_t>(hv) * HS + dl * N : dummy, vbias);
+    if constexpr (!OLD_ONLY) {
+        load_elems<T, N>(qkv_bias ? qkv_bias + static_cast<size_t>(hk) * HS + dl * N : dummy, kbias);
+        load_elems<T, N>(qkv_bias ? qkv_bias + static_cast<size_t>(hv) * HS + dl * N : dummy, vbias);
+    }
     float2 csraw[N];
     if (rope) {
         const float2 *cs = rope + static_cast<size_t>(t_new) * (HS / 2) + (dl % (LPT / 2)) * N;
@@ -285,7 +292,7 @@
 #pragma unroll
         for (int e = 0; e < N; ++e) {
             const float partner = (LPT / 2 < 16) ? lane_xor_lt16<(LPT / 2 < 16 ? LPT / 2 : 8)>(x[e]) : __shfl_xor(x[e], LPT / 2, 64);
-            x[e] = x[e] * rc[e] + partner * rs[e];
+            x[e] = rope_rotate(x[e], partner, rc[e], rs[e]);
         }
     };
     const float k_p2 = __builtin_bit_cast(float, __builtin_bit_cast(uint32_t, k_scale) & 0x7f800000u);
@@ -317,7 +324,7 @@
     }
 
     V knv, vnv;
-    {
+    if constexpr (!OLD_ONLY) {
         T kn[N], vn[N];
 #pragma unroll
         for (int e = 0; e < N; ++e) {
@@ -346,7 +353,7 @@
     }
     auto inject = [&]() {
         bool mine = false;
-        if (t_new >= tc0 && t_new < tc0 + CHUNK) {
+        if (!OLD_ONLY && t_new >= tc0 && t_new < tc0 + CHUNK) {
 #pragma unroll
         for (int i = 0; i < kAttnG; ++i) {
             const bool is_new = tok[i] == t_new;
@@ -491,7 +498,7 @@
             o += f * s_o[r][w][d];
         }
         const int h = g * REP + r;
-        if (nsplits == 1) {
+        if (!OLD_ONLY && nsplits == 1) {
             out[attn_out_index(pg.out_x32, b, h * HS + d, head_num * HS)] = from_f32<T>(o / (L + 1e-6f));
         } else {
             float *p = part + ((static_cast<size_t>(b) * head_num + h) * max_splits + split) * (HS + 2);
@@ -502,8 +509,7 @@
             }
         }
     }
-    (void)batch;
-    if (tickets && nsplits > 1) {
+    if (!OLD_ONLY && tickets && nsplits > 1) {
         __shared__ int s_ticket;
         asm volatile("s_waitcnt vmcnt(0)" ::: "memory");
         __syncthreads();
@@ -531,6 +537,17 @@
             }
         }
     }
+}
+
+template <typename T, int HS, int REP, int kAttnWaves = 4, int kAttnG = 8, typename KT = T>
+__global__ __launch_bounds__(kAttnWaves * 64) void decode_attn_split_kernel(
+    const T *__restrict__ qkv, const T *__restrict__ qkv_bias, KT *k_cache, KT *v_cache, float *__restrict__ part, T *__restrict__ out,
+    int head_num, int kv_head_num, int max_seq_len, int step_arg, const int32_t *__restrict__ step_dev, int max_splits,
+    const float2 *__restrict__ rope, int rotary_dim, int32_t *tickets, const QkvSlabs qs, const float k_scale, const float v_scale,
+    const PagedKv pg, const int cpw) {
+    decode_attn_split_body<T, HS, REP, kAttnWaves, kAttnG, KT, false>(blockIdx.x, blockIdx.y, blockIdx.z, qkv, qkv_bias, k_cache, v_cache, part,
+                                                                      out, head_num, kv_head_num, max_seq_len, step_arg, step_dev, max_splits,
+                                                                      rope, rotary_dim, tickets, qs, k_scale, v_scale, pg, cpw);
 }
 
 template <typename T>
@@ -808,6 +825,211 @@
                                     step_dev, workspace, workspace_bytes, rope, rot_dim, tickets, qs, st, pg, num_pages);
 }
 
+
+template <int HS> struct KvProjRows {
+    static constexpr bool custom = true;
+    const half_t *bias;
+    half_t *kc, *vc;
+    half_t *kv_new;
+    const float2 *rope;
+    int rotary_dim, head_num, kv_head_num, max_seq_len;
+    int step;
+    template <int RPW> __device__ __forceinline__ int ngroups() const { return (kv_head_num * HS + RPW / 2 - 1) / (RPW / 2); }
+    template <int RPW> __device__ __forceinline__ int row_of(int grp, int r) const {
+        const int nk = kv_head_num * (HS / 2);
+        const int item = min(grp * (RPW / 2) + (r >> 1), 2 * nk - 1);
+        if (item < nk) return head_num * HS + (item / (HS / 2)) * HS + item % (HS / 2) + (r & 1) * (HS / 2);
+        return (head_num + kv_head_num) * HS + 2 * (item - nk) + (r & 1);
+    }
+    template <int M, int RPW> __device__ __forceinline__ void store(int cur, const float *slot, int tid) const {
+        if (tid >= M * (RPW / 2) || step == 0) return;
+        const int m = tid / (RPW / 2), q = tid % (RPW / 2);
+        const int nk = kv_head_num * (HS / 2), item = cur * (RPW / 2) + q;
+        if (item >= 2 * nk) return;
+        float s0 = 0.f, s1 = 0.f;
+#pragma unroll
+        for (int w = 0; w < 4; ++w) {
+            s0 += slot[w * (M * RPW) + m * RPW + 2 * q];
+            s1 += slot[w * (M * RPW) + m * RPW + 2 * q + 1];
+        }
+        half_t x0 = from_f32<half_t>(s0), x1 = from_f32<half_t>(s1);
+        const int t_new = step - 1;
+        const bool is_k = item < nk;
+        const int col = is_k ? (item / (HS / 2)) * HS + item % (HS / 2) : 2 * (item - nk);
+        const int second = is_k ? HS / 2 : 1;
+        const int g = col / HS, d = col % HS;
+        if (is_k && rope) {
+            const float2 cs = d < (rotary_dim >> 1) ? rope[static_cast<size_t>(t_new) * (HS / 2) + d] : float2{1.f, 0.f};
+            const float f0 = rope_rotate(to_f32(x0), to_f32(x1), cs.x, -cs.y), f1 = rope_rotate(to_f32(x1), to_f32(x0), cs.x, cs.y);
+            x0 = from_f32<half_t>(f0);
+            x1 = from_f32<half_t>(f1);
+        }
+        if (bias) {
+            const half_t *bp = bias + static_cast<size_t>(head_num + (is_k ? 0 : kv_head_num)) * HS + col;
+            x0 = from_f32<half_t>(to_f32(x0) + to_f32(bp[0]));
+            x1 = from_f32<half_t>(to_f32(x1) + to_f32(bp[second]));
+        }
+        half_t *c = (is_k ? kc : vc) + ((static_cast<size_t>(m) * kv_head_num + g) * max_seq_len + t_new) * HS + d;
+        c[0] = x0;
+        c[second] = x1;
+        half_t *n = kv_new + (static_cast<size_t>(m) * 2 + (is_k ? 0 : 1)) * kv_head_num * HS + col;
+        n[0] = x0;
+        n[second] = x1;
+    }
+};
+
+template <int M, int RPW, int XC, int HS, int REP>
+__global__ __launch_bounds__(256) void decode_kv_overlap_kernel(const GemvArgs a, KvProjRows<HS> rows, const half_t *__restrict__ q,
+                                                                float *__restrict__ part, int step_arg,
+                                                                const int32_t *__restrict__ step_dev, int max_splits, int attn_splits,
+                                                                int proj_wgs) {
+    if (static_cast<int>(blockIdx.x) < proj_wgs) {
+        rows.step = seq_step(step_dev, step_arg, 0, 0, rows.max_seq_len);
+        gemv_ksplit_body<M, RPW, XC, 16, false, false, 1>(a, blockIdx.x, proj_wgs, rows);
+    } else {
+        const int idx = blockIdx.x - proj_wgs;
+        const int split = idx % attn_splits, gb = idx / attn_splits;
+        decode_attn_split_body<half_t, HS, REP, 4, 8, half_t, true>(
+            split, gb % rows.kv_head_num, gb / rows.kv_head_num, q, rows.bias, rows.kc, rows.vc, part, nullptr, rows.head_num,
+            rows.kv_head_num, rows.max_seq_len, step_arg, step_dev, max_splits, rows.rope, rows.rotary_dim, nullptr,
+            QkvSlabs{nullptr, 0, 0, SlabScale{nullptr, nullptr, nullptr}}, 1.f, 1.f, PagedKv{nullptr, 0, 0, 0}, 1);
+    }
+}
+
+template <int HS>
+__global__ __launch_bounds__(HS < 64 ? 64 : HS) void decode_attn_merge_new_kernel(
+    const float *__restrict__ part, const half_t *__restrict__ q, const half_t *__restrict__ qkv_bias, const half_t *__restrict__ kv_new,
+    half_t *__restrict__ out, int head_num, int kv_head_num, int chunk, int step_arg, const int32_t *__restrict__ step_dev, int max_splits,
+    int max_seq_len, const float2 *__restrict__ rope, int rotary_dim) {
+    constexpr int NT = HS < 64 ? 64 : HS;
+    __shared__ float red[NT / 64];
+    const int h = blockIdx.x, b = blockIdx.y, g = h / (head_num / kv_head_num);
+    const int d = min(static_cast<int>(threadIdx.x), HS - 1);
+    const size_t stride = static_cast<size_t>(HS) + 2;
+    const float *p = part + (static_cast<size_t>(b) * head_num + h) * max_splits * stride;
+    float ms[16], ls[16], os[16];
+    merge_load(p, 0, max_splits - 1, stride, d, ms, ls, os);
+    const half_t *qr = q + (static_cast<size_t>(b) * head_num + h) * HS;
+    const half_t qx = qr[d], qp = qr[d ^ (HS / 2)];
+    const half_t qb = qkv_bias ? qkv_bias[static_cast<size_t>(h) * HS + d] : half_t(0);
+    const half_t *kn = kv_new + (static_cast<size_t>(b) * 2 * kv_head_num + g) * HS;
+    const half_t kx = kn[d], vx = kn[static_cast<size_t>(kv_head_num) * HS + d];
+    const int step = seq_step(step_dev, step_arg, 0, b, max_seq_len);
+    if (step == 0) return;
+    float f = to_f32(qx);
+    if (rope) {
+        const int i = d % (HS / 2);
+        const float2 cs = i < (rotary_dim >> 1) ? rope[static_cast<size_t>(step - 1) * (HS / 2) + i] : float2{1.f, 0.f};
+        f = to_f32(from_f32<half_t>(rope_rotate(f, to_f32(qp), cs.x, d < HS / 2 ? -cs.y : cs.y)));
+    }
+    f += qkv_bias ? to_f32(qb) : 0.f;
+    const float qf = f * rsqrtf(static_cast<float>(HS));
+    const float m_new = block_sum<NT / 64>(static_cast<int>(threadIdx.x) < HS ? qf * to_f32(kx) : 0.f, red);
+    const int nsplits = (step - 1 + chunk - 1) / chunk;
+    float M = -INFINITY, L = 0.f, o = 0.f;
+    merge_round(ms, ls, os, 0, nsplits, M, L, o);
+    for (int s0 = 16; s0 < nsplits; s0 += 16) {
+        merge_load(p, s0, nsplits - 1, stride, d, ms, ls, os);
+        merge_round(ms, ls, os, s0, nsplits, M, L, o);
+    }
+    ms[0] = m_new;
+    ls[0] = 1.f;
+    os[0] = to_f32(vx);
+    merge_round(ms, ls, os, 0, 1, M, L, o);
+    if (static_cast<int>(threadIdx.x) < HS) out[(static_cast<size_t>(b) * head_num + h) * HS + d] = from_f32<half_t>(o / (L + 1e-6f));
+}
+
+constexpr int kKvProjWgs = 512;
+
+struct KvOverlapCall {
+    GemvArgs a;
+    const half_t *bias, *q;
+    half_t *kc, *vc, *kv_new, *out;
+    float *part;
+    const float2 *rope;
+    int rot_dim, batch, head_num, kv_head_num, max_seq_len, step;
+    const int32_t *step_dev;
+};
+template <int M, int RPW, int XC, int HS, int REP> static void launch_kv_overlap(const KvOverlapCall &c, hipStream_t st) {
+    using G = AttnGeom<half_t, HS, 4, 8>;
+    const int max_splits_ws = (c.max_seq_len + attn_min_chunk() - 1) / attn_min_chunk();
+    const int bound = (c.step_dev ? c.max_seq_len : c.step) - 1;
+    const int attn_splits = (bound + G::CHUNK - 1) / G::CHUNK;
+    const int groups = (c.kv_head_num * HS + RPW / 2 - 1) / (RPW / 2);
+    const int iters = (groups + kKvProjWgs - 1) / kKvProjWgs;
+    const int proj_wgs = (groups + iters - 1) / iters;
+    const KvProjRows<HS> rows{c.bias, c.kc, c.vc, c.kv_new, c.rope, c.rot_dim, c.head_num, c.kv_head_num, c.max_seq_len, 0};
+    decode_kv_overlap_kernel<M, RPW, XC, HS, REP><<<proj_wgs + attn_splits * c.kv_head_num * c.batch, 256, 0, st>>>(
+        c.a, rows, c.q, c.part, c.step, c.step_dev, max_splits_ws, attn_splits, proj_wgs);
+    decode_attn_merge_new_kernel<HS><<<dim3(c.head_num, c.batch), HS < 64 ? 64 : HS, 0, st>>>(
+        c.part, c.q, c.bias, c.kv_new, c.out, c.head_num, c.kv_head_num, G::CHUNK, c.step, c.step_dev, max_splits_ws, c.max_seq_len,
+        c.rope, c.rot_dim);
+}
+template <int M, int RPW, int XC, int HS> static void kv_overlap_rep(int rep, const KvOverlapCall &c, hipStream_t st) {
+    switch (rep) {
+        case 1: return launch_kv_overlap<M, RPW, XC, HS, 1>(c, st);
+        case 2: return launch_kv_overlap<M, RPW, XC, HS, 2>(c, st);
+        case 4: return launch_kv_overlap<M, RPW, XC, HS, 4>(c, st);
+        default: return launch_kv_overlap<M, RPW, XC, HS, 8>(c, st);
+    }
+}
+template <int M, int RPW, int XC> static void kv_overlap_hs(int hs, int rep, const KvOverlapCall &c, hipStream_t st) {
+    if constexpr (M * XC <= 16) {
+        if (hs == 128) kv_overlap_rep<M, RPW, XC, 128>(rep, c, st);
+        else kv_overlap_rep<M, RPW, XC, 64>(rep, c, st);
+    }
+}
+template <int M> static void kv_overlap_form(int xc, int hs, int rep, const KvOverlapCall &c, hipStream_t st) {
+    switch (xc) {
+        case 1: return kv_overlap_hs<M, 8, 1>(hs, rep, c, st);
+        case 2: return kv_overlap_hs<M, 4, 2>(hs, rep, c, st);
+        default: return kv_overlap_hs<M, 4, 4>(hs, rep, c, st);
+    }
+}
+
+static bool kv_overlap_form_of(int batch, int K, int *xc) {
+    int rpw;
+    return batch >= 1 && batch <= 5 && gemv_f16_ksplit_form(batch, K, xc, &rpw) && ((*xc == 1 && rpw == 8) || ((*xc == 2 || *xc == 4) && rpw == 4));
+}
+bool decoder_kv_overlap_eligible(int batch, int K, int head_num, int kv_head_num, int head_size) {
+    int xc;
+    const int rep = kv_head_num > 0 ? head_num / kv_head_num : 0;
+    return kv_overlap_form_of(batch, K, &xc) && (head_size == 64 || head_size == 128) && (rep == 1 || rep == 2 || rep == 4 || rep == 8) &&
+           head_num == rep * kv_head_num;
+}
+int decoder_kv_overlap(const half_t *x, const half_t *wqkv, const half_t *gamma, float eps, const half_t *q, const half_t *qkv_bias,
+                       half_t *kv_new, const KvView &kv, half_t *out, int layer, int batch, int K, int head_num, int kv_head_num,
+                       int head_size, int max_seq_len, const DecodePos &pos, void *workspace, size_t workspace_bytes, const float2 *rope,
+                       int rot_dim, hipStream_t st) {
+    int xc = 0;
+    const size_t need = llmie_decoder_mha_workspace_bytes(batch, head_num, head_size, max_seq_len);
+    if (!decoder_kv_overlap_eligible(batch, K, head_num, kv_head_num, head_size) || !kv_overlap_form_of(batch, K, &xc) || kv.block_table ||
+        kv.fp8 || pos.ragged || (!pos.step_dev && (pos.step < 1 || pos.step > max_seq_len)) ||
+        (mis16(x) | mis16(wqkv) | mis16(gamma) | mis16(q) | mis16(qkv_bias) | mis16(kv_new) | mis16(kv.k) | mis16(kv.v)) != 0) {
+        set_error("decoder_kv_overlap: batch %d, K %d, heads %d/%d x %d: not a shape of the K/V-overlap launch", batch, K, head_num, kv_head_num,
+                  head_size);
+        return LLMIE_ERR_UNSUPPORTED;
+    }
+    if (!workspace || workspace_bytes < need) {
+        set_error("decoder_kv_overlap: workspace too small (%zu < %zu bytes)", workspace_bytes, need);
+        return LLMIE_ERR_WORKSPACE;
+    }
+    const size_t layer_off = static_cast<size_t>(layer) * batch * kv_head_num * max_seq_len * head_size;
+    const int qkv_rows = (head_num + 2 * kv_head_num) * head_size;
+    const KvOverlapCall c{GemvArgs{x, wqkv, nullptr, K, qkv_rows, nullptr, nullptr, gamma, nullptr, eps, EPI_NONE, 1, nullptr, 0},
+                          qkv_bias, q, static_cast<half_t *>(kv.k) + layer_off, static_cast<half_t *>(kv.v) + layer_off, kv_new, out,
+                          static_cast<float *>(workspace), rope, rot_dim, batch, head_num, kv_head_num, max_seq_len, pos.step, pos.step_dev};
+    const int rep = head_num / kv_head_num;
+    switch (batch) {
+        case 1: kv_overlap_form<1>(xc, head_size, rep, c, st); break;
+        case 2: kv_overlap_form<2>(xc, head_size, rep, c, st); break;
+        case 3: kv_overlap_form<3>(xc, head_size, rep, c, st); break;
+        case 4: kv_overlap_form<4>(xc, head_size, rep, c, st); break;
+        default: kv_overlap_form<5>(xc, head_size, rep, c, st); break;
+    }
+    return launch_status("decoder_kv_overlap");
+}
+
 }
 
 using namespace llmie;
diff --git a/llm-inference-engine_amd/csrc/engine.hip b/llm-inference-engine_amd/csrc/engine.hip
--- a/llm-inference-engine_amd/csrc/engine.hip
+++ b/llm-inference-engine_amd/csrc/engine.hip
@@ -2,6 +2,7 @@
 
 #include <cmath>
 #include <cstdlib>
+#include <cstring>
 #include <new>
 #include <vector>
 
@@ -499,18 +500,25 @@
 }
 
 struct EngineSwitches {
-    bool no_fused_decode, no_fused_batch, no_packed_batch, chain, no_fused_short_prefill, no_qkv_rope_fusion;
+    bool no_fused_decode, no_fused_batch, no_packed_batch, chain, no_fused_short_prefill, no_qkv_rope_fusion, no_kv_overlap;
 };
+static const char kNoKvOverlapEnv[] = "LLMIE_NO_KV_OVERLAP";
+constexpr bool kKvOverlapDefault = false;
+static bool no_kv_overlap_env() {
+    const char *v = getenv(kNoKvOverlapEnv);
+    return v ? strcmp(v, "0") != 0 : !kKvOverlapDefault;
+}
 static const EngineSwitches &engine_switches() {
     static const EngineSwitches s{getenv("LLMIE_NO_FUSED_DECODE") != nullptr,        getenv("LLMIE_NO_FUSED_BATCH") != nullptr,
                                   getenv("LLMIE_NO_PACKED_BATCH") != nullptr,        getenv("LLMIE_CHAIN") != nullptr,
-                                  getenv("LLMIE_NO_FUSED_SHORT_PREFILL") != nullptr, getenv("LLMIE_NO_QKV_ROPE_FUSION") != nullptr};
+                                  getenv("LLMIE_NO_FUSED_SHORT_PREFILL") != nullptr, getenv("LLMIE_NO_QKV_ROPE_FUSION") != nullptr,
+                                  no_kv_overlap_env()};
     return s;
 }
 static EngineSwitches switches_of_mask(unsigned m) {
     return EngineSwitches{(m & LLMIE_SW_NO_FUSED_DECODE) != 0,        (m & LLMIE_SW_NO_FUSED_BATCH) != 0, (m & LLMIE_SW_NO_PACKED_BATCH) != 0,
                           (m & LLMIE_SW_CHAIN) != 0,                  (m & LLMIE_SW_NO_FUSED_SHORT_PREFILL) != 0,
-                          (m & LLMIE_SW_NO_QKV_ROPE_FUSION) != 0};
+                          (m & LLMIE_SW_NO_QKV_ROPE_FUSION) != 0,     (m & LLMIE_SW_NO_KV_OVERLAP) != 0 || !kKvOverlapDefault};
 }
 static bool fused_attention_geometry(const llmie_decoder_config &c) {
     const int rep = c.head_num / c.kv_head_num;
@@ -663,6 +671,7 @@
     int H, QKV, I, wbits;
     bool fp8;
     llmie_dtype dt;
+    bool no_kv_overlap;
 
     int attention(const void *qkv, const void *qkv_bias, void *out, int layer, const SplitKSlabs *qkv_slabs = nullptr,
                   const SlabScale *qkv_scale = nullptr, int out_x32 = 0) const {
@@ -694,10 +703,22 @@
                              epi, nullptr, (const half_t *)residual, (const half_t *)gamma, (const half_t *)pre_bias,
                              c.rms_eps, dec->slab_ws, st);
         };
+        const int Hq = c.head_num * c.head_size;
+        const bool kv_overlap = !no_kv_overlap && wbits == 16 && !fp8 && !kv.fp8 && !kv.block_table && !pos.ragged &&
+                                decoder_kv_overlap_eligible(batch, H, c.head_num, c.kv_head_num, c.head_size);
         for (int l = 0; l < c.num_layers; ++l) {
             const llmie_layer_weights &w = dec->layers[l];
-            TIMED(LLMIE_OP_QKV_GEMM, lin(h, w.qkv, dec->qkv, H, QKV, EPI_NONE_, nullptr, w.attn_norm_gamma, nullptr));
-            TIMED(LLMIE_OP_MHA, attention(dec->qkv, w.qkv.bias, dec->mha, l));
+            if (kv_overlap && !mis16(w.qkv.data) && !mis16(w.qkv.bias) && !mis16(w.attn_norm_gamma)) {
+                half_t *q = reinterpret_cast<half_t *>(dec->qkv);
+                TIMED(LLMIE_OP_QKV_GEMM, lin(h, w.qkv, q, H, Hq, EPI_NONE_, nullptr, w.attn_norm_gamma, nullptr));
+                TIMED(LLMIE_OP_MHA, decoder_kv_overlap((const half_t *)h, (const half_t *)w.qkv.data, (const half_t *)w.attn_norm_gamma, c.rms_eps, q,
+                                                       (const half_t *)w.qkv.bias, q + static_cast<size_t>(batch) * Hq, kv, (half_t *)dec->mha, l,
+                                                       batch, H, c.head_num, c.kv_head_num, c.head_size, c.max_seq_len, pos, dec->attn_ws,
+                                                       dec->attn_ws_bytes, dec->rope_table, c.rotary_dim, st));
+            } else {
+                TIMED(LLMIE_OP_QKV_GEMM, lin(h, w.qkv, dec->qkv, H, QKV, EPI_NONE_, nullptr, w.attn_norm_gamma, nullptr));
+                TIMED(LLMIE_OP_MHA, attention(dec->qkv, w.qkv.bias, dec->mha, l));
+            }
             TIMED(LLMIE_OP_O_GEMM, lin(dec->mha, w.o, h, H, H, EPI_NONE_, h, nullptr, nullptr));
             TIMED(LLMIE_OP_GATE_UP_SWIGLU, lin(h, w.gate_up, dec->act, H, 2 * I, EPI_SWIGLU_, nullptr, w.ffn_norm_gamma, w.o.bias));
             TIMED(LLMIE_OP_DOWN_GEMM, lin(dec->act, w.down, h, I, H, EPI_NONE_, h, nullptr, nullptr));
@@ -869,7 +890,7 @@
     const DecodePlan plan = plan_decode(call);
     const DecodeStep s{dec, c, hidden_out, batch, kv_view(c, k_cache, v_cache, block_table, max_pages, num_pages), pos, stream, as_stream(stream),
                        dec->H, dec->QKV, dec->I, c.wfmt == LLMIE_W_F16 ? 16 : (c.wfmt == LLMIE_W_INT8 ? 8 : (c.wfmt == LLMIE_W_INT4 ? 4 : 0)),
-                       c.wfmt == LLMIE_W_FP8, c.dtype};
+                       c.wfmt == LLMIE_W_FP8, c.dtype, call.sw.no_kv_overlap};
     switch (plan.path) {
         case DP_GEMV: return s.gemv();
         case DP_PACKED: return plan.chain_wanted && s.chain_joins() ? s.packed_chain() : s.packed();
diff --git a/llm-inference-engine_amd/csrc/gemm_kernels.cuh b/llm-inference-engine_amd/csrc/gemm_kernels.cuh
--- a/llm-inference-engine_amd/csrc/gemm_kernels.cuh
+++ b/llm-inference-engine_amd/csrc/gemm_kernels.cuh
@@ -87,8 +87,12 @@
     return half8_t{v[0], v[4], v[1], v[5], v[2], v[6], v[3], v[7]};
 }
 
-template <int M, int RPW, int XC, int WBITS, bool DB = false, bool FP8 = false, int RI = 1>
-__global__ __launch_bounds__(256) void gemv_ksplit_kernel(const GemvArgs a) {
+struct GemvPlainRows {
+    static constexpr bool custom = false;
+};
+template <int M, int RPW, int XC, int WBITS, bool DB, bool FP8, int RI, class Rows>
+__device__ __forceinline__ void gemv_ksplit_body(const GemvArgs &a, const int first_grp, const int grp_stride, const Rows &rows) {
+    static_assert(!Rows::custom || (RI == 1 && WBITS == 16), "custom rows: fp16 weights, one row per workgroup instruction");
     static_assert(RPW % 2 == 0, "rows come in pairs");
     constexpr int XE = WFmt<WBITS>::XE;
     constexpr int EPC = 8 * XE;
@@ -105,8 +109,10 @@
     const bool swiglu = a.epi == EPI_SWIGLU;
     const int half_n = N >> 1;
     const int out_n = swiglu ? half_n : N;
-    const int ngroups = swiglu ? (half_n + (RPW / 2) * RI - 1) / ((RPW / 2) * RI) : (N + RPW * RI - 1) / (RPW * RI);
+    int ngroups = swiglu ? (half_n + (RPW / 2) * RI - 1) / ((RPW / 2) * RI) : (N + RPW * RI - 1) / (RPW * RI);
+    if constexpr (Rows::custom) ngroups = rows.template ngroups<RPW>();
     auto row_of = [&](int grp, int r) {
+        if constexpr (Rows::custom) return rows.template row_of<RPW>(grp, r);
         int row = swiglu ? (grp * (RPW / 2) + (r >> 1)) * RI + sub + (r & 1) * half_n : (grp * RPW + r) * RI + sub;
         const int lim = swiglu ? ((r & 1) ? N : half_n) : N;
         return row < lim ? row : lim - 1;
@@ -155,7 +161,7 @@
             }
         }
     };
-    int grp = blockIdx.x;
+    int grp = first_grp;
     if (grp < ngroups) load_group(grp, wbA, wscA);
 
     if (a.norm) {
@@ -271,7 +277,7 @@
         }
     }
     auto step = [&](auto &wb, auto &wsc, auto &wbn, auto &wscn, const int cur, const int it) {
-        const int nxt = cur + gridDim.x;
+        const int nxt = cur + grp_stride;
         if constexpr (DB) {
             if (nxt < ngroups) load_group(nxt, wbn, wscn);
         }
@@ -313,7 +319,9 @@
             if constexpr (FP8) return reinterpret_cast<const float *>(a.scale)[row];
             else return (WBITS == 8) ? to_f32(scale[row]) : 1.0f;
         };
-        if (swiglu) {
+        if constexpr (Rows::custom) {
+            rows.template store<M, RPW>(cur, slot, tid);
+        } else if (swiglu) {
             if (tid < M * (RPW / 2) * RI) {
                 const int m = tid / ((RPW / 2) * RI), qh = tid % ((RPW / 2) * RI), q = qh / RI, h = qh % RI;
                 const int col = (cur * (RPW / 2) + q) * RI + h;
@@ -347,16 +355,20 @@
     };
     for (int it = 0; grp < ngroups;) {
         step(wbA, wscA, wbB, wscB, grp, it);
-        grp += gridDim.x;
+        grp += grp_stride;
         ++it;
         if constexpr (DB) {
             if (grp < ngroups) {
                 step(wbB, wscB, wbA, wscA, grp, it);
-                grp += gridDim.x;
+                grp += grp_stride;
                 ++it;
             }
         }
     }
+}
+template <int M, int RPW, int XC, int WBITS, bool DB = false, bool FP8 = false, int RI = 1>
+__global__ __launch_bounds__(256) void gemv_ksplit_kernel(const GemvArgs a) {
+    gemv_ksplit_body<M, RPW, XC, WBITS, DB, FP8, RI>(a, blockIdx.x, gridDim.x, GemvPlainRows{});
 }
 
 template <int M>
diff --git a/llm-inference-engine_amd/csrc/linear.hip b/llm-inference-engine_amd/csrc/linear.hip
--- a/llm-inference-engine_amd/csrc/linear.hip
+++ b/llm-inference-engine_amd/csrc/linear.hip
@@ -42,6 +42,14 @@
     return -1;
 }
 bool ksplit_eligible(int M, int K, int wbits) { return ksplit_form(M, K, wbits) >= 0; }
+bool gemv_f16_ksplit_form(int M, int K, int *xc, int *rpw) {
+    const int form = ksplit_form(M, K, 16);
+    if (form < 0) return false;
+    const KsplitForm f = ksplit_form_at(16, false, form);
+    *xc = f.xc;
+    *rpw = f.rpw;
+    return true;
+}
 
 template <int M, int WBITS, bool FP8, int I> static void launch_ksplit_form(const GemvArgs &a, hipStream_t st) {
     constexpr KsplitForm f = ksplit_form_at(WBITS, FP8, I);
diff --git a/llm-inference-engine_amd/csrc/llmie_internal.h b/llm-inference-engine_amd/csrc/llmie_internal.h
--- a/llm-inference-engine_amd/csrc/llmie_internal.h
+++ b/llm-inference-engine_amd/csrc/llmie_internal.h
@@ -105,6 +105,7 @@
 WqWorkspace wq_workspace(int wbits, int M, int K, int N, void *workspace, size_t workspace_bytes);
 struct GemvArgs;
 bool ksplit_eligible(int M, int K, int wbits);
+bool gemv_f16_ksplit_form(int M, int K, int *xc, int *rpw);
 void gemv_q_launch(int wbits, int M, const GemvArgs &a, hipStream_t st);
 bool gemv_fp8_launch(int M, const GemvArgs &a, hipStream_t st);
 int linear_fp8_gemv(const half_t *x, const uint8_t *wq, const float *wscale, half_t *y, int M, int K, int N, int epi,
@@ -163,6 +164,12 @@
                      const SlabScale *qkv_scale = nullptr,
                      int out_x32 = 0 );
 
+bool decoder_kv_overlap_eligible(int batch, int K, int head_num, int kv_head_num, int head_size);
+int decoder_kv_overlap(const half_t *x, const half_t *wqkv, const half_t *gamma, float eps, const half_t *q, const half_t *qkv_bias,
+                       half_t *kv_new, const KvView &kv, half_t *out, int layer, int batch, int K, int head_num, int kv_head_num,
+                       int head_size, int max_seq_len, const DecodePos &pos, void *workspace, size_t workspace_bytes, const float2 *rope,
+                       int rot_dim, hipStream_t st);
+
 int topk_round1_only(const void *probs, int32_t *tmp_ids, void *tmp_vals, int rows, int vocab, int K, int bpr, llmie_dtype dtype, hipStream_t st);
 int decode_tail(const int32_t *tmp_ids, const void *tmp_vals, int32_t *ids, void *vals, int K, int bpr, int32_t *seq_len, uint8_t *finished,
                 int32_t *out_id, int rows, int step, int32_t *step_dev, int end_id, int vocab, const void *embed, void *next_hidden, int hidden,
```

Result: no change. 384.6 tokens/s (median of 6 runs) (+0.3%).
